# liortalker/MindTheEdge

Hardware: AMD Instinct MI355X
Metric: training images/sec, PackNet-SAN+edge-loss 384x1280 bf16 (higher is better)
Workload: dtype bf16; 1 GPU; T8: PackNet-SAN + silog + 4-scale depth-edge loss training step, 384x1280, 8 frames/GPU, dropout 0.5, flip 0.5; global_batch=8, height=384, width=1280, parallelism=single GPU

## Files before the change

### include/mte_kernels.h

```cpp
#ifndef MTE_KERNELS_H
#define MTE_KERNELS_H

#ifdef __cplusplus
extern "C" {
#endif

typedef struct ihipStream_t* mte_stream_t;

#define MTE_OK 0
#define MTE_ERR_ARG (-1)
#define MTE_ERR_LAUNCH (-2)
#define MTE_ERR_UNSUPPORTED (-3)
#define MTE_DT_BF16 0
#define MTE_DT_F32 1

#define MTE_CONV_ACCUMULATE 1
#define MTE_CONV_SOLO 2
int mte_conv2d_igemm(const void* x, long ldx, const void* wpack, const float* bias, void* y, long ldy, int out_f32,
                     int B, int H, int W, int Cin_p, int N, int KH, int KW, int dtype,
                     float* workspace, long workspace_elems, int accumulate, mte_stream_t stream);
int mte_conv2d_igemm_unshuffle(const void* x, long ldx, const void* wpack, void* y, long ldy,
                               int B, int H, int W, int Cin_p, int N, int KH, int KW, int dtype, int accumulate, mte_stream_t stream);
#define MTE_OPT_GN_PREZEROED 0
#define MTE_OPT_LOSS_PREZEROED 1
#define MTE_OPT_HANDOFF_FENCES 2
#define MTE_OPT_WGRAD_SHARES_CHIP 3
int mte_set_option(int option, int value);
#define MTE_DEVERR_GN_CLUSTER_FWD 1
#define MTE_DEVERR_GN_CLUSTER_BWD 2
#define MTE_DEVERR_IMAGE_RESAMPLE 4
int mte_device_error_init(void);
int mte_device_error_poll(void);
int mte_conv2d_wgrad(const void* x, long ldx, const void* dy, long ldy, float* dw_stage, int stage_parts, int* parts_out,
                     int B, int H, int W, int Cin_p, int N, int KH, int KW, int dtype, mte_stream_t stream);
int mte_conv2d_wgrad_nine_tap(int H, int W, int Cin_p, int N, int KH, int KW, int dtype);
int mte_pack_conv_weights(const float* w_oihw, void* wfwd, void* wbwd, int Cout, int Cin, int KH, int KW,
                          int Cin_p, int Cout_p, int dtype, mte_stream_t stream);
typedef struct { const float* w; void* wf; void* wb; void* pf; void* pb; int Cout, Cin, taps, Cin_p; int end_f, end_b, end_pf, end_pb; } mte_pack_job;
int mte_pack_conv_weights_multi(const void* jobs, int njobs, int dtype, mte_stream_t stream);
int mte_pack_conv_weights_bwd(const void* wfwd, void* wbwd, int Cout, int KH, int KW, int Cin_p, int dtype, mte_stream_t stream);
int mte_unpack_conv_wgrad(float* dw_stage, int parts, float* dw_oihw, int Cout, int Cin, int KH, int KW, int Cin_p, mte_stream_t stream);
int mte_colsum(const void* y, long ld, long M, int N, float* out, int dtype, mte_stream_t stream);

int mte_conv2d_patch_supported(int W, int Cin_p, int N, int KH, int KW, int dtype);
int mte_conv2d_patch_wgrad_supported(int W, int Cin_p, int N, int KH, int KW, int dtype);
long mte_conv2d_patch_pack_elems(int Cin_p, int N, int KH, int KW);
int mte_conv2d_patch_repack(const void* wgeneric, void* wpatch, int Cin_p, int N, int KH, int KW, mte_stream_t stream);
int mte_conv2d_patch_fwd(const void* x, long ldx, const void* wpatch, const float* bias, void* y, long ldy,
                         int B, int H, int W, int Cin_p, int N, int KH, int KW, int accumulate, mte_stream_t stream);
int mte_conv2d_patch_wgrad(const void* x, long ldx, const void* dy, long lddy, float* dw_stage, int stage_parts, int* parts_out,
                           int B, int H, int W, int Cin_p, int N, int KH, int KW, mte_stream_t stream);
long mte_conv2d_patch_fwd_gn_elems(int B, int H, int W);
int mte_conv2d_patch_fwd_gn(const void* x, long ldx, const void* wpatch, const float* bias, void* y, long ldy, int B, int H, int W, int Cin_p, int N, int KH, int KW,
                            int accumulate, float* rec, long rec_elems, int* tiles_per_sample_out, mte_stream_t stream);

int mte_conv2d_stem_supported(int W, int Cin_p, int N, int KH, int KW, int dtype);
int mte_conv2d_stem_fwd(const void* x, long ldx, const void* wf, const float* bias, void* y, long ldy,
                        int B, int H, int W, int N, int KH, int KW, mte_stream_t stream);
int mte_conv2d_stem_wgrad(const void* x, long ldx, const void* dy, long lddy, float* dw_stage, int stage_parts, int* parts_out,
                          int B, int H, int W, int N, int KH, int KW, mte_stream_t stream);

long mte_gn_stats_elems(int B);
int mte_gn_stats(const void* y1, long ld1, const void* y2, long ld2, const float* scale2, double* stats,
                 int B, int HW, int C, int dtype, mte_stream_t stream);
int mte_gn_stats_from_records(const float* rec, int tiles_per_sample, double* stats, int B, mte_stream_t stream);
int mte_gn_fwd_is_single_pass(int HW, int C, int has_y2, int dtype);
int mte_gn_fwd_is_single_pass_b(int B, int HW, int C, int has_y2, int dtype);
int mte_gn_elu_fwd(const void* y1, long ld1, const void* y2, long ld2, const float* scale2, double* stats, int stats_ready,
                   const float* gamma, const float* beta, void* z, long ldz,
                   int B, int HW, int C, float eps, int dtype, mte_stream_t stream);
int mte_gn_elu_bwd(const void* dz, long lddz, const void* y1, long ld1, const void* y2, long ld2, const float* scale2,
                   const double* stats, const float* gamma, const float* beta, float* red,
                   void* d1, long ldd1, void* d2, long ldd2, float* dgamma, float* dbeta, float* dbias,
                   int B, int HW, int C, float eps, int dtype, mte_stream_t stream);
int mte_gn_tail_fwd(const void* y1, long ld1, const double* stats1, const float* gamma1, const float* beta1,
                    const void* y2, long ld2, const float* scale2, void* t, long ldt, double* stats_t,
                    const float* gamma_t, const float* beta_t, void* z, long ldz,
                    int B, int HW, int C, float eps, int dtype, mte_stream_t stream);

int mte_pack3d_fwd(const void* x, long ldx, const float* w3, const float* b3, void* out, long ldo,
                   int B, int H, int W, int C, int dtype, mte_stream_t stream);
int mte_pack3d_bwd_data(const void* dout, long ldo, const float* w3, void* dx, long lddx,
                        int B, int H, int W, int C, int dtype, mte_stream_t stream);
int mte_pack3d_bwd_weight(const void* x, long ldx, const void* dout, long ldo, float* dwb,
                          int B, int H, int W, int C, int dtype, mte_stream_t stream);
int mte_unpack3d_fwd(const void* x, long ldx, const float* w3, const float* b3, void* out, long ldo,
                     int B, int H, int W, int C, int dtype, mte_stream_t stream);
int mte_unpack3d_bwd_data(const void* dout, long ldo, const float* w3, void* dx, long lddx,
                          int B, int H, int W, int C, int dtype, mte_stream_t stream);
int mte_unpack3d_bwd_weight(const void* x, long ldx, const void* dout, long ldo, float* dwb,
                            int B, int H, int W, int C, int dtype, mte_stream_t stream);

int mte_fold_pack_weights(const float* W, const float* K3, const float* b, const float* b3, float* Wf, float* bf,
                          int Co, int D, int k, mte_stream_t stream);
int mte_unfold_pack_wgrad(const float* dWf, const float* dbf, const float* W, const float* K3, const float* b3,
                          float* dW, float* dk3b, int Co, int D, int k, int accumulate, mte_stream_t stream);
int mte_pixel_shuffle(const void* src, long lds_, void* dst, long ldd, int B, int H, int W, int C, int dir, int dtype, mte_stream_t stream);
int mte_copy_rect(const void* src, long lds_, int Hs, int Ws, int sy, int sx, void* dst, long ldd, int Hd, int Wd, int dy, int dx,
                  int B, int h, int w, int C, int mode, int dtype, mte_stream_t stream);
typedef struct { const void* src; long lds_; int Hs, Ws, sy, sx; void* dst; long ldd; int Hd, Wd, dy, dx, h, w, mode; } mte_rect_op;
int mte_copy_rects(const void* ops, int n, int B, int C, int dtype, mte_stream_t stream);

long mte_pack_ring_work_elems(void);
long mte_pack_border_scatter_work_elems(int Co, int k);
long mte_pack_border_class_sums_elems(int Co, int k);
int mte_pack_ring_fwd(const void* P, long ldp, const float* K3, void* R_rows, void* R_cols, int B, int H2, int W2, int D, int dtype, mte_stream_t stream);
int mte_pack_ring_bwd_data(const void* dR_rows, const void* dR_cols, const float* K3, void* dx, long lddx, int B, int H2, int W2, int D, int dtype,
                           mte_stream_t stream);
int mte_pack_ring_bwd_weight(const void* dR_rows, const void* dR_cols, const void* P, long ldp, float* dk3, float* work, int B, int H2, int W2, int D,
                             int dtype, mte_stream_t stream);
int mte_pack_border_weights(const float* W, const float* b3, float* Wr, float* Wc, float* Dt, int Co, int D, int k, mte_stream_t stream);
int mte_pack_border_apply(void* y, long ldy, const float* corr_rows, const float* corr_cols, const float* Dt, int B, int H2, int W2, int Co, int k,
                          int dtype, mte_stream_t stream);
int mte_pack_border_gather(const void* dy, long lddy, void* G_rows, void* G_cols, int B, int H2, int W2, int Co, int k, int dtype, mte_stream_t stream);
int mte_pack_border_class_sums(const void* dy, long lddy, float* part, int B, int H2, int W2, int Co, int k, int dtype, mte_stream_t stream);
int mte_pack_border_scatter(const float* dWr, const float* dWc, const float* part, const float* W, const float* b3, float* dW, float* dk3b, float* work,
                            int Co, int D, int k, mte_stream_t stream);
long mte_pack_border_gemm_ws_elems(int B, int H2, int W2, int C16, int Co, int k, int dtype, int force_splits, int* splits);
int mte_pack_border_gemm_fwd(const void* R_rows, const void* R_cols, const void* Wr_pack, const void* Wc_pack, float* ws, long ws_elems, int B, int H2, int W2,
                             int C16, int Co, int k, int dtype, int force_splits, mte_stream_t stream);
int mte_pack_border_apply_slabs(void* y, long ldy, const float* ws, int splits, const float* Dt, int B, int H2, int W2, int Co, int k, int dtype,
                                mte_stream_t stream);

int mte_invdepth_fwd(const void* x, long ldx, const float* w, const float* bias, float* out,
                     int B, int H, int W, int C, float min_depth, int dtype, mte_stream_t stream);
int mte_invdepth_bwd_data(const float* w, const float* inv_out, const float* dout, float* dlogit,
                          void* dx, long lddx, int B, int H, int W, int C, float min_depth, int dtype, mte_stream_t stream);
long mte_invdepth_bwd_weight_workspace_elems(int C);
int mte_invdepth_bwd_weight(const void* x, long ldx, const float* dlogit, float* dwb, float* records,
                            int B, int H, int W, int C, int dtype, mte_stream_t stream);

int mte_rank1_conv_fwd(const float* inv, const float* w, long w_stride, void* y, long ldy, int B, int h, int wl, int N, int dtype, mte_stream_t stream);
int mte_rank1_conv_bwd_data(const void* dy, long lddy, const float* w, long w_stride, float* dinv, int B, int h, int wl, int N, int accumulate, int dtype,
                            mte_stream_t stream);
int mte_upsample2_f32(const float* inv, float* out, int B, int h, int wl, mte_stream_t stream);
int mte_conv2d_patch_fwd_rank1_ok(const float* bias, long ldx, int B, int H, int W, int Cin_p, int N);
int mte_conv2d_patch_fwd_rank1(const void* x, long ldx, const void* wpatch, const float* bias, void* y, long ldy, int B, int H, int W, int Cin_p, int N,
                               const float* inv, const float* w1, long w1_stride, mte_stream_t stream);
int mte_conv2d_patch_fwd_plus1x1(const void* x, long ldx, const void* wpatch, const float* bias, void* y, long ldy, int B, int H, int W, int Cin_p, int N,
                                 const void* x2, long ldx2, const void* wpatch2, int C2, mte_stream_t stream);
long mte_rank1_conv_bwd_records_elems(int N);
int mte_rank1_conv_bwd_weight(const void* dy, long lddy, const float* inv, float* dw, long dw_stride, float* records,
                              int B, int h, int wl, int N, int dtype, mte_stream_t stream);
int mte_nchw_to_nhwc(const float* src, void* dst, long ldd, int B, int C, int H, int W, int Cp, int flip_w, int dtype, mte_stream_t stream);
int mte_upsample_inv_fwd(const float* inv, void* dst, long ldd, int B, int h, int w, int dtype, mte_stream_t stream);
int mte_upsample_inv_bwd(const void* dsrc, long lds_, float* dinv, int B, int h, int w, int accumulate, int dtype, mte_stream_t stream);
int mte_copy_channels(const void* src, long lds_, void* dst, long ldd, long npix, int C, int dtype, mte_stream_t stream);
int mte_split_record(const float* src, float* dst0, int n0, float* dst1, int n1, mte_stream_t stream);
int mte_add_channels(const void* a, long lda, const void* b, long ldb, void* out, long ldo, long npix, int C, int dtype, mte_stream_t stream);

typedef struct { const float* pred; const float* edge; const float* normal; const float* mask; float* gmap; float* dpred; int H; int W; } mte_edge_scale;
long mte_edge_loss_work_elems(const void* scales, int nscales, int B);
int mte_edge_loss_multi_fwd(const void* scales, int nscales, int B, int from_inv, int is_grad, int is_sigmoid, float thresh,
                            float weight, float pos_to_neg, const float* gt_depth, double* work, float* losses, float* coef,
                            float* silog_loss, float* silog_aux, mte_stream_t stream);
int mte_edge_loss_multi_bwd(const void* scales, int nscales, int B, int from_inv, int is_grad, int is_sigmoid, float thresh,
                            const float* coef, const float* gout, const float* gt_depth, const float* silog_aux, const float* silog_gout,
                            mte_stream_t stream);
typedef struct { const float* pred[2]; float* dpred[2]; const float* edge; const float* normal; int H; int W; } mte_edge_pair_scale;
long mte_edge_loss_pair_work_elems(const void* scales, int nscales, int B);
int mte_edge_loss_pair_fwd(const void* scales, int nscales, int B, float thresh, float weight, float pos_to_neg,
                           const float* gt_depth, double* work, float* losses, float* coef,
                           float* silog_loss, float* silog_aux, mte_stream_t stream);
int mte_edge_loss_pair_bwd(const void* scales, int nscales, int B, float thresh, const float* coef, const float* gout,
                           const float* gt_depth, const float* silog_aux, const float* silog_gout, mte_stream_t stream);
long mte_edge_loss_sums_elems(int B, int H, int W);
int mte_edge_loss_fwd(const float* pred, const float* edge, const float* normal, const float* mask, double* sums, float* gmap,
                      int B, int H, int W, int from_inv, int is_grad, int is_sigmoid, float thresh, mte_stream_t stream);
int mte_edge_loss_finalize(const double* sums, int B, long numel, float weight, float pos_to_neg, int has_mask,
                           float out_scale, float* loss_acc, float* loss_this, float* coef, mte_stream_t stream);
int mte_edge_loss_bwd(const float* pred, const float* edge, const float* normal, const float* mask, const float* coef, const float* gout,
                      float* dpred, int B, int H, int W, int from_inv, int is_grad, int is_sigmoid, float thresh, mte_stream_t stream);

long mte_edge_loss_kind_work_elems(int B, int H, int W);
int mte_edge_loss_kind_fwd(const float* pred, const float* edge, const float* normal, const float* mask, float* gmap, int B, int H, int W,
                           int kind, int dice, int from_inv, int is_grad, int is_sigmoid, float thresh, float weight, float pos_to_neg,
                           double* work, float* loss, float* coef, mte_stream_t stream);
int mte_edge_loss_kind_bwd(const float* pred, const float* edge, const float* normal, const float* mask, const float* coef, const float* gout,
                           float* dpred, int B, int H, int W, int kind, int dice, int from_inv, int is_grad, int is_sigmoid, float thresh,
                           mte_stream_t stream);

typedef struct { const float* pred; float* dpred; int H; int W; } mte_sup_scale;
long mte_supervised_loss_work_elems(const void* scales, int nscales, int B);
int mte_supervised_loss_fwd(const void* scales, int nscales, int B, const float* depth, int Hd, int Wd, int method, int sparse,
                            double* work, float* loss, float* scale_loss, float* coef, mte_stream_t stream);
int mte_supervised_loss_bwd(const void* scales, int nscales, int B, const float* depth, int Hd, int Wd, int method, int sparse,
                            const float* coef, const float* gout, mte_stream_t stream);
typedef struct { const float* src; float* dst; int h; int w; } mte_upsample_map;
int mte_upsample_nearest_fwd(const void* maps, int nmaps, int B, int H, int W, mte_stream_t stream);
int mte_upsample_nearest_bwd(const void* maps, int nmaps, int B, int H, int W, mte_stream_t stream);

int mte_resize_bilinear_fwd(const float* x, float* y, int B, int h, int w, int H, int W, mte_stream_t stream);
int mte_resize_bilinear_bwd(const float* dy, float* dx, int B, int h, int w, int H, int W, mte_stream_t stream);

int mte_silog_fwd(const float* inv, const float* depth, long n, double* sums, float out_scale, float* loss_acc, float* loss_this, float* aux, mte_stream_t stream);
int mte_silog_bwd(const float* inv, const float* depth, const float* aux, const float* gout, float* dinv, long n, int accumulate, mte_stream_t stream);

int mte_adam_step(float* p, const float* g, float* m, float* v, long n, float lr, float beta1, float beta2, float eps,
                  int step, float gscale, mte_stream_t stream);
int mte_adam_step_dev(float* p, const float* g, float* m, float* v, long n, const float* hyper, float beta1, float beta2, float eps,
                      float gscale, mte_stream_t stream);
int mte_adamw_step(float* p, const float* g, float* m, float* v, long n, float lr, float beta1, float beta2, float eps, float weight_decay,
                   int decoupled, int step, float gscale, mte_stream_t stream);
int mte_adamw_step_dev(float* p, const float* g, float* m, float* v, long n, const float* hyper, float beta1, float beta2, float eps,
                       float weight_decay, int decoupled, float gscale, mte_stream_t stream);
int mte_sgd_step(float* p, const float* g, float* buf, long n, float lr, float momentum, float dampening, float weight_decay, int nesterov,
                 int step, float gscale, mte_stream_t stream);
int mte_sgd_step_dev(float* p, const float* g, float* buf, long n, const float* hyper, float momentum, float weight_decay, int nesterov,
                     float gscale, mte_stream_t stream);
long mte_grad_norm_work_bytes(long n);
int mte_grad_norm_clip(const float* g, long n, float gscale, float max_norm, int skip_nonfinite, void* work, float* ctl, mte_stream_t stream);
int mte_adamw_step_ctl_dev(float* p, const float* g, float* m, float* v, long n, const float* hyper, float beta1, float beta2, float eps,
                           float weight_decay, int decoupled, float gscale, const float* ctl, mte_stream_t stream);
int mte_sgd_step_ctl_dev(float* p, const float* g, float* buf, long n, const float* hyper, float momentum, float weight_decay, int nesterov,
                         float gscale, const float* ctl, mte_stream_t stream);
int mte_grad_accumulate(float* dst, const float* src, long n, int assign, mte_stream_t stream);
int mte_ema_update(float* ema, const float* p, long n, float d, float omd, mte_stream_t stream);
int mte_ema_update_dev(float* ema, const float* p, long n, const float* scal, const float* ctl, mte_stream_t stream);
int mte_flat_swap(float* a, float* b, long n, mte_stream_t stream);
int mte_adamw_step_seg_dev(float* p, const float* g, float* m, float* v, long n, const float* hyper, float beta1, float beta2, float eps,
                           float weight_decay, int decoupled, float gscale, const unsigned char* block_class, const float* class_scales,
                           int n_classes, const float* ctl, mte_stream_t stream);
int mte_sgd_step_seg_dev(float* p, const float* g, float* buf, long n, const float* hyper, float momentum, float weight_decay, int nesterov,
                         float gscale, const unsigned char* block_class, const float* class_scales, int n_classes, const float* ctl,
                         mte_stream_t stream);
long mte_tensor_stats_work_bytes(long n, int T);
int mte_tensor_stats(const float* g, const float* p, long n, const long* seg_begin, const long* seg_numel, int T, void* work, double* out,
                     mte_stream_t stream);
long mte_lamb_work_bytes(long n, int T);
int mte_lamb_moments(const float* p, const float* g, float* m, float* v, long n, const float* hyper, float beta1, float beta2, float eps,
                     float weight_decay, float gscale, float max_trust, const long* seg_begin, const long* seg_numel,
                     const float* tensor_table, int T, void* work, float* trust, double* sums, const float* ctl, mte_stream_t stream);
int mte_lamb_apply(float* p, const float* m, const float* v, long n, const float* hyper, float eps, float weight_decay,
                   const long* seg_begin, const long* seg_numel, const float* tensor_table, int T, const float* trust,
                   const float* ctl, mte_stream_t stream);

long mte_depth_metrics_workspace_bytes(int B);
int mte_depth_metrics(const float* gt, const float* pred, int B, int H, int W, int h, int w, int scale_mode, int garg_crop,
                      float min_depth, float max_depth, int use_gt_scale, void* workspace, long workspace_bytes,
                      float* out7, mte_stream_t stream);
int mte_post_process_inv_depth(const float* inv_depth, const float* inv_depth_flipped, float* out, int B, int H, int W,
                               int method, mte_stream_t stream);

int mte_dee_sobel_nms(const float* pred, float scale, unsigned char* normals_u8, float* nms, int B, int H, int W, mte_stream_t stream);
int mte_hysteresis_begin(const float* img, unsigned char* state, int* info, int B, int H, int W, double t_low, double t_high,
                         mte_stream_t stream);
int mte_hysteresis_propagate(unsigned char* state, int* flags, int sweeps, int B, int H, int W, mte_stream_t stream);
int mte_hysteresis_finish(const float* img, const unsigned char* state, const int* info, float* out, int B, int H, int W,
                          mte_stream_t stream);

long mte_chamfer_workspace_bytes(int B, int H, int W);
int mte_chamfer_distance(const float* im_pred, const float* im_gt, int B, int H, int W, double edge_to_edge_thresh,
                         void* workspace, long workspace_bytes, double* out, float* dist_map, float* cond_map, mte_stream_t stream);

int mte_canny_begin(const float* depth, int B, int H, int W, int n_pairs, const int* thresholds, unsigned* max_ws,
                    unsigned char* vis_u8, unsigned char* state, mte_stream_t stream);
int mte_resize_linear(const float* src, int B, int h, int w, float* dst, int H, int W, mte_stream_t stream);
int mte_canny_propagate(unsigned char* state, int* flags, int sweeps, int maps, int H, int W, mte_stream_t stream);
int mte_canny_finish(const unsigned char* state, float* edges, int maps, int H, int W, mte_stream_t stream);
int mte_canny_begin_fixed(const float* depth, int B, int H, int W, float min_depth, float max_depth, float factor, int n_pairs,
                          const int* thresholds, unsigned char* vis_u8, unsigned char* state, mte_stream_t stream);

long mte_edge_match_workspace_bytes(int B, int H, int W, int r2);
int mte_edge_match(const float* pred, const float* gt, const int* gt_of, int B, int Bg, int H, int W, int r2, const int* init_mate,
                   void* workspace, long workspace_bytes, int* result, int* mate_pred, mte_stream_t stream);

int mte_frame_depth_metrics(const double* gt, const float* pred, const unsigned char* mask_u8, int B, int H, int W,
                            double min_depth, double max_depth, int x0, int x1, int y0, int y1, double* out, long* counts, mte_stream_t stream);

int mte_sparsify_depth(const float* depth, void* feat, long ldf, unsigned char* mask, int B, int H, int W, int dtype, mte_stream_t stream);
long mte_sparse_site_list_workspace_elems(long npix);
int mte_sparse_site_list(const unsigned char* mask, long npix, int* sites, int* count, int* ws, mte_stream_t stream);
int mte_conv2d_igemm_sparse(const void* x, long ldx, const void* wpack, const float* bias, void* y, long ldy,
                            int B, int H, int W, int Cin_p, int N, int KH, int KW, int dtype,
                            const int* sites, const int* count, int accumulate, mte_stream_t stream);
int mte_sparse_maxpool3s2(const void* in, long ldi, const unsigned char* mask_in, void* out, long ldo, unsigned char* mask_out,
                          int B, int H, int W, int C, int dtype, mte_stream_t stream);
int mte_sparse_bn_relu(const void* a, long lda, const void* b, long ldb, const void* c, long ldc, const unsigned char* mask,
                       const float* gamma, const float* beta, const float* mean, const float* var, float eps,
                       void* out, long ldo, long npix, int C, int dtype, mte_stream_t stream);
int mte_san_fuse(const void* skip, long ld_skip, const void* sparse, long ld_sparse, const float* w, const float* bias,
                 void* out, long ldo, long npix, int C, int dtype, mte_stream_t stream);
int mte_sparse_bn_stats(const void* a, long lda, const void* b, long ldb, const void* c, long ldc, const unsigned char* mask,
                        double* sums, long npix, int C, int dtype, mte_stream_t stream);
int mte_sparse_bn_relu_bwd(const void* a, long lda, const void* b, long ldb, const void* c, long ldc, const void* out, long ldo,
                           const void* dout, long ldd, const unsigned char* mask, const float* gamma, const float* mean, const float* invstd,
                           const double* n_active, double* sums, void* dx, long ldx, long npix, int C, int dtype, mte_stream_t stream);
int mte_sparse_maxpool3s2_bwd(const void* in, long ldi, const unsigned char* mask_in, const void* dout, long ldd, void* din, long ldn,
                              int B, int H, int W, int C, int dtype, mte_stream_t stream);
int mte_san_fuse_bwd(const void* skip, long ld_skip, const void* dout, long ldd, const float* w, void* dskip, long ldk, double* sums,
                     long npix, int C, int dtype, mte_stream_t stream);
// ... 50 lines not shown
```

### mindtheedge_amd/_lib.py

```python
import ctypes
import os
import re

_HERE = os.path.dirname(os.path.abspath(__file__))
HEADER = os.path.join(os.path.dirname(_HERE), "include", "mte_kernels.h")
DEV_LIB_PATH = os.path.join(_HERE, "csrc", "libmte_hip_dev.so")
_USE_DEV = bool(os.environ.get("MTE_USE_DEV_LIB"))
LIB_PATH = os.environ.get("MTE_LIB_PATH") or (DEV_LIB_PATH if _USE_DEV else os.path.join(_HERE, "csrc", "libmte_hip.so"))

_CTYPES = {"int": ctypes.c_int, "long": ctypes.c_long, "float": ctypes.c_float, "double": ctypes.c_double, "mte_stream_t": ctypes.c_void_p}
_ERRORS = {-1: "MTE_ERR_ARG (bad argument / unsupported shape)", -2: "MTE_ERR_LAUNCH (HIP launch failed)",
           -3: "MTE_ERR_UNSUPPORTED"}


class MteError(RuntimeError):
    pass


RETURNS = {}
QUERIES = ("mte_conv2d_patch_supported", "mte_conv2d_stem_supported", "mte_conv2d_patch_wgrad_supported", "mte_conv2d_wgrad_nine_tap", "mte_conv2d_patch_fwd_gn_elems", "mte_conv2d_patch_pack_elems", "mte_depth_metrics_workspace_bytes",
           "mte_chamfer_workspace_bytes", "mte_edge_match_workspace_bytes", "mte_edge_loss_sums_elems", "mte_gn_fwd_is_single_pass", "mte_gn_fwd_is_single_pass_b",
           "mte_edge_loss_work_elems", "mte_edge_loss_pair_work_elems", "mte_edge_loss_kind_work_elems", "mte_supervised_loss_work_elems", "mte_rank1_conv_bwd_records_elems", "mte_conv2d_patch_fwd_rank1_ok", "mte_gn_stats_elems", "mte_device_error_poll", "mte_invdepth_bwd_weight_workspace_elems", "mte_sparse_site_list_workspace_elems", "mte_image_resample_work_bytes", "mte_lidar_perturb_work_bytes", "mte_order_stats_work_bytes",
           "mte_pack_ring_work_elems", "mte_pack_border_scatter_work_elems", "mte_pack_border_class_sums_elems", "mte_grad_norm_work_bytes",
           "mte_pack_border_gemm_ws_elems", "mte_tensor_stats_work_bytes", "mte_lamb_work_bytes")


def parse_header(path=HEADER, dev=False):
    text = open(path).read()
    text = re.sub(r"/\*.*?\*/", "", text, flags=re.S)
    if not dev:
        text = re.sub(r"#ifdef MTE_DEV.*?#endif", "", text, flags=re.S)
    protos = {}
    for m in re.finditer(r"\b(int|long)\s+(mte_\w+)\s*\(([^)]*)\)\s*;", text):
        RETURNS[m.group(2)] = ctypes.c_long if m.group(1) == "long" else ctypes.c_int
        args = []
        for a in ([] if m.group(3).strip() in ("", "void") else m.group(3).split(",")):
            a = " ".join(a.split())
            if "*" in a:
                args.append((ctypes.c_void_p, a.split("*")[-1].strip()))
            else:
                ty, name = a.rsplit(" ", 1)
                args.append((_CTYPES[ty.replace("const ", "").strip()], name))
        protos[m.group(2)] = args
    return protos


class _Lib:
    def __init__(self, path=None, dev=None):
        self._dll = None
        self._path = path or LIB_PATH
        self._dev = (self._path == DEV_LIB_PATH) if dev is None else bool(dev)
        self._protos = parse_header(dev=self._dev)
        self._options = {}
        self._loaded = {}

    def load(self):
        if self._dll is None:
            if not os.path.exists(self._path):
                raise MteError("%s is not built (%s). Run `python -c 'import __graft_entry__ as g; g.build()'` "
                               "or `python mindtheedge_amd/_build.py`; there is no CPU/eager fallback." % (os.path.basename(self._path), self._path))
            import torch
            dll = self._loaded.get(self._path)
            if dll is None:
                dll = self._loaded[self._path] = ctypes.CDLL(self._path)
            for name, args in self._protos.items():
                fn = getattr(dll, name)
                fn.argtypes = [t for t, _ in args]
                fn.restype = RETURNS.get(name, ctypes.c_int)
            self._dll = dll
            for opt, val in self._options.items():
                dll.mte_set_option(opt, val)
        return self._dll

    def switch(self, path, dev):
        for k in [k for k in self.__dict__ if k.startswith("mte_")]:
            del self.__dict__[k]
        self._dll, self._path, self._dev = None, path, bool(dev)
        self._protos = parse_header(dev=self._dev)

    def set_option(self, option, value, lazy=False):
        self._options[int(option)] = int(value)
        if not lazy or self._dll is not None:
            self.mte_set_option(int(option), int(value))

    def __getattr__(self, name):
        if name.startswith("mte_"):
            fn = getattr(self.load(), name)
            if name in QUERIES:
                call = fn
            else:
                def call(*args):
                    rc = fn(*args)
                    if rc != 0:
                        raise MteError("%s failed: %s" % (name, _ERRORS.get(rc, rc)))
            self.__dict__[name] = call
            return call
        raise AttributeError(name)


lib = _Lib()


class dev_library:

    def __enter__(self):
        self._prev = (lib._path, lib._dev)
        lib.switch(DEV_LIB_PATH, True)
        return lib

    def __exit__(self, *exc):
        lib.switch(*self._prev)
        return False
```

### mindtheedge_amd/csrc/conv_args.hpp

```cpp
#pragma once
#include "common.hpp"
#include "conv_plan.hpp"
#include "wgrad_plan.hpp"

struct ConvArgs {
    const void* x; long ldx;
    const void* w;
    const float* bias;
    void* y; long ldy; int out_f32;
    int B, H, W, Cin_p, N, KH, KW;
    long M;
    int splits; float* ws;
    int accum;
    int solo;
    const int* rows; const int* nrows;
    int kslice;
    int unshuffle_c;
};

__attribute__((visibility("hidden"))) int igemm8_launch(const IgemmPlan& p, const ConvArgs& a, hipStream_t st);

__attribute__((visibility("hidden"))) int wgrad9_launch(const WgradPlan& pl, const void* x, long ldx, const void* dy, long ldy, float* dw_stage,
                                                        int B, int H, int W, int Cin_p, int N, hipStream_t st);
```

### mindtheedge_amd/csrc/conv_igemm.hip

```cpp
#include "common.hpp"
#include "conv_args.hpp"

#ifdef MTE_STAMPS
__device__ unsigned long long g_igemm_stamps[16384 * 8];
extern "C" int mtei_igemm_stamps(unsigned long long* host, int n) {
    return hipMemcpyFromSymbol(host, HIP_SYMBOL(g_igemm_stamps), sizeof(unsigned long long) * n) == hipSuccess ? 0 : -1;
}
#endif

namespace {


template <typename T> struct Mma;
template <> struct Mma<bf16_t> {
    __device__ static __forceinline__ void run(const u32x4_t& a, const u32x4_t& b, f32x16_t& c) {
        c = __builtin_amdgcn_mfma_f32_32x32x16_bf16(__builtin_bit_cast(bf16x8_t, a), __builtin_bit_cast(bf16x8_t, b), c, 0, 0, 0);
    }
};
template <> struct Mma<float> {
    __device__ static __forceinline__ void run(const u32x4_t& a, const u32x4_t& b, f32x16_t& c) {
#pragma unroll
        for (int i = 0; i < 4; ++i)
            c = __builtin_amdgcn_mfma_f32_32x32x2f32(__uint_as_float(a[i]), __uint_as_float(b[i]), c, 0, 0, 0);
    }
};

#if MTE_IGEMM_MFMA16
__device__ __forceinline__ int lds_swz(int row) { return (row >> 1) & 3; }
#else
__device__ __forceinline__ int lds_swz(int row) { return (row >> 2) & 3; }
#endif
__device__ __forceinline__ int lds_chunk_off(int row, int kc) { return row * 64 + ((kc ^ lds_swz(row)) << 4); }

template <typename T> struct Mma16;
template <> struct Mma16<bf16_t> {
    __device__ static __forceinline__ void run(const u32x4_t& a, const u32x4_t& b, f32x4_t& c) {
        c = __builtin_amdgcn_mfma_f32_16x16x32_bf16(__builtin_bit_cast(bf16x8_t, a), __builtin_bit_cast(bf16x8_t, b), c, 0, 0, 0);
    }
};
template <> struct Mma16<float> {
    __device__ static __forceinline__ void run(const u32x4_t& a, const u32x4_t& b, f32x4_t& c) {
#pragma unroll
        for (int i = 0; i < 4; ++i)
            c = __builtin_amdgcn_mfma_f32_16x16x4f32(__uint_as_float(a[i]), __uint_as_float(b[i]), c, 0, 0, 0);
    }
};

__device__ u32x4_t g_zero16 = {0u, 0u, 0u, 0u};

template <typename T, int WM, int WN, int TM, int TN, int LD, int RING = 4, int MINW = 1, int ABL = 0>
__global__ __launch_bounds__(WM * WN * 64, MINW) void conv_igemm_kernel(ConvArgs a) {
    constexpr bool DMA = LD != 0;
    constexpr int NTHR = WM * WN * 64;
    constexpr int BM = WM * TM * 32, BN = WN * TN * 32;
    constexpr int PER16 = Elem<T>::PER16;
    constexpr int A_CH = BM * 4 / NTHR;
    static_assert(BM * 4 % NTHR == 0, "the A tile must split evenly over the threads");
    constexpr int B_CH = (BN * 4 + NTHR - 1) / NTHR;
    constexpr int ST = DMA ? RING : 2;
    extern __shared__ __attribute__((aligned(16))) char smem[];
    char* sA = smem;
    char* sB = smem + ST * BM * 64;

    const int tid = threadIdx.x, lane = tid & 63, wave = tid >> 6;
    const int tiles_n = (a.N + BN - 1) / BN;
    const int tiles_m = (int)((a.M + BM - 1) / BM);
    const int ntiles = tiles_m * tiles_n;
    const int split = blockIdx.x / ntiles;
    const int id = xcd_remap(blockIdx.x - split * ntiles, ntiles);
    const int tile_n = id % tiles_n, tile_m = id / tiles_n;
    const long m0 = (long)tile_m * BM;
    const long Mrows = a.rows ? (long)*a.nrows : a.M;
    if (m0 >= Mrows) return;
    const int n0 = tile_n * BN;

    const int taps = a.KH * a.KW, pad_h = a.KH >> 1, pad_w = a.KW >> 1;
    const int cpt = a.Cin_p / PER16;
    const int total_chunks = taps * cpt;
    const int ksteps_all = (total_chunks + 3) >> 2;
    const int per_split = (ksteps_all + a.splits - 1) / a.splits;
    const int s_begin = split * per_split;
    const int s_end = min(ksteps_all, s_begin + per_split);
    const long Kp = (long)taps * a.Cin_p;
    const T* __restrict__ xp = (const T*)a.x;
    const T* __restrict__ wp = (const T*)a.w;

    const int kc = DMA ? ((tid & 3) ^ lds_swz(tid >> 2)) : (tid & 3);
    int c, ty, tx;
    {
        const int q0 = 4 * s_begin + kc, tap0 = q0 / cpt;
        c = q0 - tap0 * cpt; ty = tap0 / a.KW; tx = tap0 - ty * a.KW;
    }
    long a_pix[A_CH]; int a_oy[A_CH], a_ox[A_CH]; bool a_ok[A_CH];
#pragma unroll
    for (int i = 0; i < A_CH; ++i) {
        const int row = (tid + i * NTHR) >> 2;
        const long m = m0 + row;
        a_ok[i] = m < Mrows;
        const long mm = a_ok[i] ? (a.rows ? (long)a.rows[m] : m) : 0;
        const int hw = a.H * a.W;
        const int b = (int)(mm / hw), rem = (int)(mm - (long)b * hw);
        a_oy[i] = rem / a.W; a_ox[i] = rem - a_oy[i] * a.W;
        a_pix[i] = mm;
    }
    u32x4_t ra[A_CH], rb[B_CH];

    auto load_step = [&](int s) {
        const bool tap_ok = ty < a.KH;
        const int dy = ty - pad_h, dx = tx - pad_w;
#pragma unroll
        for (int i = 0; i < A_CH; ++i) {
            const int iy = a_oy[i] + dy, ix = a_ox[i] + dx;
            const bool ok = a_ok[i] && tap_ok && (unsigned)iy < (unsigned)a.H && (unsigned)ix < (unsigned)a.W;
            u32x4_t v = {0u, 0u, 0u, 0u};
            if (ok) v = *(const u32x4_t*)(xp + (a_pix[i] + (long)dy * a.W + dx) * a.ldx + c * PER16);
            ra[i] = v;
        }
        const int q = 4 * s + kc;
#pragma unroll
        for (int i = 0; i < B_CH; ++i) {
            const int idx = tid + i * NTHR;
            const int row = idx >> 2, n = n0 + row;
            u32x4_t v = {0u, 0u, 0u, 0u};
            if (idx < BN * 4 && n < a.N && q < total_chunks) v = *(const u32x4_t*)(wp + (long)n * Kp + (long)q * PER16);
            rb[i] = v;
        }
        c += 4;
        while (c >= cpt) { c -= cpt; if (++tx == a.KW) { tx = 0; ++ty; } }
    };
    auto dma_step = [&](int s, int buf) {
        typedef const __attribute__((address_space(1))) void* gptr_t;
        typedef __attribute__((address_space(3))) void* lptr_t;
        const bool tap_ok = ty < a.KH;
        const int dy = ty - pad_h, dx = tx - pad_w;
        const int wv = __builtin_amdgcn_readfirstlane(wave);
#pragma unroll
        for (int i = 0; i < A_CH; ++i) {
            const int iy = a_oy[i] + dy, ix = a_ox[i] + dx;
            const bool ok = a_ok[i] && tap_ok && (unsigned)iy < (unsigned)a.H && (unsigned)ix < (unsigned)a.W;
            const void* src = ok ? (const void*)(xp + (a_pix[i] + (long)dy * a.W + dx) * a.ldx + c * PER16) : (const void*)&g_zero16;
            __builtin_amdgcn_global_load_lds((gptr_t)src, (lptr_t)(sA + buf * BM * 64 + (wv * 16 + i * (NTHR / 4)) * 64), 16, 0, 0);
        }
        const int q = 4 * s + kc;
#pragma unroll
        for (int i = 0; i < B_CH; ++i) {
            if (wv * 64 + i * NTHR < BN * 4) {
                const int row = (tid + i * NTHR) >> 2, n = n0 + row;
                const void* src = (n < a.N && q < total_chunks) ? (const void*)(wp + (long)n * Kp + (long)q * PER16) : (const void*)&g_zero16;
                __builtin_amdgcn_global_load_lds((gptr_t)src, (lptr_t)(sB + buf * BN * 64 + (wv * 16 + i * (NTHR / 4)) * 64), 16, 0, 0);
            }
        }
        c += 4;
        while (c >= cpt) { c -= cpt; if (++tx == a.KW) { tx = 0; ++ty; } }
    };
    constexpr unsigned OOB = 0xfffffff0u;
    constexpr int ES = (int)sizeof(T);
    unsigned voffA[A_CH], voffT[A_CH], voffB[B_CH];
    int f_ty = 0, f_tx = 0, f_cb = 0;
    auto set_tap = [&]() {
        const int dy = f_ty - pad_h, dx = f_tx - pad_w;
        const int delta = (dy * a.W + dx) * (int)a.ldx * ES;
#pragma unroll
        for (int i = 0; i < A_CH; ++i) {
            const int iy = a_oy[i] + dy, ix = a_ox[i] + dx;
            const bool ok = a_ok[i] && (unsigned)iy < (unsigned)a.H && (unsigned)ix < (unsigned)a.W;
            voffT[i] = ok ? voffA[i] + (unsigned)delta : OOB;
        }
    };
    if constexpr (LD == 2) {
#pragma unroll
        for (int i = 0; i < A_CH; ++i) voffA[i] = (unsigned)((a_pix[i] * a.ldx + kc * PER16) * ES);
#pragma unroll
        for (int i = 0; i < B_CH; ++i) {
            const int n = n0 + ((tid + i * NTHR) >> 2);
            voffB[i] = n < a.N ? (unsigned)(((long)n * Kp + kc * PER16) * ES) : OOB;
        }
        const int q0 = 4 * s_begin, tap0 = q0 / cpt;
        f_cb = q0 - tap0 * cpt; f_ty = tap0 / a.KW; f_tx = tap0 - f_ty * a.KW;
        set_tap();
    }
    auto dma_fast = [&](int s, int slot) {
#if defined(__HIP_DEVICE_COMPILE__)
        typedef __attribute__((address_space(3))) void* lptr_t;
        const auto rsA = __builtin_amdgcn_make_buffer_rsrc((void*)xp, 0, (int)(((a.M - 1) * a.ldx + a.Cin_p) * ES), 0x00020000);
        const auto rsB = __builtin_amdgcn_make_buffer_rsrc((void*)wp, 0, (int)((long)a.N * Kp * ES), 0x00020000);
        const int wv = __builtin_amdgcn_readfirstlane(wave);
        if (f_cb == cpt) {
            f_cb = 0;
            if (++f_tx == a.KW) { f_tx = 0; ++f_ty; }
            set_tap();
        }
        const int soffA = f_cb * PER16 * ES, soffB = s * 64;
#pragma unroll
        for (int i = 0; i < A_CH; ++i)
            __builtin_amdgcn_raw_ptr_buffer_load_lds(rsA, (lptr_t)(sA + slot * BM * 64 + (wv * 16 + i * (NTHR / 4)) * 64), 16, voffT[i], soffA, 0, 0);
#pragma unroll
        for (int i = 0; i < B_CH; ++i)
            __builtin_amdgcn_raw_ptr_buffer_load_lds(rsB, (lptr_t)(sB + slot * BN * 64 + (wv * 16 + i * (NTHR / 4)) * 64), 16, voffB[i], soffB, 0, 0);
        f_cb += 4;
#else
        (void)s; (void)slot;
#endif
    };
    auto store_step = [&](int buf) {
#pragma unroll
        for (int i = 0; i < A_CH; ++i) {
            const int row = (tid + i * NTHR) >> 2;
            *(u32x4_t*)(sA + buf * BM * 64 + lds_chunk_off(row, kc)) = ra[i];
        }
#pragma unroll
        for (int i = 0; i < B_CH; ++i) {
            const int idx = tid + i * NTHR;
            if (idx < BN * 4) *(u32x4_t*)(sB + buf * BN * 64 + lds_chunk_off(idx >> 2, kc)) = rb[i];
        }
    };

    const int wm = wave / WN, wn = wave % WN;
#if MTE_IGEMM_MFMA16
    static_assert(ABL == 0, "the ablation arms exist for the 32x32x16 form only");
    constexpr int AM = TM * 2, AN = TN * 2;
    f32x4_t acc[AM][AN];
#pragma unroll
    for (int i = 0; i < AM; ++i)
#pragma unroll
        for (int j = 0; j < AN; ++j) acc[i][j] = f32x4_t{0.f, 0.f, 0.f, 0.f};
    const int r16 = lane & 15, q16 = lane >> 4;
    u32x4_t fa[AM], fb[AN];
    auto read_frags = [&](int slot) {
        const char* pA = sA + slot * BM * 64;
        const char* pB = sB + slot * BN * 64;
#pragma unroll
        for (int i = 0; i < AM; ++i) fa[i] = *(const u32x4_t*)(pA + lds_chunk_off((wm * AM + i) * 16 + r16, q16));
#pragma unroll
        for (int j = 0; j < AN; ++j) fb[j] = *(const u32x4_t*)(pB + lds_chunk_off((wn * AN + j) * 16 + r16, q16));
    };
    auto mfmas = [&]() {
#pragma unroll
        for (int i = 0; i < AM; ++i)
#pragma unroll
            for (int j = 0; j < AN; ++j) Mma16<T>::run(fb[j], fa[i], acc[i][j]);
    };
    auto compute = [&](int slot) { read_frags(slot); mfmas(); };
    auto acc_row = [&](int i, int e) { (void)e; return (wm * AM + i) * 16 + r16; };
    auto acc_col = [&](int j, int e) { return (wn * AN + j) * 16 + 4 * q16 + e; };
    constexpr int AE = 4;
#else
    constexpr int AM = TM, AN = TN;
    f32x16_t acc[TM][TN];
#pragma unroll
    for (int i = 0; i < TM; ++i)
#pragma unroll
        for (int j = 0; j < TN; ++j)
#pragma unroll
            for (int e = 0; e < 16; ++e) acc[i][j][e] = 0.f;

    const int r = lane & 31, h = lane >> 5;

    auto compute = [&](int slot) {
        const char* pA = sA + slot * BM * 64;
        const char* pB = sB + slot * BN * 64;
#pragma unroll
        for (int kk = 0; kk < 2; ++kk) {
            u32x4_t fa[TM], fb[TN];
            if constexpr (ABL & 4) {
#pragma unroll
                for (int i = 0; i < TM; ++i) { fa[i] = u32x4_t{(unsigned)lane, (unsigned)i, 0x3f803f80u, 0x3f803f80u}; asm volatile("" : "+v"(fa[i])); }
#pragma unroll
                for (int j = 0; j < TN; ++j) { fb[j] = u32x4_t{(unsigned)lane, (unsigned)j, 0x3f803f80u, 0x3f803f80u}; asm volatile("" : "+v"(fb[j])); }
            } else {
#pragma unroll
            for (int i = 0; i < TM; ++i) fa[i] = *(const u32x4_t*)(pA + lds_chunk_off((wm * TM + i) * 32 + r, 2 * kk + h));
#pragma unroll
            for (int j = 0; j < TN; ++j) fb[j] = *(const u32x4_t*)(pB + lds_chunk_off((wn * TN + j) * 32 + r, 2 * kk + h));
            }
            if constexpr (ABL & 1) {
#pragma unroll
                for (int i = 0; i < TM; ++i) asm volatile("" ::"v"(fa[i]));
#pragma unroll
                for (int j = 0; j < TN; ++j) asm volatile("" ::"v"(fb[j]));
            } else {
#pragma unroll
            for (int i = 0; i < TM; ++i)
#pragma unroll
                for (int j = 0; j < TN; ++j) Mma<T>::run(fa[i], fb[j], acc[i][j]);
            }
        }
    };
    auto acc_row = [&](int i, int e) { return (wm * TM + i) * 32 + (e & 3) + 8 * (e >> 2) + 4 * h; };
    auto acc_col = [&](int j, int e) { (void)e; return (wn * TN + j) * 32 + r; };
    constexpr int AE = 16;
#endif
    if constexpr (DMA) {
        static_assert((BN * 4) % NTHR == 0, "every wave must issue the same number of DMA instructions per stage");
        static_assert(ST == 3 || ST == 4 || ST == 6, "wait ladder below is written for 3, 4 or 6 slots");
        constexpr int LPS = A_CH + B_CH;
        constexpr int AHEAD = ST - 1;
        const int nst = s_end - s_begin;
#pragma unroll
        for (int p = 0; p < AHEAD; ++p)
            if (p < nst) { if constexpr (LD == 2) dma_fast(s_begin + p, p); else dma_step(s_begin + p, p); }
#if MTE_IGEMM_MFMA16
        constexpr bool PP = LD == 2 && WM == 2 && WN == 4 && TM == 4 && TN == 2 && ST == 4;
        if constexpr (PP) {
            const int grp = __builtin_amdgcn_readfirstlane(wm);
            {
                if (nst >= 3) asm volatile("s_waitcnt vmcnt(%0)" ::"n"(2 * LPS) : "memory");
                else if (nst == 2) asm volatile("s_waitcnt vmcnt(%0)" ::"n"(LPS) : "memory");
                else asm volatile("s_waitcnt vmcnt(0)" ::: "memory");
                __builtin_amdgcn_s_barrier();
            }
            if (grp == 1) __builtin_amdgcn_s_barrier();
#ifdef MTE_STAMPS
            unsigned long long t_wait = 0, t_bar = 0, t_dma = 0, t_cmp = 0, t_a, t_b;
            const unsigned long long t_start = __builtin_amdgcn_s_memtime();
#define PP_STAMP(ACC) { __builtin_amdgcn_sched_barrier(0); t_b = __builtin_amdgcn_s_memtime(); ACC += t_b - t_a; t_a = t_b; __builtin_amdgcn_sched_barrier(0); }
#else
#define PP_STAMP(ACC)
#endif
            for (int k = 0; k < nst; ++k) {
#ifdef MTE_STAMPS
                t_a = __builtin_amdgcn_s_memtime();
#endif
                const int rem = nst - 2 - k;
                read_frags(k % ST);
                if (k + AHEAD < nst) dma_fast(s_begin + k + AHEAD, (k + AHEAD) % ST);
                asm volatile("s_waitcnt lgkmcnt(0)" ::: "memory");
                if (rem >= 2) asm volatile("s_waitcnt vmcnt(%0)" ::"n"(2 * LPS) : "memory");
                else if (rem == 1) asm volatile("s_waitcnt vmcnt(%0)" ::"n"(LPS) : "memory");
                else asm volatile("s_waitcnt vmcnt(0)" ::: "memory");
                PP_STAMP(t_dma)
                __builtin_amdgcn_s_barrier();
                PP_STAMP(t_bar)
                mfmas();
                PP_STAMP(t_cmp)
                if (rem >= 2) asm volatile("s_waitcnt vmcnt(%0)" ::"n"(2 * LPS) : "memory");
                else if (rem == 1) asm volatile("s_waitcnt vmcnt(%0)" ::"n"(LPS) : "memory");
                else asm volatile("s_waitcnt vmcnt(0)" ::: "memory");
                __builtin_amdgcn_s_barrier();
                PP_STAMP(t_wait)
// ... 126 lines not shown
#pragma unroll
                    for (int e = 0; e < AE; ++e) {
                        const int row = acc_row(i, e);
                        Elem<T>::st((T*)(smem + (row * BN) * ES + (((col / PER16) + row) % CPR_) * 16 + (col % PER16) * ES), acc[i][j][e] + bv);
                    }
            }
#endif
            __syncthreads();
            constexpr int CPR = BN / PER16;
            const int cvalid = (a.N - n0) / PER16;
            const int cc = tid % CPR;
            if constexpr (sizeof(T) == 2 && BN % 32 == 0) {
                if (a.unshuffle_c) {
                    constexpr int C8 = BN / 32;
                    const int hw = a.H * a.W;
                    for (int idx = tid; idx < BM * C8; idx += NTHR) {
                        const int row = idx / C8, c8l = idx - row * C8;
                        const int c0 = (n0 >> 2) + c8l * 8;
                        const long m = m0 + row;
                        if (m < Mrows && c0 + 8 <= a.unshuffle_c) {
                            const int b = (int)(m / hw), rem = (int)(m - (long)b * hw);
                            const int h = rem / a.W, w = rem - h * a.W;
                            const char* rowp = smem + (row * BN) * ES;
                            u32x4_t q[4];
#pragma unroll
                            for (int j = 0; j < 4; ++j) q[j] = *(const u32x4_t*)(rowp + ((4 * c8l + j + row) % CPR) * 16);
                            T* dst0 = (T*)a.y + ((((long)b * 2 * a.H + 2 * h) * (2 * a.W) + 2 * w) * a.ldy + c0);
#pragma unroll
                            for (int s_ = 0; s_ < 4; ++s_) {
                                u32x4_t c;
#pragma unroll
                                for (int j = 0; j < 4; ++j) c[j] = __builtin_amdgcn_perm(q[j][2 + (s_ >> 1)], q[j][s_ >> 1], (s_ & 1) ? 0x07060302u : 0x05040100u);
                                T* dst = dst0 + ((long)(s_ >> 1) * (2 * a.W) + (s_ & 1)) * a.ldy;
                                if (a.accum) {
                                    float vn[PER16], vo[PER16];
                                    unpack16<T>(c, vn);
                                    unpack16<T>(*(const u32x4_t*)dst, vo);
#pragma unroll
                                    for (int k = 0; k < PER16; ++k) vn[k] += vo[k];
                                    c = pack16<T>(vn);
                                }
                                *(u32x4_t*)dst = c;
                            }
                        }
                    }
                    return;
                }
            }
#pragma unroll
            for (int it = 0; it < BM * CPR / NTHR; ++it) {
                const int row = tid / CPR + it * (NTHR / CPR);
                const long m = m0 + row;
                if (m < Mrows && cc < cvalid) {
                    const long pm = a.rows ? (long)a.rows[m] : m;
                    u32x4_t c = *(const u32x4_t*)(smem + (row * BN) * ES + ((cc + row) % CPR) * 16);
                    if (a.accum) {
                        float vn[PER16], vo[PER16];
                        unpack16<T>(c, vn);
                        unpack16<T>(*(const u32x4_t*)((const T*)a.y + pm * a.ldy + n0 + cc * PER16), vo);
#pragma unroll
                        for (int k = 0; k < PER16; ++k) vn[k] += vo[k];
                        c = pack16<T>(vn);
                    }
                    *(u32x4_t*)((T*)a.y + pm * a.ldy + n0 + cc * PER16) = c;
                }
            }
            return;
        }
    }

#pragma unroll
    for (int j = 0; j < AN; ++j) {
#pragma unroll
        for (int i = 0; i < AM; ++i) {
#pragma unroll
            for (int e = 0; e < AE; ++e) {
                const int n = n0 + acc_col(j, e);
                if (n >= a.N) continue;
                const float bv = a.bias ? a.bias[n] : 0.f;
                const long m = m0 + acc_row(i, e);
                if (m < Mrows) {
                    const float v = acc[i][j][e] + bv;
                    const long pm = a.rows ? (long)a.rows[m] : m;
                    if (a.splits > 1) a.ws[((long)split * a.M + m) * a.N + n] = acc[i][j][e];
                    else if (a.out_f32) ((float*)a.y)[pm * a.ldy + n] = a.accum ? v + ((float*)a.y)[pm * a.ldy + n] : v;
                    else Elem<T>::st((T*)a.y + pm * a.ldy + n, a.accum ? Elem<T>::rnd(v) + Elem<T>::ld((const T*)a.y + pm * a.ldy + n) : v);
                }
            }
        }
    }
}


template <typename T>
__global__ void splitk_finish_kernel(const float* __restrict__ ws, int splits, const float* __restrict__ bias, T* y, long ldy, long M, int N, int accum) {
    const long n4 = M * N / 4;
    for (long i = blockIdx.x * (long)blockDim.x + threadIdx.x; i < n4; i += (long)gridDim.x * blockDim.x) {
        const long m = (i * 4) / N; const int n = (int)((i * 4) % N);
        f32x4_t v = ((const f32x4_t*)ws)[i];
        for (int s = 1; s < splits; ++s) v += ((const f32x4_t*)ws)[(long)s * n4 + i];
#pragma unroll
        for (int k = 0; k < 4; ++k) {
            const float r = v[k] + (bias ? bias[n + k] : 0.f);
            Elem<T>::st(y + m * ldy + n + k, accum ? Elem<T>::rnd(r) + Elem<T>::ld(y + m * ldy + n + k) : r);
        }
    }
}

IgemmKnobs g_igemm_knobs;

template <auto Kernel> int launch_instance(const IgemmPlan& p, const ConvArgs& a, hipStream_t st) {
    if (p.lds_optin && mte_allow_lds<Kernel>(p.lds_bytes) != MTE_OK) return MTE_ERR_LAUNCH;
    hipLaunchKernelGGL(Kernel, dim3(p.grid), dim3(p.threads), p.lds_bytes, st, a);
    return MTE_OK;
}

constexpr int igemm_instance(IgemmForm f, int elem_size, int loader, int ring = 4) { return (((int)f * 2 + (elem_size == 4)) * 4 + loader) * 8 + ring; }

#if defined(MTE_DEV) && !MTE_IGEMM_MFMA16
template <int WM, int WN, int TM, int TN> int launch_ablated_tile(const IgemmPlan& p, const ConvArgs& a, hipStream_t st) {
    switch (p.ablate) {
    case 1: return launch_instance<conv_igemm_kernel<bf16_t, WM, WN, TM, TN, 2, 4, 1, 1>>(p, a, st);
    case 2: return launch_instance<conv_igemm_kernel<bf16_t, WM, WN, TM, TN, 2, 4, 1, 2>>(p, a, st);
    case 3: return launch_instance<conv_igemm_kernel<bf16_t, WM, WN, TM, TN, 2, 4, 1, 3>>(p, a, st);
    case 4: return launch_instance<conv_igemm_kernel<bf16_t, WM, WN, TM, TN, 2, 4, 1, 4>>(p, a, st);
    case 5: return launch_instance<conv_igemm_kernel<bf16_t, WM, WN, TM, TN, 2, 4, 1, 5>>(p, a, st);
    case 6: return launch_instance<conv_igemm_kernel<bf16_t, WM, WN, TM, TN, 2, 4, 1, 6>>(p, a, st);
    default: return launch_instance<conv_igemm_kernel<bf16_t, WM, WN, TM, TN, 2, 4, 1, 7>>(p, a, st);
    }
}
int launch_ablated(const IgemmPlan& p, const ConvArgs& a, hipStream_t st) {
    switch (p.form) {
    case IgemmForm::T256x128: return launch_ablated_tile<4, 2, 2, 2>(p, a, st);
    case IgemmForm::T128x128: return launch_ablated_tile<2, 2, 2, 2>(p, a, st);
    case IgemmForm::T256x256_PP: return launch_ablated_tile<2, 4, 4, 2>(p, a, st);
    case IgemmForm::T256x256_W16: return launch_ablated_tile<4, 4, 2, 2>(p, a, st);
    default: return MTE_ERR_UNSUPPORTED;
    }
}
#else
int launch_ablated(const IgemmPlan&, const ConvArgs&, hipStream_t) { return MTE_ERR_UNSUPPORTED; }
#endif

int launch_plan(const IgemmPlan& p, ConvArgs a, hipStream_t st) {
    using F = IgemmForm;
    if (p.rc != MTE_OK) return p.rc;
    a.splits = p.splits;
    a.kslice = p.kslice;
    int rc = MTE_ERR_UNSUPPORTED;
#define MTE_IGEMM_CASE(FORM, T, WM, WN, TM, TN, ...) \
    case igemm_instance(FORM, sizeof(T), __VA_ARGS__): rc = launch_instance<conv_igemm_kernel<T, WM, WN, TM, TN, __VA_ARGS__>>(p, a, st); break
    if (p.form == F::P8_256x256 || p.form == F::P8_256x128) rc = igemm8_launch(p, a, st);
    else if (p.ablate) rc = launch_ablated(p, a, st);
    else switch (igemm_instance(p.form, p.elem_size, p.loader, p.ring)) {
    MTE_IGEMM_CASE(F::T128x32, bf16_t, 4, 1, 1, 1, 0);
    MTE_IGEMM_CASE(F::T128x32_W2, bf16_t, 2, 1, 2, 1, 2);
    MTE_IGEMM_CASE(F::T128x32_W2, bf16_t, 2, 1, 2, 1, 1);
    MTE_IGEMM_CASE(F::T128x64, bf16_t, 2, 2, 2, 1, 2);
    MTE_IGEMM_CASE(F::T128x64, bf16_t, 2, 2, 2, 1, 1);
    MTE_IGEMM_CASE(F::T128x64, bf16_t, 2, 2, 2, 1, 0);
    MTE_IGEMM_CASE(F::T128x128, bf16_t, 2, 2, 2, 2, 2);
    MTE_IGEMM_CASE(F::T128x128, bf16_t, 2, 2, 2, 2, 1);
    MTE_IGEMM_CASE(F::T128x128, bf16_t, 2, 2, 2, 2, 0);
    MTE_IGEMM_CASE(F::T192x96, bf16_t, 2, 3, 3, 1, 2);
    MTE_IGEMM_CASE(F::T192x96, bf16_t, 2, 3, 3, 1, 1);
    MTE_IGEMM_CASE(F::T256x128, bf16_t, 4, 2, 2, 2, 2);
    MTE_IGEMM_CASE(F::T256x128, bf16_t, 4, 2, 2, 2, 1);
    MTE_IGEMM_CASE(F::T256x128, bf16_t, 4, 2, 2, 2, 2, 6);
    case igemm_instance(F::T256x128, 2, 2, 3): rc = launch_instance<conv_igemm_kernel<bf16_t, 4, 2, 2, 2, 2, 3, 4>>(p, a, st); break;
    MTE_IGEMM_CASE(F::T256x256_PP, bf16_t, 2, 4, 4, 2, 2);
    MTE_IGEMM_CASE(F::T256x256_PP, bf16_t, 2, 4, 4, 2, 1);
    MTE_IGEMM_CASE(F::T256x256_W16, bf16_t, 4, 4, 2, 2, 2);
    MTE_IGEMM_CASE(F::T256x256_W16, bf16_t, 4, 4, 2, 2, 1);
    MTE_IGEMM_CASE(F::T128x32, float, 4, 1, 1, 1, 0);
    MTE_IGEMM_CASE(F::T128x64, float, 2, 2, 2, 1, 2);
    MTE_IGEMM_CASE(F::T128x64, float, 2, 2, 2, 1, 1);
    MTE_IGEMM_CASE(F::T128x64, float, 2, 2, 2, 1, 0);
    MTE_IGEMM_CASE(F::T128x128, float, 2, 2, 2, 2, 2);
    MTE_IGEMM_CASE(F::T128x128, float, 2, 2, 2, 2, 1);
    MTE_IGEMM_CASE(F::T128x128, float, 2, 2, 2, 2, 0);
    }
#undef MTE_IGEMM_CASE
    if (rc != MTE_OK) return rc;
    if (p.finish) {
        if (p.elem_size == 2) hipLaunchKernelGGL(splitk_finish_kernel<bf16_t>, dim3(p.finish_grid), dim3(256), 0, st, a.ws, a.splits, a.bias, (bf16_t*)a.y, a.ldy, a.M, a.N, a.accum);
        else hipLaunchKernelGGL(splitk_finish_kernel<float>, dim3(p.finish_grid), dim3(256), 0, st, a.ws, a.splits, a.bias, (float*)a.y, a.ldy, a.M, a.N, a.accum);
    }
    return mte_check_launch();
}

#ifdef MTE_DEV
constexpr bool kDevBuild = true;
#else
constexpr bool kDevBuild = false;
#endif

int plan_and_launch(const ConvArgs& a, int elem_size, long ws_elems, hipStream_t st) {
    const IgemmProblem p{elem_size, a.M, a.N, a.Cin_p, a.KH, a.KW, a.ldx, a.out_f32, a.rows != nullptr, a.unshuffle_c, a.solo, a.ws != nullptr, ws_elems};
    return launch_plan(plan_igemm(p, g_igemm_knobs, kDevBuild), a, st);
}

struct WgradArgs {
    const void* x; long ldx;
    const void* dy; long ldy;
    float* dw;
    int B, H, W, Cin_p, N, KH, KW;
    long M;
    int splits, blocks_per_split;
    int tiles_c, tiles_n;
    long part_stride;
};

template <int BYTES> __device__ __forceinline__ int padded_row(void) {
    return (BYTES % 128 == 64) ? BYTES : BYTES + 64;
}

template <typename T, int WNO, int WC, int TNO, int TC, bool FL>
__global__ __launch_bounds__(256) void conv_wgrad_kernel(WgradArgs a) {
    constexpr int BNO = WNO * TNO * 32, BC = WC * TC * 32;
    constexpr int PER16 = Elem<T>::PER16, ES = (int)sizeof(T);
    constexpr int RS_Y = (BNO * ES % 128 == 64) ? BNO * ES : BNO * ES + 64;
    constexpr int RS_X = (BC * ES % 128 == 64) ? BC * ES : BC * ES + 64;
    constexpr int KB = 32;
    constexpr int YCH = KB * BNO / PER16, XCH = KB * BC / PER16;
    constexpr int YCT = (YCH + 255) / 256, XCT = (XCH + 255) / 256;
    constexpr int YCPR = BNO / PER16, XCPR = BC / PER16;
    extern __shared__ __attribute__((aligned(16))) char smem[];
    char* sY = smem;
    char* sX = smem + 2 * KB * RS_Y;

    const int tid = threadIdx.x, lane = tid & 63, wave = tid >> 6;
    int id = blockIdx.x;
    const int taps = a.KH * a.KW;
    const int tile_c = id % a.tiles_c; id /= a.tiles_c;
    const int tap = id % taps; id /= taps;
    const int tile_n = id % a.tiles_n; id /= a.tiles_n;
    const int split = id;
    const int ty = tap / a.KW, tx = tap % a.KW;
    const int dyo = ty - (a.KH >> 1), dxo = tx - (a.KW >> 1);
    const int n0 = tile_n * BNO, c0 = tile_c * BC;
    const T* __restrict__ xp = (const T*)a.x;
    const T* __restrict__ yp = (const T*)a.dy;

    const int bpr = (a.W + KB - 1) / KB;
    const long nblk_total = FL ? (long)a.B * a.H * bpr : (a.M + KB - 1) / KB;
    const long blk0 = (long)split * a.blocks_per_split;
    long blk1 = blk0 + a.blocks_per_split; if (blk1 > nblk_total) blk1 = nblk_total;

    int y_row[YCT], y_cc[YCT], x_row[XCT], x_cc[XCT];
    int x_b[XCT], x_oy[XCT], x_ox[XCT];
#pragma unroll
    for (int i = 0; i < YCT; ++i) { const int idx = tid + i * 256; y_row[i] = idx / YCPR; y_cc[i] = idx % YCPR; }
#pragma unroll
    for (int i = 0; i < XCT; ++i) {
        const int idx = tid + i * 256; x_row[i] = idx / XCPR; x_cc[i] = idx % XCPR;
        const long m = blk0 * KB + x_row[i];
        const int hw = a.H * a.W;
        const int b = (int)(m / hw), rem = (int)(m - (long)b * hw);
        x_b[i] = b; x_oy[i] = rem / a.W; x_ox[i] = rem - x_oy[i] * a.W;
    }
    u32x4_t ry[YCT], rx[XCT];
    auto load_step = [&](long blk) {
#pragma unroll
        for (int i = 0; i < YCT; ++i) {
            const long m = blk * KB + y_row[i];
            const int n = n0 + y_cc[i] * PER16;
            u32x4_t v = {0u, 0u, 0u, 0u};
            if ((YCH % 256 == 0 || tid + i * 256 < YCH) && m < a.M && n < a.N) v = *(const u32x4_t*)(yp + m * a.ldy + n);
            ry[i] = v;
        }
#pragma unroll
        for (int i = 0; i < XCT; ++i) {
            const int cc = c0 + x_cc[i] * PER16;
            const int iy = x_oy[i] + dyo, ix = x_ox[i] + dxo;
            const bool ok = (XCH % 256 == 0 || tid + i * 256 < XCH) && x_b[i] < a.B && cc < a.Cin_p &&
                            (unsigned)iy < (unsigned)a.H && (unsigned)ix < (unsigned)a.W;
            u32x4_t v = {0u, 0u, 0u, 0u};
            if (ok) v = *(const u32x4_t*)(xp + (((long)x_b[i] * a.H + iy) * a.W + ix) * a.ldx + cc);
            rx[i] = v;
            x_ox[i] += KB;
            while (x_ox[i] >= a.W) { x_ox[i] -= a.W; if (++x_oy[i] == a.H) { x_oy[i] = 0; ++x_b[i]; } }
        }
    };
    constexpr unsigned OOB = 0xfffffff0u;
    const int padw = a.KW >> 1;
    unsigned voffY[YCT], voffX[XCT];
    int f_xb = 0, f_y = 0, f_b = 0;
    if constexpr (FL) {
        f_xb = (int)(blk0 % bpr); const long t = blk0 / bpr; f_y = (int)(t % a.H); f_b = (int)(t / a.H);
#pragma unroll
        for (int i = 0; i < YCT; ++i) {
            const int n = n0 + y_cc[i] * PER16;
            voffY[i] = ((YCH % 256 == 0 || tid + i * 256 < YCH) && n < a.N) ? (unsigned)((y_row[i] * a.ldy + n) * ES) : OOB;
        }
#pragma unroll
        for (int i = 0; i < XCT; ++i) {
            const int cc = c0 + x_cc[i] * PER16;
            voffX[i] = ((XCH % 256 == 0 || tid + i * 256 < XCH) && cc < a.Cin_p) ? (unsigned)(((x_row[i] + dxo + padw) * a.ldx + cc) * ES) : OOB;
        }
    }
    auto load_fast = [&]() {
#if defined(__HIP_DEVICE_COMPILE__)
        const auto rsY = __builtin_amdgcn_make_buffer_rsrc((void*)yp, 0, (int)(((a.M - 1) * a.ldy + a.N) * ES), 0x00020000);
        const auto rsX = __builtin_amdgcn_make_buffer_rsrc((void*)(xp - (long)padw * a.ldx), 0, (int)(((a.M - 1 + padw) * a.ldx + a.Cin_p) * ES), 0x00020000);
        const int x0 = f_xb * KB, rem = a.W - x0;
        const int yy = f_y + dyo;
        const bool row_ok = (unsigned)yy < (unsigned)a.H;
        const int soffY = (int)((((long)f_b * a.H + f_y) * a.W + x0) * a.ldy * ES);
        const int soffX = (int)((((long)f_b * a.H + yy) * a.W + x0) * a.ldx * ES);
#pragma unroll
        for (int i = 0; i < YCT; ++i)
            ry[i] = __builtin_amdgcn_raw_buffer_load_b128(rsY, y_row[i] < rem ? voffY[i] : OOB, soffY, 0);
#pragma unroll
        for (int i = 0; i < XCT; ++i) {
            const bool ok = row_ok && (unsigned)(x0 + x_row[i] + dxo) < (unsigned)a.W;
            rx[i] = __builtin_amdgcn_raw_buffer_load_b128(rsX, ok ? voffX[i] : OOB, row_ok ? soffX : 0, 0);
        }
        if (++f_xb == bpr) { f_xb = 0; if (++f_y == a.H) { f_y = 0; ++f_b; } }
#endif
    };
    auto store_step = [&](int buf) {
#pragma unroll
        for (int i = 0; i < YCT; ++i)
            if (YCH % 256 == 0 || tid + i * 256 < YCH) *(u32x4_t*)(sY + buf * KB * RS_Y + y_row[i] * RS_Y + y_cc[i] * 16) = ry[i];
#pragma unroll
        for (int i = 0; i < XCT; ++i)
            if (XCH % 256 == 0 || tid + i * 256 < XCH) *(u32x4_t*)(sX + buf * KB * RS_X + x_row[i] * RS_X + x_cc[i] * 16) = rx[i];
    };

    f32x16_t acc[TNO][TC];
#pragma unroll
    for (int i = 0; i < TNO; ++i)
#pragma unroll
        for (int j = 0; j < TC; ++j)
#pragma unroll
            for (int e = 0; e < 16; ++e) acc[i][j][e] = 0.f;

    const int wno = wave / WC, wc = wave % WC;
    const int r = lane & 31, h = lane >> 5;

    if (blk0 < blk1) {
        if constexpr (FL) load_fast(); else load_step(blk0);
        store_step(0);
        __syncthreads();
        for (long blk = blk0; blk < blk1; ++blk) {
            const int buf = (int)((blk - blk0) & 1);
            if (blk + 1 < blk1) { if constexpr (FL) load_fast(); else load_step(blk + 1); }
            const char* pY = sY + buf * KB * RS_Y;
            const char* pX = sX + buf * KB * RS_X;
            if constexpr (sizeof(T) == 2) {
                const int g = lane >> 4, li = lane & 15, q = li >> 2, p = li & 3;
                const int chb = 16 * (g & 1) + 4 * p, pxb = 8 * (g >> 1) + q;
#pragma unroll
                for (int kk = 0; kk < 2; ++kk) {
// ... 727 lines not shown
```

### mindtheedge_amd/csrc/conv_igemm8.hip

```cpp
#include "common.hpp"
#include "conv_args.hpp"

#ifdef MTE_STAMPS
__device__ unsigned long long g_igemm8_stamps[4096 * 24];
extern "C" int mtei_igemm8_stamps(unsigned long long* host, int n) {
    return hipMemcpyFromSymbol(host, HIP_SYMBOL(g_igemm8_stamps), sizeof(unsigned long long) * n) == hipSuccess ? 0 : -1;
}
#endif

MTE_CLOCK_DEFINE(igemm8)

namespace {

constexpr unsigned OOB8 = 0xfffffff0u;

__device__ __forceinline__ f32x4_t mma16(const u32x4_t& a, const u32x4_t& b, const f32x4_t& c) {
    return __builtin_amdgcn_mfma_f32_16x16x32_bf16(__builtin_bit_cast(bf16x8_t, a), __builtin_bit_cast(bf16x8_t, b), c, 0, 0, 0);
}

template <int BN, bool SM = false, bool ONE = false>
__global__ __launch_bounds__(512, 2) void conv_igemm8_kernel(ConvArgs a) {
    static_assert(!(SM && ONE), "the slice-major order has its own single tap state");
    typedef bf16_t T;
    constexpr int BM = 256, HM = 128, HN = BN / 2;
    constexpr int WN = BN == 256 ? 4 : 2;
    constexpr int QA = BN == 256 ? 4 : 2, QB = 2;
    constexpr int IA = 2, IB = BN == 256 ? 2 : 1;
    constexpr int A_BYTES = 4 * HM * 64, B_BYTES = 4 * HN * 64;
    constexpr int BUF = A_BYTES + B_BYTES;
    extern __shared__ __attribute__((aligned(16))) char smem[];

    const int tid = threadIdx.x, lane = tid & 63;
    const int wv = __builtin_amdgcn_readfirstlane(tid >> 6);
    const int wm = wv / WN, wn = wv % WN;
    const int grp = wv >> 2;
    const int tiles_n = (a.N + BN - 1) / BN;
    const int tiles_m = (int)((a.M + BM - 1) / BM);
    const int ntiles = tiles_m * tiles_n;
    const int split = blockIdx.x / ntiles;
    const int id = xcd_remap(blockIdx.x - split * ntiles, ntiles);
    const int tile_n = id % tiles_n, tile_m = id / tiles_n;
    const long m0 = (long)tile_m * BM;
    const int n0 = tile_n * BN;

    const int pad_h = a.KH >> 1, pad_w = a.KW >> 1;
    const int taps = a.KH * a.KW;
    const int cpt = a.Cin_p >> 3;
    const int ksteps_all = (taps * cpt) >> 2;
    constexpr bool sm = SM;
    const int units_all = sm ? ksteps_all >> 1 : ksteps_all;
    const int per_split = (units_all + a.splits - 1) / a.splits;
    const int s_begin = split * per_split;
    const int s_end = min(units_all, s_begin + per_split);
    const int nkt = s_end > s_begin ? (sm ? s_end - s_begin : (s_end - s_begin + 1) >> 1) : 0;
    const long Kp = (long)taps * a.Cin_p;
    const T* __restrict__ xp = (const T*)a.x;
    const T* __restrict__ wp = (const T*)a.w;

    const int lrow = wv * 16 + (lane >> 2);
    const int kc = (lane & 3) ^ ((lane >> 3) & 3);
    int a_oy[2], a_ox[2]; unsigned voffA[2]; bool a_ok[2];
#pragma unroll
    for (int h = 0; h < 2; ++h) {
        const long m = m0 + h * HM + lrow;
        a_ok[h] = m < a.M;
        const long mm = a_ok[h] ? m : 0;
        const int hw = a.H * a.W;
        const int b = (int)(mm / hw), rem = (int)(mm - (long)b * hw);
        a_oy[h] = rem / a.W; a_ox[h] = rem - a_oy[h] * a.W;
        voffA[h] = (unsigned)((mm * a.ldx + kc * 8) * 2);
    }
    const int brow = BN == 256 ? lrow : (wv & 3) * 16 + (lane >> 2);
    unsigned voffB[2];
#pragma unroll
    for (int h = 0; h < 2; ++h) {
        const int n = n0 + h * HN + brow;
        voffB[h] = n < a.N ? (unsigned)(((long)n * Kp + kc * 8) * 2) : OOB8;
    }
    int st_s[2], st_ty[2], st_tx[2], st_cb[2];
    bool st_live[2];
    int a_t = s_begin, a_slice = 0;
    unsigned voffT[2][2];
    auto set_tap = [&](int kh) {
#ifdef MTE_I8_TAP0
        const int dy = 0, dx = 0;
#else
        const int dy = st_ty[kh] - pad_h, dx = st_tx[kh] - pad_w;
#endif
        const int delta = (dy * a.W + dx) * (int)a.ldx * 2;
#pragma unroll
        for (int h = 0; h < 2; ++h) {
            const int iy = a_oy[h] + dy, ix = a_ox[h] + dx;
            const bool ok = a_ok[h] && (unsigned)iy < (unsigned)a.H && (unsigned)ix < (unsigned)a.W;
            voffT[kh][h] = ok ? voffA[h] + (unsigned)delta : OOB8;
        }
    };
    auto sm_place = [&]() {
        const int tap = st_ty[0] * a.KW + st_tx[0];
#pragma unroll
        for (int kh = 0; kh < 2; ++kh) {
            st_cb[kh] = a_slice * 8 + 4 * kh;
            st_s[kh] = tap * (cpt >> 2) + a_slice * 2 + kh;
            st_live[kh] = a_t < s_end;
        }
        st_ty[1] = st_ty[0]; st_tx[1] = st_tx[0];
        set_tap(0);
        voffT[1][0] = voffT[0][0]; voffT[1][1] = voffT[0][1];
    };
    if (sm) {
        a_slice = s_begin / taps;
        const int tap0 = s_begin - a_slice * taps;
        st_ty[0] = tap0 / a.KW; st_tx[0] = tap0 - st_ty[0] * a.KW;
        sm_place();
    } else {
#pragma unroll
        for (int kh = 0; kh < 2; ++kh) {
            st_s[kh] = s_begin + kh;
            st_live[kh] = st_s[kh] < s_end;
            const int q0 = 4 * st_s[kh], tap0 = q0 / cpt;
            st_cb[kh] = q0 - tap0 * cpt; st_ty[kh] = tap0 / a.KW; st_tx[kh] = tap0 - st_ty[kh] * a.KW;
            set_tap(kh);
        }
    }
    auto advance = [&]() {
        if (sm) {
            ++a_t;
            if (++st_tx[0] == a.KW) { st_tx[0] = 0; if (++st_ty[0] == a.KH) { st_ty[0] = 0; ++a_slice; } }
            sm_place();
            return;
        }
        if constexpr (ONE) {
            st_s[0] += 2; st_cb[0] += 8;
            st_live[0] = st_s[0] < s_end;
            if (st_cb[0] >= cpt) {
                st_cb[0] = 0;
                if (++st_tx[0] == a.KW) { st_tx[0] = 0; ++st_ty[0]; }
                set_tap(0);
            }
            return;
        }
#pragma unroll
        for (int kh = 0; kh < 2; ++kh) {
            st_s[kh] += 2; st_cb[kh] += 8;
            st_live[kh] = st_s[kh] < s_end;
            if (st_cb[kh] >= cpt) {
                do { st_cb[kh] -= cpt; if (++st_tx[kh] == a.KW) { st_tx[kh] = 0; ++st_ty[kh]; } } while (st_cb[kh] >= cpt);
                set_tap(kh);
            }
        }
    };
    int b_t = s_begin, b_tap = 0, b_slice = 0, b_sp0 = s_begin;
    if (sm) { b_slice = s_begin / taps; b_tap = s_begin - b_slice * taps; b_sp0 = b_tap * (cpt >> 2) + b_slice * 2; }
    auto advanceB = [&]() {
        if (sm) {
            ++b_t;
            if (++b_tap == taps) { b_tap = 0; ++b_slice; }
            b_sp0 = b_tap * (cpt >> 2) + b_slice * 2;
        } else { b_t += 2; b_sp0 += 2; }
    };
#if defined(__HIP_DEVICE_COMPILE__)
    typedef __attribute__((address_space(3))) void* lptr_t;
    const auto rsA = __builtin_amdgcn_make_buffer_rsrc((void*)xp, 0, (int)(((a.M - 1) * a.ldx + a.Cin_p) * 2), 0x00020000);
    const auto rsB = __builtin_amdgcn_make_buffer_rsrc((void*)wp, 0, (int)((long)a.N * Kp * 2), 0x00020000);
#endif
    auto stageA = [&](int h, int buf) {
#if defined(__HIP_DEVICE_COMPILE__)
#pragma unroll
        for (int kh = 0; kh < 2; ++kh) {
            if constexpr (ONE) {
                const unsigned vo = st_live[0] ? voffT[0][h] : OOB8;
                __builtin_amdgcn_raw_ptr_buffer_load_lds(rsA, (lptr_t)(smem + buf * BUF + (h * 2 + kh) * (HM * 64) + wv * 1024), 16, vo, (st_cb[0] + 4 * kh) * 16, 0, 0);
            } else {
                const unsigned vo = st_live[kh] ? voffT[kh][h] : OOB8;
                __builtin_amdgcn_raw_ptr_buffer_load_lds(rsA, (lptr_t)(smem + buf * BUF + (h * 2 + kh) * (HM * 64) + wv * 1024), 16, vo, st_cb[kh] * 16, 0, 0);
            }
        }
#endif
    };
    auto stageB = [&](int h, int buf) {
#if defined(__HIP_DEVICE_COMPILE__)
        if constexpr (BN == 256) {
#pragma unroll
            for (int kh = 0; kh < 2; ++kh) {
                const bool live = (sm || ONE) ? b_t < s_end : b_t + kh < s_end;
                __builtin_amdgcn_raw_ptr_buffer_load_lds(rsB, (lptr_t)(smem + buf * BUF + A_BYTES + (h * 2 + kh) * (HN * 64) + wv * 1024), 16,
                                                         live ? voffB[h] : OOB8, (b_sp0 + kh) * 64, 0, 0);
            }
        } else {
            const int kh = wv >> 2;
            const bool live = (sm || ONE) ? b_t < s_end : b_t + kh < s_end;
            __builtin_amdgcn_raw_ptr_buffer_load_lds(rsB, (lptr_t)(smem + buf * BUF + A_BYTES + (h * 2 + kh) * (HN * 64) + (wv & 3) * 1024), 16,
                                                     live ? voffB[h] : OOB8, (b_sp0 + kh) * 64, 0, 0);
        }
#endif
    };

    const int r16 = lane & 15, q16 = lane >> 4;
    const int swz = (q16 ^ ((r16 >> 1) & 3)) << 4;
    const int offA = (wm * QA * 16 + r16) * 64 + swz;
    const int offB = A_BYTES + (wn * QB * 16 + r16) * 64 + swz;
    u32x4_t fa[QA][2], fb0[QB][2], fb1[QB][2];
    f32x4_t acc[2][QA][2][QB];
#pragma unroll
    for (int h = 0; h < 2; ++h)
#pragma unroll
        for (int i = 0; i < QA; ++i)
#pragma unroll
            for (int g = 0; g < 2; ++g)
#pragma unroll
                for (int j = 0; j < QB; ++j) acc[h][i][g][j] = f32x4_t{0.f, 0.f, 0.f, 0.f};
    auto readA = [&](int h, const char* pb) {
#pragma unroll
        for (int kh = 0; kh < 2; ++kh)
#pragma unroll
            for (int i = 0; i < QA; ++i) fa[i][kh] = *(const u32x4_t*)(pb + offA + (h * 2 + kh) * (HM * 64) + i * 1024);
    };
    auto readB = [&](int g, u32x4_t (&fb)[QB][2], const char* pb) {
#pragma unroll
        for (int kh = 0; kh < 2; ++kh)
#pragma unroll
            for (int j = 0; j < QB; ++j) fb[j][kh] = *(const u32x4_t*)(pb + offB + (g * 2 + kh) * (HN * 64) + j * 1024);
    };
    auto quadrant = [&](int h, int g, const u32x4_t (&fb)[QB][2]) {
        __builtin_amdgcn_s_setprio(1);
#pragma unroll
        for (int kh = 0; kh < 2; ++kh)
#pragma unroll
            for (int i = 0; i < QA; ++i)
#pragma unroll
                for (int j = 0; j < QB; ++j) acc[h][i][g][j] = mma16(fb[j][kh], fa[i][kh], acc[h][i][g][j]);
        __builtin_amdgcn_s_setprio(0);
    };
#define MTE8_WAIT_VM(N) asm volatile("s_waitcnt vmcnt(%0)" ::"n"(N) : "memory")
#define MTE8_WAIT_LGKM(N) asm volatile("s_waitcnt lgkmcnt(%0)" ::"n"(N) : "memory")
#define MTE8_BARRIER() { __builtin_amdgcn_sched_barrier(0); __builtin_amdgcn_s_barrier(); __builtin_amdgcn_sched_barrier(0); }

    stageB(0, 0); stageA(0, 0); stageB(1, 0); stageA(1, 0);
    advance(); advanceB();
    stageB(0, 1); stageA(0, 1); stageB(1, 1);
    advanceB();
    MTE8_WAIT_VM(2 * IB + IA);
    MTE8_BARRIER();
    if (grp == 1) MTE8_BARRIER();
#ifdef MTE_STAMPS
    unsigned long long t_st[16] = {0, 0, 0, 0, 0, 0, 0, 0, 0, 0, 0, 0, 0, 0, 0, 0}, t_a, t_b;
    const unsigned long long t_start = __builtin_amdgcn_s_memtime();
#define ST8(ACC) { __builtin_amdgcn_sched_barrier(0); t_b = __builtin_amdgcn_s_memtime(); t_st[ACC] += t_b - t_a; t_a = t_b; __builtin_amdgcn_sched_barrier(0); }
#else
#define ST8(ACC)
#endif
    MTE_CLOCK_BEGIN()
    for (int kt = 0; kt < nkt; ++kt) {
        const int buf = kt & 1;
        const char* pb = smem + buf * BUF;
#ifdef MTE_STAMPS
        t_a = __builtin_amdgcn_s_memtime();
#endif
        readB(0, fb0, pb);
        __builtin_amdgcn_sched_barrier(0);
        readA(0, pb);
        stageA(1, buf ^ 1);
        MTE8_WAIT_LGKM(QA * 2);
        ST8(0)
        MTE8_BARRIER();
        ST8(1)
        MTE8_WAIT_LGKM(0);
        __builtin_amdgcn_sched_barrier(0);
        quadrant(0, 0, fb0);
        ST8(2)
        MTE8_BARRIER();
        ST8(3)
        readB(1, fb1, pb);
        stageB(0, buf);
        advance();
        ST8(4)
        MTE8_BARRIER();
        ST8(5)
        MTE8_WAIT_LGKM(0);
        __builtin_amdgcn_sched_barrier(0);
        quadrant(0, 1, fb1);
        ST8(6)
        MTE8_BARRIER();
        ST8(7)
        readA(1, pb);
        stageA(0, buf);
        ST8(8)
        MTE8_BARRIER();
        ST8(9)
        MTE8_WAIT_LGKM(0);
        __builtin_amdgcn_sched_barrier(0);
        quadrant(1, 1, fb1);
        ST8(10)
        MTE8_BARRIER();
        ST8(11)
        stageB(1, buf);
        advanceB();
        MTE8_WAIT_VM(2 * IB + IA);
        ST8(12)
        MTE8_BARRIER();
        ST8(13)
        quadrant(1, 0, fb0);
        ST8(14)
        MTE8_BARRIER();
        ST8(15)
    }
    MTE_CLOCK_END(igemm8)
    if (grp == 0) MTE8_BARRIER();
#ifdef MTE_STAMPS
    if (lane == 0 && blockIdx.x < 512) {
        unsigned long long* o = g_igemm8_stamps + ((long)blockIdx.x * 8 + wv) * 24;
#pragma unroll
        for (int k = 0; k < 16; ++k) o[k] = t_st[k];
        o[16] = __builtin_amdgcn_s_memtime() - t_start; o[17] = nkt;
    }
#endif
    MTE8_WAIT_VM(0);
    MTE8_BARRIER();

    if (a.splits > 1) {
#pragma unroll
        for (int h = 0; h < 2; ++h)
#pragma unroll
            for (int i = 0; i < QA; ++i) {
                const long m = m0 + h * HM + (wm * QA + i) * 16 + r16;
#pragma unroll
                for (int g = 0; g < 2; ++g)
#pragma unroll
                    for (int j = 0; j < QB; ++j) {
                        const int n = n0 + g * HN + (wn * QB + j) * 16 + 4 * q16;
                        if (m < a.M && n < a.N) *(f32x4_t*)(a.ws + ((long)split * a.M + m) * a.N + n) = acc[h][i][g][j];
                    }
            }
        return;
    }
    constexpr int ROWB = BN * 2, CPR = BN / 8;
    static_assert(BM * ROWB <= 2 * BUF, "output tile must fit the ring");
#pragma unroll
    for (int g = 0; g < 2; ++g)
#pragma unroll
        for (int j = 0; j < QB; ++j) {
            const int col = g * HN + (wn * QB + j) * 16 + 4 * q16;
            f32x4_t bv = {0.f, 0.f, 0.f, 0.f};
            if (a.bias && n0 + col < a.N) {
#pragma unroll
                for (int e = 0; e < 4; ++e) bv[e] = a.bias[n0 + col + e];
            }
#pragma unroll
            for (int h = 0; h < 2; ++h)
#pragma unroll
                for (int i = 0; i < QA; ++i) {
                    const int row = h * HM + (wm * QA + i) * 16 + r16;
                    const f32x4_t v = acc[h][i][g][j] + bv;
                    uint2 pk; pk.x = pack2bf(v[0], v[1]); pk.y = pack2bf(v[2], v[3]);
                    *(uint2*)(smem + row * ROWB + ((((col >> 3) ^ r16)) << 4) + (col & 7) * 2) = pk;
                }
        }
    __syncthreads();
    const int cvalid = (a.N - n0) >> 3;
    const int cc = tid % CPR;
#pragma unroll
    for (int it = 0; it < BM * CPR / 512; ++it) {
        const int row = tid / CPR + it * (512 / CPR);
        const long m = m0 + row;
        if (m < a.M && cc < cvalid) {
            u32x4_t c = *(const u32x4_t*)(smem + row * ROWB + ((cc ^ (row & 15)) << 4));
            T* dst = (T*)a.y + m * a.ldy + n0 + cc * 8;
            if (a.accum) {
                float vn[8], vo[8];
                unpack16<T>(c, vn);
                unpack16<T>(*(const u32x4_t*)dst, vo);
#pragma unroll
                for (int k = 0; k < 8; ++k) vn[k] += vo[k];
                c = pack16<T>(vn);
            }
            *(u32x4_t*)dst = c;
        }
    }
}


template <auto Kernel> int launch8(const IgemmPlan& p, const ConvArgs& a, hipStream_t st) {
    if (mte_allow_lds<Kernel>(p.lds_bytes) != MTE_OK) return MTE_ERR_LAUNCH;
    hipLaunchKernelGGL(Kernel, dim3(p.grid), dim3(p.threads), p.lds_bytes, st, a);
    return MTE_OK;
}

}

int igemm8_launch(const IgemmPlan& p, const ConvArgs& a, hipStream_t st) {
    const bool wide = p.form == IgemmForm::P8_256x256;
    if (p.kslice) {
#ifdef MTE_DEV
        return wide ? launch8<conv_igemm8_kernel<256, true>>(p, a, st) : launch8<conv_igemm8_kernel<128, true>>(p, a, st);
#else
        return MTE_ERR_UNSUPPORTED;
#endif
    }
    if (p.one) return wide ? launch8<conv_igemm8_kernel<256, false, true>>(p, a, st) : launch8<conv_igemm8_kernel<128, false, true>>(p, a, st);
    return wide ? launch8<conv_igemm8_kernel<256, false>>(p, a, st) : launch8<conv_igemm8_kernel<128, false>>(p, a, st);
}
```

### mindtheedge_amd/csrc/conv_patch.hip

```cpp
#include "common.hpp"
#include "patch_plan.hpp"
#include <type_traits>

#ifdef MTE_STAMPS
__device__ unsigned long long g_patch_stamps[16384 * 16];
extern "C" int mtei_patch_stamps(unsigned long long* host, int n) {
    return hipMemcpyFromSymbol(host, HIP_SYMBOL(g_patch_stamps), sizeof(unsigned long long) * n) == hipSuccess ? 0 : -1;
}
#define PATCH_STAMP_DECL int stamp_i_ = 0
#define PATCH_STAMP()                                                                                                              \
    {                                                                                                                               \
        if (threadIdx.x == 0 && blockIdx.x < 16384 && stamp_i_ < 16) g_patch_stamps[blockIdx.x * 16 + stamp_i_] = __builtin_amdgcn_s_memrealtime(); \
        ++stamp_i_;                                                                                                                 \
    }
#else
#define PATCH_STAMP_DECL
#define PATCH_STAMP()
#endif

MTE_CLOCK_DEFINE(patch)

namespace {

constexpr int TH = 8, TW = 32;
typedef __attribute__((ext_vector_type(2))) unsigned int u32x2_t;

__device__ __forceinline__ int swz_off(int p, int kc) { return p * 64 + ((kc ^ ((p >> 2) & 3)) << 4); }

struct PatchArgs {
    const bf16_t* x; long ldx;
    const bf16_t* wp;
    const float* bias;
    bf16_t* y; long ldy;
    int B, H, W, Cin_p, N;
    int accum;
    const float* r1_inv;
    const float* r1_w; long r1_ws;
    const bf16_t* x2; long ldx2; const bf16_t* wp2; int C2;
    float* gn_rec;
};

__device__ __forceinline__ void patch_gn_add(const u32x4_t& v, bool ok, float* s, float* q) {
    float f[8];
    unpack16<bf16_t>(v, f);
#pragma unroll
    for (int k = 0; k < 8; ++k) { const float t = ok ? f[k] : 0.f; s[k] += t; q[k] = fmaf(t, t, q[k]); }
}
template <int NT>
__device__ __forceinline__ void patch_gn_record(const PatchArgs& a, float* s, float* q, int tid, long tile, char* smem) {
    constexpr int NC = NT * 4;
    const int lane = tid & 63, wave = tid >> 6, c = tid % NC;
#pragma unroll
    for (int k = 0; k < 8; ++k)
#pragma unroll
        for (int off = NC; off < 64; off <<= 1) { s[k] += __shfl_xor(s[k], off, 64); q[k] += __shfl_xor(q[k], off, 64); }
    __syncthreads();
    float* sred = (float*)smem;
    if (lane < NC) {
#pragma unroll
        for (int k = 0; k < 8; ++k) { sred[(wave * NC + c) * 16 + k] = s[k]; sred[(wave * NC + c) * 16 + 8 + k] = q[k]; }
    }
    __syncthreads();
    if (tid < 32) {
        const int g = tid >> 1, which = tid & 1, gs = a.N >> 4;
        float t = 0.f;
        for (int ch = g * gs; ch < (g + 1) * gs; ++ch)
#pragma unroll
            for (int w = 0; w < 4; ++w) t += sred[(w * NC + (ch >> 3)) * 16 + which * 8 + (ch & 7)];
        a.gn_rec[tile * 32 + tid] = t;
    }
}


template <int MM, int Q> struct ExtraFrags { u32x4_t px[Q][MM][2], w[Q][2]; };
template <int MM, int NT, int Q>
__device__ __forceinline__ void extra_load(ExtraFrags<MM, Q>& f, const PatchArgs& a, int s2, int b, int yrow0, int xcol, int h, int nsel, int lane) {
    const int cp2 = a.C2 >> 3, n2 = (a.C2 + 31) >> 5;
#pragma unroll
    for (int q = 0; q < Q; ++q) {
        const int sl = s2 + q;
        const bool sok = sl < n2;
#pragma unroll
        for (int kk = 0; kk < 2; ++kk) {
            const u32x4_t wv = *((const u32x4_t*)a.wp2 + lane + ((long)((sok ? sl : 0) * 2 + kk) * NT + nsel) * 64);
            f.w[q][kk] = sok ? wv : u32x4_t{0u, 0u, 0u, 0u};
            const int cc = sl * 4 + kk * 2 + h;
            const bool cok = sok && cc < cp2;
#pragma unroll
            for (int m = 0; m < MM; ++m) {
                const int yy = yrow0 + m;
                const bool ok = cok && yy < a.H;
                const u32x4_t v = *(const u32x4_t*)(a.x2 + (((long)b * a.H + (yy < a.H ? yy : a.H - 1)) * a.W + xcol) * a.ldx2 + (cok ? cc : 0) * 8);
                f.px[q][m][kk] = ok ? v : u32x4_t{0u, 0u, 0u, 0u};
            }
        }
    }
}

template <int MM, int NT, int Q>
__device__ __forceinline__ void extra_load16(ExtraFrags<MM, Q>& f, const PatchArgs& a, int s2, int b, int yrow0, int x0, int c16, int g16, unsigned w16off) {
    const int cp2 = a.C2 >> 3, n2 = (a.C2 + 31) >> 5;
#pragma unroll
    for (int q = 0; q < Q; ++q) {
        const int sl = s2 + q;
        const bool sok = sl < n2;
#pragma unroll
        for (int c = 0; c < 2; ++c) {
            const u32x4_t wv = *(const u32x4_t*)((const char*)a.wp2 + (long)(sok ? sl : 0) * (2 * NT * 1024) + w16off + c * 256);
            f.w[q][c] = sok ? wv : u32x4_t{0u, 0u, 0u, 0u};
        }
        const int cc = sl * 4 + g16;
        const bool cok = sok && cc < cp2;
#pragma unroll
        for (int m = 0; m < MM; ++m) {
            const int yy = yrow0 + m;
            const bool ok = cok && yy < a.H;
#pragma unroll
            for (int ph = 0; ph < 2; ++ph) {
                const u32x4_t v = *(const u32x4_t*)(a.x2 + (((long)b * a.H + (yy < a.H ? yy : a.H - 1)) * a.W + x0 + 16 * ph + c16) * a.ldx2 + (cok ? cc : 0) * 8);
                f.px[q][m][ph] = ok ? v : u32x4_t{0u, 0u, 0u, 0u};
            }
        }
    }
}

template <int K, int NT, bool TALL, bool ACC = false, bool EXTRA = false, bool M16 = false>
__global__ __launch_bounds__(256, 2) void conv_patch_fwd_kernel(PatchArgs a) {
    static_assert(!TALL || NT == 1, "tall tiles are for the 32-output kernels");
    static_assert(!EXTRA || K == 3, "the 1x1 second source rides the 3x3 kernels");
    constexpr int TH = TALL ? 16 : 8;
    constexpr int PAD = K / 2, PH = TH + K - 1, PW = TW + K - 1, TAPS = K * K;
    constexpr int PCH = PH * PW * 4;
    constexpr int NCH = (PCH + 255) / 256;
    constexpr int PBYTES = PH * PW * 64;
    constexpr int OSTR = M16 ? NT * 64 + 16 : NT * 64;
    constexpr int OBYTES = TH * TW * OSTR;
    constexpr int NBUF = (TALL && K > 3) ? 1 : 2;
    constexpr int LDS_BYTES = ((NBUF * PBYTES > OBYTES) ? NBUF * PBYTES : OBYTES);
    __shared__ __attribute__((aligned(16))) char smem[LDS_BYTES];

    const int tid = threadIdx.x, lane = tid & 63, wave = tid >> 6;
    const int r = lane & 31, h = lane >> 5;
    const int tiles_x = a.W / TW, tiles_y = (a.H + TH - 1) / TH;
    int id = xcd_remap(blockIdx.x, tiles_x * tiles_y * a.B);
    const int tx_ = id % tiles_x; id /= tiles_x;
    const int ty_ = id % tiles_y; const int b = id / tiles_y;
    const int x0 = tx_ * TW, y0 = ty_ * TH;
    const int cpt = a.Cin_p >> 3;
    const int nslices = (a.Cin_p + 31) >> 5;

    u32x4_t st[NCH];
    auto load_patch = [&](int s) {
#pragma unroll
        for (int i = 0; i < NCH; ++i) {
// ... 783 lines not shown
            for (int e = 0; e < 16; ++e) {
                const int co = (nh * NT + n) * 32 + (e & 3) + 8 * (e >> 2) + 4 * h;
                if (co < a.N) {
                    float* dst = a.dw + (long)blockIdx.x * a.part_stride + ((long)co * TAPS + tap) * a.Cin_p + cc;
                    if (a.part_stride) *dst = acc[i][n][e]; else atomicAdd(dst, acc[i][n][e]);
                }
            }
    }
}

static_assert(TH == PATCH_TH && TW == PATCH_TW, "patch_plan.hpp counts the tiles the kernels walk");

PatchKnobs g_patch_knobs;

template <auto K> int launch_patch_fwd(const PatchPlan& pl, const PatchArgs& a, hipStream_t st) {
    hipLaunchKernelGGL(K, dim3(pl.grid_x), dim3(pl.block), 0, st, a);
    return mte_check_launch();
}
template <auto K> int launch_patch_wgrad(const PatchPlan& pl, const PatchWgradArgs& a, hipStream_t st) {
    if (mte_allow_lds<K>((int)pl.lds) != MTE_OK) return MTE_ERR_LAUNCH;
    hipLaunchKernelGGL(K, dim3(pl.grid_x, pl.grid_y), dim3(pl.block), pl.lds, st, a);
    return mte_check_launch();
}

#define PATCH_FWD(...) case patch_fwd_key(__VA_ARGS__): return launch_patch_fwd<conv_patch_fwd_kernel<__VA_ARGS__>>(pl, a, st);
#define PATCH_FWD2(...) case patch_fwd2_key(__VA_ARGS__): return launch_patch_fwd<conv_patch_fwd2_kernel<__VA_ARGS__>>(pl, a, st);
#define PATCH_WGRAD(...) case patch_wgrad_key(__VA_ARGS__): return launch_patch_wgrad<conv_patch_wgrad_kernel<__VA_ARGS__>>(pl, a, st);
#ifdef MTE_DEV
#define PATCH_FWD_32(...) PATCH_FWD(__VA_ARGS__, false)
#define PATCH_FWD2_32(...) PATCH_FWD2(__VA_ARGS__, false)
#else
#define PATCH_FWD_32(...)
#define PATCH_FWD2_32(...)
#endif
int launch_patch_plan(const PatchPlan& pl, const PatchArgs& a, hipStream_t st) {
    if (pl.rc != MTE_OK) return pl.rc;
    switch (patch_key(pl)) {
    PATCH_FWD_32(1, 1, true, true, false) PATCH_FWD_32(1, 1, true, false, false) PATCH_FWD(1, 1, true, true, false, true) PATCH_FWD(1, 1, true, false, false, true)
    PATCH_FWD_32(1, 1, false, true, false) PATCH_FWD_32(1, 1, false, false, false) PATCH_FWD(1, 1, false, true, false, true) PATCH_FWD(1, 1, false, false, false, true)
    PATCH_FWD2_32(3, 1, true, false, true, false) PATCH_FWD2_32(3, 1, true, false, false, false) PATCH_FWD2(3, 1, true, false, true, false, true) PATCH_FWD2(3, 1, true, false, false, false, true)
    PATCH_FWD_32(3, 1, true, true, false) PATCH_FWD_32(3, 1, true, false, false) PATCH_FWD(3, 1, true, true, false, true) PATCH_FWD(3, 1, true, false, false, true)
    PATCH_FWD2_32(3, 1, false, false, true, false) PATCH_FWD2_32(3, 1, false, false, false, false) PATCH_FWD2(3, 1, false, false, true, false, true) PATCH_FWD2(3, 1, false, false, false, false, true)
    PATCH_FWD_32(3, 1, false, true, false) PATCH_FWD_32(3, 1, false, false, false) PATCH_FWD(3, 1, false, true, false, true) PATCH_FWD(3, 1, false, false, false, true)
    PATCH_FWD2_32(5, 1, true, false, true, false) PATCH_FWD2_32(5, 1, true, false, false, false) PATCH_FWD2(5, 1, true, false, true, false, true) PATCH_FWD2(5, 1, true, false, false, false, true)
    PATCH_FWD_32(5, 1, true, true, false) PATCH_FWD_32(5, 1, true, false, false) PATCH_FWD(5, 1, true, true, false, true) PATCH_FWD(5, 1, true, false, false, true)
    PATCH_FWD2_32(5, 1, false, false, true, false) PATCH_FWD2_32(5, 1, false, false, false, false) PATCH_FWD2(5, 1, false, false, true, false, true) PATCH_FWD2(5, 1, false, false, false, false, true)
    PATCH_FWD_32(5, 1, false, true, false) PATCH_FWD_32(5, 1, false, false, false) PATCH_FWD(5, 1, false, true, false, true) PATCH_FWD(5, 1, false, false, false, true)
    PATCH_FWD2_32(7, 1, true, false, true, false) PATCH_FWD2_32(7, 1, true, false, false, false) PATCH_FWD2(7, 1, true, false, true, false, true) PATCH_FWD2(7, 1, true, false, false, false, true)
    PATCH_FWD_32(7, 1, true, true, false) PATCH_FWD_32(7, 1, true, false, false) PATCH_FWD(7, 1, true, true, false, true) PATCH_FWD(7, 1, true, false, false, true)
    PATCH_FWD2_32(7, 1, false, false, true, false) PATCH_FWD2_32(7, 1, false, false, false, false) PATCH_FWD2(7, 1, false, false, true, false, true) PATCH_FWD2(7, 1, false, false, false, false, true)
    PATCH_FWD_32(7, 1, false, true, false) PATCH_FWD_32(7, 1, false, false, false) PATCH_FWD(7, 1, false, true, false, true) PATCH_FWD(7, 1, false, false, false, true)
    PATCH_FWD_32(1, 2, false, true, false) PATCH_FWD_32(1, 2, false, false, false) PATCH_FWD(1, 2, false, true, false, true) PATCH_FWD(1, 2, false, false, false, true)
    PATCH_FWD2_32(3, 2, false, false, true, false) PATCH_FWD2_32(3, 2, false, false, false, false) PATCH_FWD2(3, 2, false, false, true, false, true) PATCH_FWD2(3, 2, false, false, false, false, true)
    PATCH_FWD_32(3, 2, false, true, false) PATCH_FWD_32(3, 2, false, false, false) PATCH_FWD(3, 2, false, true, false, true) PATCH_FWD(3, 2, false, false, false, true)
    PATCH_FWD2_32(5, 2, false, false, true, false) PATCH_FWD2_32(5, 2, false, false, false, false) PATCH_FWD2(5, 2, false, false, true, false, true) PATCH_FWD2(5, 2, false, false, false, false, true)
    PATCH_FWD_32(5, 2, false, true, false) PATCH_FWD_32(5, 2, false, false, false) PATCH_FWD(5, 2, false, true, false, true) PATCH_FWD(5, 2, false, false, false, true)
    PATCH_FWD2_32(3, 1, true, true, false, false) PATCH_FWD2(3, 1, true, true, false, false, true)
    PATCH_FWD2_32(3, 1, false, true, false, false) PATCH_FWD2(3, 1, false, true, false, false, true)
    PATCH_FWD2_32(3, 2, false, true, false, false) PATCH_FWD2(3, 2, false, true, false, false, true)
    PATCH_FWD2_32(3, 1, true, false, false, true) PATCH_FWD2(3, 1, true, false, false, true, true)
    PATCH_FWD_32(3, 1, true, false, true) PATCH_FWD(3, 1, true, false, true, true)
    PATCH_FWD2_32(3, 1, false, false, false, true) PATCH_FWD2(3, 1, false, false, false, true, true)
    PATCH_FWD_32(3, 1, false, false, true) PATCH_FWD(3, 1, false, false, true, true)
    PATCH_FWD2_32(3, 2, false, false, false, true) PATCH_FWD2(3, 2, false, false, false, true, true)
    PATCH_FWD_32(3, 2, false, false, true) PATCH_FWD(3, 2, false, false, true, true)
    }
    return MTE_ERR_UNSUPPORTED;
}
int launch_patch_plan(const PatchPlan& pl, PatchWgradArgs a, hipStream_t st) {
    if (pl.rc != MTE_OK) return pl.rc;
    a.groups = pl.groups; a.part_stride = pl.part_stride;
    if (pl.clear_bytes && mte_memset_async(a.dw, 0, pl.clear_bytes, st) != hipSuccess) return MTE_ERR_LAUNCH;
    switch (patch_key(pl)) {
    PATCH_WGRAD(3, 2, 2, 8, 2, 4)
    PATCH_WGRAD(1, 1, 2, 4, 1, 8) PATCH_WGRAD(1, 1, 1, 4, 1, 8) PATCH_WGRAD(3, 1, 3, 8, 1, 8) PATCH_WGRAD(3, 1, 2, 4, 1, 8)
    PATCH_WGRAD(3, 1, 1, 4, 1, 8) PATCH_WGRAD(5, 1, 2, 8, 1, 8) PATCH_WGRAD(5, 1, 2, 4, 1, 8) PATCH_WGRAD(5, 1, 1, 4, 1, 8)
    PATCH_WGRAD(7, 1, 1, 8, 1, 8) PATCH_WGRAD(7, 1, 1, 4, 1, 8)
    PATCH_WGRAD(1, 2, 2, 4, 1, 8) PATCH_WGRAD(1, 2, 1, 4, 1, 8) PATCH_WGRAD(3, 2, 3, 8, 1, 4) PATCH_WGRAD(3, 2, 2, 8, 1, 8)
    PATCH_WGRAD(3, 2, 2, 4, 1, 8) PATCH_WGRAD(3, 2, 1, 4, 1, 8) PATCH_WGRAD(5, 2, 1, 8, 1, 8) PATCH_WGRAD(5, 2, 1, 4, 1, 8)
    }
    return MTE_ERR_UNSUPPORTED;
}
#undef PATCH_FWD
#undef PATCH_FWD2
#undef PATCH_WGRAD
#undef PATCH_FWD_32
#undef PATCH_FWD2_32

PatchProblem fwd_problem(PatchOp op, const float* bias, long ldx, int B, int H, int W, int Cin_p, int N, int KH, int KW, int accumulate = 0, int C2 = 0) {
    return {op, B, H, W, Cin_p, N, KH, KW, ldx, accumulate != 0, ((uintptr_t)bias & 15) == 0, C2, 0, false};
}

}

#ifdef MTE_DEV
extern "C" int mtei_set_patch_tall(int v) { return patch_knob_set(g_patch_knobs, v); }
#endif

extern "C" {

int mte_conv2d_patch_supported(int W, int Cin_p, int N, int KH, int KW, int dtype) {
    return (dtype == MTE_DT_BF16 && plan_patch(fwd_problem(PatchOp::Fwd, nullptr, Cin_p, 1, 1, W, Cin_p, N, KH, KW), g_patch_knobs).rc == MTE_OK) ? 1 : 0;
}

int mte_conv2d_patch_wgrad_supported(int W, int Cin_p, int N, int KH, int KW, int dtype) {
    const PatchProblem p{PatchOp::Wgrad, 1, 1, W, Cin_p, N, KH, KW, Cin_p, false, true, 0, 1, false};
    return (dtype == MTE_DT_BF16 && plan_patch(p, g_patch_knobs).rc == MTE_OK) ? 1 : 0;
}

long mte_conv2d_patch_pack_elems(int Cin_p, int N, int KH, int KW) {
    return (long)((Cin_p + 31) / 32) * KH * KW * 2 * ((N + 31) / 32) * 64 * 8;
}

int mte_conv2d_patch_repack(const void* wgeneric, void* wpatch, int Cin_p, int N, int KH, int KW, hipStream_t stream) {
    (void)hipGetLastError();
    if (!wgeneric || !wpatch) return MTE_ERR_ARG;
    const long total = mte_conv2d_patch_pack_elems(Cin_p, N, KH, KW);
    long g = (total + 255) / 256; if (g > 4096) g = 4096;
    hipLaunchKernelGGL(repack_patch_kernel, dim3((unsigned)g), dim3(256), 0, stream, (const bf16_t*)wgeneric, (bf16_t*)wpatch, N, KH * KW, Cin_p, (N + 31) / 32);
    return mte_check_launch();
}

int mte_conv2d_patch_fwd(const void* x, long ldx, const void* wpatch, const float* bias, void* y, long ldy,
                         int B, int H, int W, int Cin_p, int N, int KH, int KW, int accumulate, hipStream_t stream) {
    (void)hipGetLastError();
    if (!x || !wpatch || !y) return MTE_ERR_ARG;
    PatchArgs a{(const bf16_t*)x, ldx, (const bf16_t*)wpatch, bias, (bf16_t*)y, ldy, B, H, W, Cin_p, N, accumulate ? 1 : 0, nullptr, nullptr, 0, nullptr, 0, nullptr, 0};
    return launch_patch_plan(plan_patch(fwd_problem(PatchOp::Fwd, bias, ldx, B, H, W, Cin_p, N, KH, KW, accumulate), g_patch_knobs), a, stream);
}

long mte_conv2d_patch_fwd_gn_elems(int B, int H, int W) { return (long)B * (W / TW) * ((H + TH - 1) / TH) * 32; }
int mte_conv2d_patch_fwd_gn(const void* x, long ldx, const void* wpatch, const float* bias, void* y, long ldy, int B, int H, int W, int Cin_p, int N, int KH, int KW,
                            int accumulate, float* rec, long rec_elems, int* tiles_per_sample_out, hipStream_t stream) {
    (void)hipGetLastError();
    if (!x || !wpatch || !y || !rec || !tiles_per_sample_out) return MTE_ERR_ARG;
    const PatchPlan pl = plan_patch(fwd_problem(PatchOp::FwdGn, bias, ldx, B, H, W, Cin_p, N, KH, KW, accumulate), g_patch_knobs);
    if (pl.rc == MTE_OK && rec_elems < mte_conv2d_patch_fwd_gn_elems(B, H, W)) return MTE_ERR_ARG;
    PatchArgs a{(const bf16_t*)x, ldx, (const bf16_t*)wpatch, bias, (bf16_t*)y, ldy, B, H, W, Cin_p, N, accumulate ? 1 : 0, nullptr, nullptr, 0, nullptr, 0, nullptr, 0, rec};
    if (pl.rc == MTE_OK) *tiles_per_sample_out = pl.tiles_per_sample;
    return launch_patch_plan(pl, a, stream);
}

int mte_conv2d_patch_fwd_rank1_ok(const float* bias, long ldx, int B, int H, int W, int Cin_p, int N) {
    return plan_patch(fwd_problem(PatchOp::FwdRank1, bias, ldx, B, H, W, Cin_p, N, 3, 3), g_patch_knobs).rc == MTE_OK ? 1 : 0;
}
int mte_conv2d_patch_fwd_rank1(const void* x, long ldx, const void* wpatch, const float* bias, void* y, long ldy, int B, int H, int W, int Cin_p, int N,
                               const float* inv, const float* w1, long w1_stride, hipStream_t stream) {
    (void)hipGetLastError();
    if (!x || !wpatch || !y || !inv || !w1) return MTE_ERR_ARG;
    PatchArgs a{(const bf16_t*)x, ldx, (const bf16_t*)wpatch, bias, (bf16_t*)y, ldy, B, H, W, Cin_p, N, 0, inv, w1, w1_stride, nullptr, 0, nullptr, 0};
    return launch_patch_plan(plan_patch(fwd_problem(PatchOp::FwdRank1, bias, ldx, B, H, W, Cin_p, N, 3, 3), g_patch_knobs), a, stream);
}

int mte_conv2d_patch_fwd_plus1x1(const void* x, long ldx, const void* wpatch, const float* bias, void* y, long ldy, int B, int H, int W, int Cin_p, int N,
                                 const void* x2, long ldx2, const void* wpatch2, int C2, hipStream_t stream) {
    (void)hipGetLastError();
    if (!x || !wpatch || !y || !x2 || !wpatch2) return MTE_ERR_ARG;
    PatchArgs a{(const bf16_t*)x, ldx, (const bf16_t*)wpatch, bias, (bf16_t*)y, ldy, B, H, W, Cin_p, N, 0, nullptr, nullptr, 0, (const bf16_t*)x2, ldx2, (const bf16_t*)wpatch2, C2};
    return launch_patch_plan(plan_patch(fwd_problem(PatchOp::FwdPlus1x1, bias, ldx, B, H, W, Cin_p, N, 3, 3, 0, C2), g_patch_knobs), a, stream);
}
int mte_conv2d_patch_wgrad(const void* x, long ldx, const void* dy, long lddy, float* dw_stage, int stage_parts, int* parts_out,
                           int B, int H, int W, int Cin_p, int N, int KH, int KW, hipStream_t stream) {
    (void)hipGetLastError();
    if (!x || !dy || !dw_stage) return MTE_ERR_ARG;
    PatchWgradArgs a{(const bf16_t*)x, ldx, (const bf16_t*)dy, lddy, dw_stage, B, H, W, Cin_p, N, 1};
    const PatchPlan pl = plan_patch({PatchOp::Wgrad, B, H, W, Cin_p, N, KH, KW, ldx, false, true, 0, stage_parts, g_mte_wgrad_shared != 0}, g_patch_knobs);
    if (parts_out) *parts_out = pl.parts_out;
    return launch_patch_plan(pl, a, stream);
}

}
```

### mindtheedge_amd/csrc/conv_plan.hpp

```cpp
#pragma once

#ifndef MTE_OK
#define MTE_OK 0
#define MTE_ERR_ARG (-1)
#define MTE_ERR_LAUNCH (-2)
#define MTE_ERR_UNSUPPORTED (-3)
#endif

#ifndef MTE_IGEMM_MFMA16
#define MTE_IGEMM_MFMA16 1
#endif
#ifndef MTE_IGEMM8_DEFAULT
#define MTE_IGEMM8_DEFAULT 51
#endif

struct IgemmKnobs {
    int dma = 1;
    int pair_ksteps = 72;
    int ablate = 0;
    int ring6 = 0;
    int big_min_tiles = 224;
    int igemm8 = MTE_IGEMM8_DEFAULT;
    int n32_dma = 1;
    int igemm8_split_bn128 = 64;
    int igemm8_min_tiles = 200;
    int pp = 1;
    int big = 3;
    int igemm8_one = 1;
};
constexpr int MTE_KNOB_IGEMM_RESET = 33;

inline bool igemm_knob_set(IgemmKnobs& k, int key, int value) {
    switch (key) {
    case 0: k.dma = value; return true;
    case 6: k.big = value; return true;
    case 7: k.big_min_tiles = value; return true;
    case 15: k.ring6 = value; return true;
    case 17: k.ablate = value; return true;
    case 19: k.pair_ksteps = value; return true;
    case 21: k.pp = value; return true;
    case 23: k.igemm8 = value; return true;
    case 24: k.igemm8_min_tiles = value; return true;
    case 28: k.igemm8_one = value; return true;
    case 29: k.igemm8_split_bn128 = value; return true;
    case 32: k.n32_dma = value; return true;
    case MTE_KNOB_IGEMM_RESET: k = IgemmKnobs{}; return true;
    }
    return false;
}

struct IgemmProblem {
    int elem_size;
    long M;
    int N, Cin_p, KH, KW;
    long ldx;
    int out_f32;
    bool sparse;
    int unshuffle_c;
    int solo;
    bool has_ws; long ws_elems;
};

enum class IgemmForm {
    T128x32,
    T128x32_W2,
    T128x64,
    T128x128,
    T192x96,
    T256x128,
    T256x256_PP,
    T256x256_W16,
    P8_256x256, P8_256x128,
};
struct IgemmTile { int WM, WN, TM, TN; };
inline IgemmTile igemm_tile(IgemmForm f) {
    switch (f) {
    case IgemmForm::T128x32: return {4, 1, 1, 1};
    case IgemmForm::T128x32_W2: return {2, 1, 2, 1};
    case IgemmForm::T128x64: return {2, 2, 2, 1};
    case IgemmForm::T128x128: return {2, 2, 2, 2};
    case IgemmForm::T192x96: return {2, 3, 3, 1};
    case IgemmForm::T256x128: return {4, 2, 2, 2};
    case IgemmForm::T256x256_PP: return {2, 4, 4, 2};
    case IgemmForm::T256x256_W16: return {4, 4, 2, 2};
    default: return {0, 0, 0, 0};
    }
}

struct IgemmPlan {
    int rc = MTE_OK;
    int elem_size = 2;
    IgemmForm form = IgemmForm::T128x128;
    int loader = 0;
    int ring = 4, wpc = 1;
    int ablate = 0;
    int one = 0, kslice = 0;
    int splits = 1;
    unsigned grid = 0; int threads = 0, lds_bytes = 0;
    bool lds_optin = false;
    bool finish = false;
    unsigned finish_grid = 0;
};

inline int choose_splits(long tiles, int ksteps, long M, int N, long ws_elems, int nthr = 256) {
    const long want = 768L * 256 / nthr;
    if (tiles >= want / 2 || ws_elems < M * N || N % 4 != 0) return 1;
    long s = (want + tiles - 1) / tiles;
    const long max_s = ksteps / 16;
    if (s > max_s) s = max_s;
    if (s > ws_elems / (M * N)) s = ws_elems / (M * N);
    return (int)(s < 1 ? 1 : s);
}

inline bool igemm_dma_fits(const IgemmProblem& p, const IgemmKnobs& k) {
    const long es = p.elem_size;
    return k.dma == 1 && p.Cin_p % (int)(64 / es) == 0 && ((p.M - 1) * p.ldx + p.Cin_p) * es < 0x7ff00000L && (long)p.N * p.KH * p.KW * p.Cin_p * es < 0x7ff00000L;
}

namespace igemm_plan_detail {

inline void finish_after(IgemmPlan& pl, const IgemmProblem& p) {
    pl.finish = pl.splits > 1;
    long g = (p.M * p.N / 4 + 255) / 256; if (g > 4096) g = 4096;
    pl.finish_grid = (unsigned)g;
}

inline IgemmPlan plan_tile(IgemmForm form, long ws_elems, const IgemmProblem& p, const IgemmKnobs& k, bool dev_build) {
    IgemmPlan pl;
    pl.elem_size = p.elem_size; pl.form = form;
    const IgemmTile t = igemm_tile(form);
    const int BM = t.WM * t.TM * 32, BN = t.WN * t.TN * 32, NTHR = t.WM * t.WN * 64;
    const bool bf16 = p.elem_size == 2;
    const long tiles = ((p.M + BM - 1) / BM) * ((p.N + BN - 1) / BN);
    const int ksteps = (p.KH * p.KW * (p.Cin_p / (16 / p.elem_size)) + 3) / 4;
    pl.splits = (p.has_ws && !p.out_f32 && !p.sparse) ? choose_splits(tiles, ksteps, p.M, p.N, ws_elems, NTHR) : 1;
    pl.threads = NTHR;
    pl.grid = (unsigned)(tiles * pl.splits);
    finish_after(pl, p);
    const bool dma_stage = (BN * 4) % NTHR == 0;
    if (p.unshuffle_c && (pl.splits != 1 || p.out_f32 || p.sparse || !bf16 || BN % 32 != 0 || !dma_stage || !k.dma)) { pl.rc = MTE_ERR_UNSUPPORTED; return pl; }
    if (dma_stage && k.dma) {
        const bool fast = igemm_dma_fits(p, k);
        pl.loader = fast ? 2 : 1;
        pl.lds_bytes = 4 * (BM + BN) * 64;
        const bool square = (BM == 256 && BN == 128) || (BM == 128 && BN == 128) || (BM == 256 && BN == 256);
        if (dev_build && !MTE_IGEMM_MFMA16 && bf16 && square && fast && k.ablate) {
            pl.ablate = k.ablate >= 1 && k.ablate <= 6 ? k.ablate : 7;
            return pl;
        }
        if (bf16 && form == IgemmForm::T256x128 && fast) {
            const bool pair = p.solo || (ksteps <= k.pair_ksteps && tiles >= 512);
            if (k.ring6 == 3 || (k.ring6 == 0 && pair)) { pl.ring = 3; pl.wpc = 4; pl.lds_bytes = 3 * (BM + BN) * 64; pl.lds_optin = true; }
            else if (k.ring6 == 1) { pl.ring = 6; pl.lds_bytes = 6 * (BM + BN) * 64; pl.lds_optin = true; }
        }
        return pl;
    }
    if (NTHR != 256) { pl.rc = MTE_ERR_UNSUPPORTED; return pl; }
    pl.loader = 0;
    pl.lds_bytes = 2 * (BM + BN) * 64;
    return pl;
}

}

inline IgemmPlan plan_igemm(const IgemmProblem& p, const IgemmKnobs& k, bool dev_build) {
    using namespace igemm_plan_detail;
    using F = IgemmForm;
    if (p.elem_size != 2 && p.elem_size != 4) { IgemmPlan pl; pl.rc = MTE_ERR_UNSUPPORTED; return pl; }
    if (p.unshuffle_c && !(p.elem_size == 2 && k.dma == 1 && p.Cin_p % 32 == 0)) { IgemmPlan pl; pl.rc = MTE_ERR_UNSUPPORTED; return pl; }
    if (p.elem_size == 2) {
        const long tiles_big = ((p.M + 255) / 256) * ((p.N + 127) / 128);
        const bool dma_ok = igemm_dma_fits(p, k);
        const long n256 = (p.N + 255) / 256;
        const long t256 = ((p.M + 255) / 256) * n256;
        const bool wide = p.N > 128 && (p.N % 256 == 0 || p.N % 256 > 128);
        const int ksteps = p.KH * p.KW * (p.Cin_p / 32);
        const bool can_split = p.has_ws && p.ws_elems >= 2 * p.M * p.N && p.N % 4 == 0;
        long smax = can_split ? p.ws_elems / (p.M * p.N) : 1;
        if (smax > 8) smax = 8;
        const long reach256 = t256 * (can_split ? (ksteps / 16 < smax ? (ksteps / 16 > 0 ? ksteps / 16 : 1) : smax) : 1);
        if (k.igemm8 && dma_ok && !p.out_f32 && !p.sparse && p.N > 64 && !p.unshuffle_c) {
            const int nkt = (ksteps + 1) / 2;
            int bn = 0, splits = 1;
            if (k.igemm8 & 4) {
                if (wide && t256 >= k.igemm8_min_tiles) bn = 256;
                else if (tiles_big >= k.igemm8_min_tiles) bn = 128;
            } else if (wide && (k.igemm8 & 1) && t256 >= k.igemm8_min_tiles) {
                if (nkt >= (t256 <= 256 ? 18 : 36)) bn = 256;
            } else if ((k.igemm8 & 2) && tiles_big >= k.igemm8_min_tiles && tiles_big <= 256 && nkt >= 36) bn = 128;
            if (!bn && wide && (k.igemm8 & 1) && can_split && t256 < 128 && ksteps >= 32) {
                bn = 256;
                long tsp = t256;
                if (t256 <= k.igemm8_split_bn128 && ksteps <= 288) { bn = 128; tsp = tiles_big; }
                long sp = 256 / tsp;
                if (sp > smax) sp = smax;
                if (sp > ksteps / 16) sp = ksteps / 16;
                const int per = (int)((ksteps + sp - 1) / (sp < 1 ? 1 : sp));
                splits = (ksteps + per - 1) / per;
            }
            const int kslice = (!(k.igemm8 & 32) && p.Cin_p % 64 == 0) ? 1 : 0;
            if (bn && p.N % 8 == 0 && p.M < 0x7fffff00L && (!kslice || dev_build)) {
                IgemmPlan pl;
                pl.elem_size = 2; pl.form = bn == 256 ? F::P8_256x256 : F::P8_256x128;
                pl.loader = 2; pl.kslice = kslice; pl.splits = splits;
                pl.one = !kslice && k.igemm8_one && p.Cin_p % 64 == 0 && (splits == 1 || ((ksteps + splits - 1) / splits) % 2 == 0);
                pl.threads = 512;
                pl.lds_bytes = 2 * (4 * 128 * 64 + 4 * (bn / 2) * 64); pl.lds_optin = true;
                pl.grid = (unsigned)(((p.M + 255) / 256) * ((p.N + bn - 1) / bn) * splits);
                finish_after(pl, p);
                return pl;
            }
        }
        if (k.big >= 2 && dma_ok && !p.out_f32 && wide &&
            (t256 >= k.big_min_tiles || (can_split && t256 < 96 && reach256 >= 160))) {
            if (k.pp && t256 >= k.big_min_tiles) return plan_tile(F::T256x256_PP, 0, p, k, dev_build);
            return plan_tile(F::T256x256_W16, t256 >= k.big_min_tiles ? 0 : p.ws_elems, p, k, dev_build);
        }
        if (k.big >= 3 && dma_ok && !p.out_f32 && p.N > 64 && p.N <= 96 && ((p.M + 191) / 192) >= k.big_min_tiles)
            return plan_tile(F::T192x96, 0, p, k, dev_build);
        if (k.big && dma_ok && !p.out_f32 && p.N > 64 && tiles_big >= k.big_min_tiles)
            return plan_tile(F::T256x128, 0, p, k, dev_build);
        if (p.N <= 32 && k.n32_dma && dma_ok && !p.out_f32) return plan_tile(F::T128x32_W2, p.ws_elems, p, k, dev_build);
    }
    return plan_tile(p.N <= 32 ? F::T128x32 : p.N <= 64 ? F::T128x64 : F::T128x128, p.ws_elems, p, k, dev_build);
}
```

### mindtheedge_amd/kernels.py

```python
import ctypes
import itertools
import math
import os
import weakref

import torch

from ._lib import lib, MteError

DT_BF16, DT_F32 = 0, 1
_state = {"compute_dtype": torch.bfloat16, "weights_epoch": 0}


def set_compute_dtype(dtype):
    dtype = {"bf16": torch.bfloat16, "fp32": torch.float32, "f32": torch.float32}.get(dtype, dtype)
    assert dtype in (torch.bfloat16, torch.float32)
    _state["compute_dtype"] = dtype


def compute_dtype():
    return _state["compute_dtype"]


def bump_weights_epoch():
# ... 338 lines not shown
            self._pack(w, dtype, need_bwd)
            self.key = key
        else:
            self._sync_prefetch()
            if need_bwd and not self.has_bwd:
                cout, cin, kh, kw = w.shape
                cin_p = round8(cin)
                if self.wb is None:
                    self.wb = torch.empty((cin_p, kh * kw, cout), dtype=dtype, device=w.device)
                lib.mte_pack_conv_weights_bwd(self.wf.data_ptr(), self.wb.data_ptr(), cout, kh, kw, cin_p,
                                              DT_BF16 if dtype == torch.bfloat16 else DT_F32, _stream())
                self.has_bwd = True
        return self.wf, (self.wb if self.has_bwd else None)


class _PackJob(ctypes.Structure):
    _fields_ = [("w", ctypes.c_void_p), ("wf", ctypes.c_void_p), ("wb", ctypes.c_void_p), ("pf", ctypes.c_void_p), ("pb", ctypes.c_void_p),
                ("Cout", ctypes.c_int), ("Cin", ctypes.c_int), ("taps", ctypes.c_int), ("Cin_p", ctypes.c_int),
                ("end_f", ctypes.c_int), ("end_b", ctypes.c_int), ("end_pf", ctypes.c_int), ("end_pb", ctypes.c_int)]


_PACK_CHUNKS = (16, 48)
_pack_jobs = {"sig": None, "chunks": []}


def _pack_job_chunks(packs):
    sig = (len(packs),) + tuple((id(pk), pk._last[0]().data_ptr(), pk.wf.data_ptr(), _ptr(pk.wb) if pk.has_bwd else 0,
                                 _ptr(pk.pf) if pk._want_pf else 0, _ptr(pk.pb) if pk._want_pb else 0) for pk in packs)
    if _pack_jobs["sig"] == sig:
        return _pack_jobs["chunks"]
    chunks = []
    for dt in (torch.bfloat16, torch.float32):
        part = [pk for pk in packs if pk._last[1] == dt and pk.wf is not None and pk.wf.dtype == dt]
        i = 0
        while i < len(part):
            group = part[i:i + (_PACK_CHUNKS[0] if i == 0 else _PACK_CHUNKS[1])]
            i += len(group)
            arr = (_PackJob * len(group))()
            for o, pk in zip(arr, group):
                w = pk._last[0]()
                cout, cin, kh, kw = w.shape
                o.w, o.wf = w.data_ptr(), pk.wf.data_ptr()
                o.wb = pk.wb.data_ptr() if pk.has_bwd else None
                o.pf = pk.pf.data_ptr() if pk._want_pf else None
                o.pb = pk.pb.data_ptr() if pk._want_pb else None
                o.Cout, o.Cin, o.taps, o.Cin_p = cout, cin, kh * kw, round8(cin)
            chunks.append((arr, len(group), DT_BF16 if dt == torch.bfloat16 else DT_F32, group))
    _pack_jobs["sig"], _pack_jobs["chunks"] = sig, chunks
    return chunks


def prefetch_weight_packs():
    packs = []
    for r in WeightPack._live:
        pk = r()
        if pk is not None and pk._last is not None and pk.key is not None and pk._last[0]() is not None and pk._last[0]().is_cuda:
            packs.append(pk)
    WeightPack._live = [r for r in WeightPack._live if r() is not None]
    if not packs:
        return
    packs.sort(key=lambda pk: pk._order)
    if _side["enabled"]:
        if not _side["streams"]:
            _side["streams"] = [_new_side_stream() for _ in range(max(1, _SIDE_STREAMS))]
        side = _side["streams"][0]
        ev = torch.cuda.Event()
        ev.record()
        side.wait_event(ev)
    else:
        side = torch.cuda.current_stream()
    with torch.cuda.stream(side):
        _refold_all()
        _refresh_main_weights(packs)
        for pk in packs:
            pk._want_pf = pk.pf_ok and pk.pkey == pk.key and pk.pf is not None
            pk._want_pb = pk.pb_ok and pk.pkey == pk.key and pk.pb is not None and pk.has_bwd
        st = _stream()
        odd = [pk for pk in packs if not (pk._last[0]().is_contiguous() and pk._last[0]().dtype == torch.float32)]
        if odd:
            packs = [pk for pk in packs if pk not in odd]
            for pk in odd:
                w, dtype = pk._last[0](), pk._last[1]
                pk._pack(w, dtype, pk.has_bwd)
                pk.key = (w.data_ptr(), w._version, weights_epoch(), dtype, tuple(w.shape))
                pk.pkey, pk.pf_ok, pk.pb_ok, pk._event = None, False, False, None
        for arr, n, dtc, group in _pack_job_chunks(packs):
            lib.mte_pack_conv_weights_multi(ctypes.addressof(arr), n, dtc, st)
            ev = None
            if _side["enabled"]:
                ev = torch.cuda.Event()
                ev.record(side)
            for pk in group:
                w, dtype = pk._last[0](), pk._last[1]
                pk.key = (w.data_ptr(), w._version, weights_epoch(), dtype, tuple(w.shape))
                pk.pkey = pk.key
                pk.pf_ok, pk.pb_ok = pk._want_pf, pk._want_pb
                pk._event = ev
    if _side["enabled"] and torch.cuda.is_current_stream_capturing():
        torch.cuda.current_stream().wait_stream(side)
        for pk in packs:
            pk._event = None


SPLITK_SLABS = 8
_splitk_ws = {}


def _splitk_workspace(M, N, device):
    tiles = ((M + 127) // 128) * ((N + 127) // 128)
    if tiles >= 384:
        return None, 0
    n = SPLITK_SLABS * M * N
    if torch.cuda.is_current_stream_capturing():
        return torch.empty((n,), dtype=torch.float32, device=device), n
    key = (str(device), _stream())
    ws = _splitk_ws.get(key)
    if ws is None or ws.numel() < n:
        ws = _splitk_ws[key] = torch.empty((n,), dtype=torch.float32, device=device)
    return ws, n


_cfg = {"patch_kernels": True, "pack_folding": True, "pack_fold_max_overhead": 0.30,
        "no_fork_accumulate": bool(os.environ.get("MTE_NO_FORK_ACCUM")),
        "patch_wgrad_slabs": not os.environ.get("MTE_PATCH_WGRAD_ATOMICS"),
        "split_inv_channel": os.environ.get("MTE_SPLIT_INV", "1") == "1",
        "fuse_inv_term": os.environ.get("MTE_FUSE_INV", "1") == "1",
        "fold_shortcut_dgrad": os.environ.get("MTE_FOLD_SHORTCUT", "1") == "1",
        "fuse_residual_tail": os.environ.get("MTE_FUSE_TAIL", "1") == "1",
        "gn_stats_in_conv": os.environ.get("MTE_GN_IN_CONV", "1") == "1"}



def use_pack_folding(flag):
    _cfg["pack_folding"] = bool(flag)


def pack_folding_enabled():
    return _cfg["pack_folding"]


def use_patch_kernels(flag):
    _cfg["patch_kernels"] = bool(flag)


def _stem_ok(W, cin_p, n, kh, kw, dtype):
    return (_cfg["patch_kernels"] and cin_p == 8 and dtype == torch.bfloat16
            and lib.mte_conv2d_stem_supported(W, cin_p, n, kh, kw, DT_BF16) == 1)


def _patch_ok(W, cin_p, n, kh, kw, dtype):
    return _cfg["patch_kernels"] and dtype == torch.bfloat16 and lib.mte_conv2d_patch_supported(W, cin_p, n, kh, kw, DT_BF16) == 1


class SiteList:

    def __init__(self, mask):
        _require_gpu(mask)
        if mask.dtype != torch.uint8 or not mask.is_contiguous():
            raise MteError("site list: expected a contiguous uint8 mask [B,H,W]")
        n = mask.numel()
        self.rows = torch.empty((n,), dtype=torch.int32, device=mask.device)
        self.count = torch.empty((1,), dtype=torch.int32, device=mask.device)
        ws = torch.empty((int(lib.mte_sparse_site_list_workspace_elems(n)),), dtype=torch.int32, device=mask.device)
        lib.mte_sparse_site_list(mask.data_ptr(), n, self.rows.data_ptr(), self.count.data_ptr(), ws.data_ptr(), _stream())
        self.shape = tuple(mask.shape)


def conv_forward(x, wf, bias, cout, kh, kw, out=None, pack=None, w=None, accumulate=False, sites=None, gn_records=None):
    B, Cp, H, W = x.shape
    if out is None:
        out = new_act(B, cout, H, W, x.dtype, x.device)
        if sites is not None:
            out.zero_()
    xp, ldx = _pl(x)
    yp, ldy = _pl(out)
    if sites is not None:
        if sites.shape != (B, H, W):
            raise MteError("site list of a %s mask used on a %s map" % (sites.shape, (B, H, W)))
        lib.mte_conv2d_igemm_sparse(xp, ldx, wf.data_ptr(), _ptr(bias), yp, ldy, B, H, W, Cp, cout, kh, kw, _dt(x),
                                    sites.rows.data_ptr(), sites.count.data_ptr(), 1 if accumulate else 0, _stream())
        return out
    if not accumulate and _stem_ok(W, Cp, cout, kh, kw, x.dtype):
        lib.mte_conv2d_stem_fwd(xp, ldx, wf.data_ptr(), _ptr(bias), yp, ldy, B, H, W, cout, kh, kw, _stream())
        return out
    if pack is not None and _patch_ok(W, Cp, cout, kh, kw, x.dtype):
        if (gn_records is not None and _cfg["gn_stats_in_conv"] and cout % 16 == 0
                and lib.mte_gn_fwd_is_single_pass_b(B, H * W, cout, 0, _dt(x)) != 1):
            n = int(lib.mte_conv2d_patch_fwd_gn_elems(B, H, W))
            rec = torch.empty((n,), dtype=torch.float32, device=x.device)
            tiles = ctypes.c_int(0)
            lib.mte_conv2d_patch_fwd_gn(xp, ldx, pack.get_patch(w, 'f').data_ptr(), _ptr(bias), yp, ldy, B, H, W, Cp, cout, kh, kw,
                                        1 if accumulate else 0, rec.data_ptr(), n, ctypes.byref(tiles), _stream())
            gn_records.append((rec, tiles.value))
            return out
        lib.mte_conv2d_patch_fwd(xp, ldx, pack.get_patch(w, 'f').data_ptr(), _ptr(bias), yp, ldy, B, H, W, Cp, cout, kh, kw,
                                 1 if accumulate else 0, _stream())
        return out
    ws, ws_n = _splitk_workspace(B * H * W, cout, x.device)
    lib.mte_conv2d_igemm(xp, ldx, wf.data_ptr(), _ptr(bias), yp, ldy, 0, B, H, W, Cp, cout, kh, kw, _dt(x), _ptr(ws), ws_n,
                         (1 if accumulate else 0) | _CONV_SOLO, _stream())
    return out


_CONV_SOLO = 2


_side = {"enabled": True, "streams": [], "next": 0, "keep": [], "keep_bytes": 0, "callback_queued": False, "dirty": False}
lib.set_option(3, 1, lazy=True)
def _new_side_stream():
    pr = int(os.environ.get("MTE_SIDE_PRIORITY", "1"))
    if pr == 0:
        return torch.cuda.Stream()
    hip = ctypes.CDLL("libamdhip64.so")
    h = ctypes.c_void_p()
    if hip.hipStreamCreateWithPriority(ctypes.byref(h), 1, pr) != 0:
        raise RuntimeError("hipStreamCreateWithPriority(%d) failed" % pr)
    return torch.cuda.ExternalStream(h.value)


_SIDE_STREAMS = 1
_SIDE_KEEP_LIMIT = 24 << 30


def use_wgrad_side_stream(flag):
    _side["enabled"] = bool(flag)
    lib.set_option(3, 1 if flag else 0, lazy=True)


def join_side_stream():
    if _side["dirty"]:
        for st in _side["streams"]:
            ev = torch.cuda.Event()
            ev.record(st)
            torch.cuda.current_stream().wait_event(ev)
        _side["dirty"] = False
    _side["keep"].clear()
    _side["keep_bytes"] = 0


def side_streams_wait_into(stream):
    if _side["dirty"]:
        for st in _side["streams"]:
            ev = torch.cuda.Event()
            ev.record(st)
            stream.wait_event(ev)


def _side_join_callback():
    _side["callback_queued"] = False
    join_side_stream()


def _side_stream_for(*tensors):
    if not _side["streams"]:
        _side["streams"] = [_new_side_stream() for _ in range(max(1, _SIDE_STREAMS))]
    side = _side["streams"][_side["next"] % len(_side["streams"])]
    _side["next"] += 1
    ev = torch.cuda.Event()
    ev.record()
    side.wait_event(ev)
    _side["keep"].append(tensors)
    _side["keep_bytes"] += sum(t.numel() * t.element_size() for t in tensors)
    _side["dirty"] = True
    if not _side["callback_queued"]:
        try:
            torch.autograd.Variable._execution_engine.queue_callback(_side_join_callback)
            _side["callback_queued"] = True
        except RuntimeError:
            pass
    return side


def _conv_wgrad(x, dy, w, need_dbias, dw_out, dbias_out):
    cout, cin, kh, kw = w.shape
    B, Cp, H, W = x.shape
    dyp, lddy = _pl(dy)
    xp, ldx = _pl(x)
    st = _stream()
    dbias = None
    per = cout * kh * kw * Cp
    patch = _cfg["patch_kernels"] and x.dtype == torch.bfloat16 and lib.mte_conv2d_patch_wgrad_supported(W, Cp, cout, kh, kw, DT_BF16) == 1
    if patch and lib.mte_conv2d_wgrad_nine_tap(H, W, Cp, cout, kh, kw, _dt(x)) == 1:
        patch = False
    if kh * kw == 1 and Cp >= 64:
        patch = False
    wide = 256 if per <= (1 << 18) else (64 if per <= (1 << 19) else 32)
    cap = max(1, min(512, (192 << 20) // (4 * per))) if patch and _cfg["patch_wgrad_slabs"] else max(1, min(wide, (96 << 20) // (4 * per)))
    stem = _stem_ok(W, Cp, cout, kh, kw, x.dtype)
    if stem:
        cap = 2048
    stage = torch.empty((cap + (32 if cap > 32 else 0), cout, kh * kw, Cp), dtype=torch.float32, device=x.device)
    parts = ctypes.c_int(1)
    if stem:
        lib.mte_conv2d_stem_wgrad(xp, ldx, dyp, lddy, stage.data_ptr(), cap, ctypes.byref(parts), B, H, W, cout, kh, kw, st)
    elif patch:
        lib.mte_conv2d_patch_wgrad(xp, ldx, dyp, lddy, stage.data_ptr(), cap, ctypes.byref(parts), B, H, W, Cp, cout, kh, kw, st)
    else:
        lib.mte_conv2d_wgrad(xp, ldx, dyp, lddy, stage.data_ptr(), cap, ctypes.byref(parts), B, H, W, Cp, cout, kh, kw, _dt(x), st)
    dw = dw_out if dw_out is not None else torch.empty_like(w, dtype=torch.float32)
    lib.mte_unpack_conv_wgrad(stage.data_ptr(), parts.value, dw.data_ptr(), cout, cin, kh, kw, Cp, st)
    if need_dbias:
        dbias = dbias_out if dbias_out is not None else torch.empty((cout,), dtype=torch.float32, device=x.device)
        lib.mte_colsum(dyp, lddy, B * H * W, cout, dbias.data_ptr(), _dt(dy), st)
    return dw, dbias


def conv_backward(x, dy, w, pack, need_dx, need_dw=True, need_dbias=True, dw_out=None, dbias_out=None, fork_slot=None, sunk=False, sites=None):
    dw = dbias = dx = None
    on_side = False
    if need_dw:
        sunk = bool(sunk) and dw_out is not None and (dbias_out is not None or not need_dbias)
        on_side = sunk and _side["enabled"] and need_dx

    def wgrad():
        if on_side:
            if _side["keep_bytes"] > _SIDE_KEEP_LIMIT:
                join_side_stream()
            with torch.cuda.stream(_side_stream_for(x, dy)):
                return _conv_wgrad(x, dy, w, need_dbias, dw_out, dbias_out)
        return _conv_wgrad(x, dy, w, need_dbias, dw_out, dbias_out)

    if need_dw:
        dw, dbias = wgrad()
    if need_dx:
        dx = _conv_dgrad(x, dy, w, pack, fork_slot, sites)
    return dx, dw, dbias


def _conv_dgrad(x, dy, w, pack, fork_slot, sites):
    cout, cin, kh, kw = w.shape
    B, Cp, H, W = x.shape
    dyp, lddy = _pl(dy)
    st = _stream()
    target = _fork_target(fork_slot, (B, Cp, H, W), x.dtype, keep_pending=True)
    if (target is None and fork_slot is not None and (kh, kw) == (1, 1) and sites is None and _cfg["fold_shortcut_dgrad"]
            and not _cfg.get("no_fork_accumulate") and _patch_ok(W, cout, Cp, 1, 1, x.dtype) and _patch_ok(W, 32, Cp, 3, 3, x.dtype)):
        dx = new_act(B, Cp, H, W, x.dtype, x.device)
        fork_slot["buf"] = dx
        fork_slot["pending"] = (dy, w, pack)
        return dx
    pend = _pending_slot(fork_slot) if target is not None else None
    if pend is not None:
        dy3, w3, pack3 = pend["pending"]
        if ((kh, kw) == (3, 3) and sites is None and target is pend["buf"] and _patch_ok(W, cout, Cp, 3, 3, x.dtype)
                and tuple(dy3.shape[2:]) == (H, W) and dy3.dtype == x.dtype):
            del pend["pending"]
            d3p, ldd3 = _pl(dy3)
            dxp, lddx = _pl(target)
            lib.mte_conv2d_patch_fwd_plus1x1(dyp, lddy, pack.get_patch(w, 'b').data_ptr(), 0, dxp, lddx, B, H, W, cout, Cp,
                                             d3p, ldd3, pack3.get_patch(w3, 'b').data_ptr(), dy3.shape[1], st)
            fork_slot["buf"] = target
            return target
        _flush_pending(pend)
    dx = target if target is not None else new_act(B, Cp, H, W, x.dtype, x.device)
    if target is None and sites is not None:
        dx.zero_()
    acc = 1 if target is not None else 0
    dxp, lddx = _pl(dx)
    if sites is not None:
        _, wb = pack.get(w, x.dtype, True)
        lib.mte_conv2d_igemm_sparse(dyp, lddy, wb.data_ptr(), 0, dxp, lddx, B, H, W, cout, Cp, kh, kw, _dt(x),
                                    sites.rows.data_ptr(), sites.count.data_ptr(), acc, st)
    elif _patch_ok(W, cout, Cp, kh, kw, x.dtype):
        lib.mte_conv2d_patch_fwd(dyp, lddy, pack.get_patch(w, 'b').data_ptr(), 0, dxp, lddx, B, H, W, cout, Cp, kh, kw, acc, st)
    else:
        _, wb = pack.get(w, x.dtype, True)
        ws, ws_n = _splitk_workspace(B * H * W, Cp, x.device)
        lib.mte_conv2d_igemm(dyp, lddy, wb.data_ptr(), 0, dxp, lddx, 0, B, H, W, cout, Cp, kh, kw, _dt(x), _ptr(ws), ws_n, acc, st)
    if fork_slot is not None:
        fork_slot["buf"] = dx
    return dx


_stats_elems = {}


def gn_stats_buffer(B, device):
    n = _stats_elems.get(B)
    if n is None:
        n = _stats_elems[B] = int(lib.mte_gn_stats_elems(B))
    return _zeros((n,), torch.float64, device)


def _gn_forward(y1, y2, scale2, gamma, beta, eps, out=None, records=None):
    B, C, H, W = y1.shape
    p1, l1 = _pl(y1)
    p2, l2 = _pl(y2) if y2 is not None else (0, 0)
    st = _stream()
    ready = 1
    stats = gn_stats_buffer(B, y1.device)
    if lib.mte_gn_fwd_is_single_pass_b(B, H * W, C, 1 if y2 is not None else 0, _dt(y1)) == 1:
        ready = 0
    elif records and y2 is None:
        lib.mte_gn_stats_from_records(records[0][0].data_ptr(), records[0][1], stats.data_ptr(), B, st)
    else:
        lib.mte_gn_stats(p1, l1, p2, l2, _ptr(scale2), stats.data_ptr(), B, H * W, C, _dt(y1), st)
    z = out if out is not None else new_act(B, C, H, W, y1.dtype, y1.device)
    if tuple(z.shape) != (B, C, H, W) or z.dtype != y1.dtype:
        raise MteError("output destination has shape %s / %s, expected %s / %s" % (tuple(z.shape), z.dtype, (B, C, H, W), y1.dtype))
    zp, lz = _pl(z)
    lib.mte_gn_elu_fwd(p1, l1, p2, l2, _ptr(scale2), stats.data_ptr(), ready, gamma.data_ptr(), beta.data_ptr(), zp, lz,
                       B, H * W, C, eps, _dt(y1), st)
    return z, stats


def _gn_backward(dz, y1, y2, scale2, stats, gamma, beta, eps, need_d2, want_dbias=False, dgamma=None, dbeta=None, dbias=None):
    B, C, H, W = y1.shape
    dz = as_act(dz, y1.dtype)
    red = _zeros((B, C, 2), torch.float32, y1.device)
    d1 = new_act(B, C, H, W, y1.dtype, y1.device)
    d2 = new_act(B, C, H, W, y1.dtype, y1.device) if need_d2 else None
    dgamma = dgamma if dgamma is not None else _zeros((C,), torch.float32, y1.device)
    dbeta = dbeta if dbeta is not None else _zeros((C,), torch.float32, y1.device)
    if want_dbias and dbias is None:
        dbias = _zeros((C,), torch.float32, y1.device)
    pz, lz = _pl(dz)
    p1, l1 = _pl(y1)
    p2, l2 = _pl(y2) if y2 is not None else (0, 0)
    pd1, ld1 = _pl(d1)
    pd2, ld2 = _pl(d2) if d2 is not None else (0, 0)
    lib.mte_gn_elu_bwd(pz, lz, p1, l1, p2, l2, _ptr(scale2), stats.data_ptr(), gamma.data_ptr(), beta.data_ptr(), red.data_ptr(),
                       pd1, ld1, pd2, ld2, dgamma.data_ptr(), dbeta.data_ptr(), _ptr(dbias), B, H * W, C, eps, _dt(y1), _stream())
    if want_dbias:
        return d1, d2, dgamma, dbeta, dbias
    return d1, d2, dgamma, dbeta


GN_EPS = 1e-5

_dropout_pool = {}


def dropout2d_scale(B, C, p, device):
    key = (str(device), float(p))
    pool = _dropout_pool.get(key)
    n = B * C
    if pool is None or pool[1] + n > pool[0].numel():
        size = max(1 << 17, 2 * n)
        pool = _dropout_pool[key] = [(torch.rand((size,), device=device) >= p).float() / (1.0 - p), 0]
    out = pool[0][pool[1]:pool[1] + n].view(B, C)
    pool[1] += n
    return out



class ConvGnEluFn(torch.autograd.Function):

    @staticmethod
    def forward(ctx, x, w, b, gamma, beta, pack, out=None):
        ctx.fork_slot = getattr(x, "_mte_fork_slot", None)
        wf, _ = pack.get(w, x.dtype, bool(ctx.needs_input_grad[0]))
        cout, cin, kh, kw = w.shape
        recs = []
        y = conv_forward(x, wf, b, cout, kh, kw, pack=pack, w=w, gn_records=recs)
        z, stats = _gn_forward(y, None, None, gamma, beta, GN_EPS, out=None if out is None else alias_of(out), records=recs)
        ctx.save_for_backward(x, w, y, stats, gamma, beta)
        ctx.pack = pack
        ctx.bias = b
        return z

    @staticmethod
    def backward(ctx, dz):
        x, w, y, stats, gamma, beta = ctx.saved_tensors
        b = ctx.bias
        gg, sg = _grad_dst(gamma, zero=True)
        gb, sb = _grad_dst(beta, zero=True)
        gbias, sbias = _grad_dst(b, zero=True)
        gw, sw = _grad_dst(w)
        dy, _, dgamma, dbeta, db = _gn_backward(dz, y, None, None, stats, gamma, beta, GN_EPS, False, want_dbias=True,
                                                dgamma=gg, dbeta=gb, dbias=gbias)
        dx, dw, _ = conv_backward(x, dy, w, ctx.pack, ctx.needs_input_grad[0], need_dbias=False, dw_out=gw, fork_slot=ctx.fork_slot, sunk=sw)
        return dx, _grad_ret(w, dw, sw), _grad_ret(b, db, sbias), _grad_ret(gamma, dgamma, sg), _grad_ret(beta, dbeta, sb), None, None


def _main_weight(pack, w, cm):
    key = (w.data_ptr(), w._version, weights_epoch())
    wm = getattr(pack, "_main_w", None)
    if wm is None or tuple(wm.shape) != (w.shape[0], cm, w.shape[2], w.shape[3]) or wm.device != w.device:
        wm = pack._main_w = torch.empty((w.shape[0], cm, w.shape[2], w.shape[3]), dtype=torch.float32, device=w.device)
        pack._main_key = None
    pack._main_src = (weakref.ref(w), cm)
    if pack._main_key != key:
        wm.copy_(w.detach()[:, :cm])
        pack._main_key = key
    return wm


def _refresh_main_weights(packs):
    for pk in packs:
        src = getattr(pk, "_main_src", None)
        wm = getattr(pk, "_main_w", None)
        if src is None or wm is None:
            continue
        w = src[0]()
        if w is None or tuple(wm.shape) != (w.shape[0], src[1], w.shape[2], w.shape[3]):
            continue
        key = (w.data_ptr(), w._version, weights_epoch())
        if pk._main_key != key:
            wm.copy_(w.detach()[:, :src[1]])
            pk._main_key = key


class ConvGnEluInvFn(torch.autograd.Function):

    @staticmethod
    def forward(ctx, x, inv, w, b, gamma, beta, pack, out=None):
# ... 467 lines not shown
        pad, N = k // 2, 2 * (k // 2) * co
        dt, dev = _dt(x), x.device
        w3c, b3c = w3.detach().contiguous().float(), b3.detach().contiguous().float()
        P = new_act(B, 4 * C, H2, W2, x.dtype, dev)
        xp, ldx = _pl(x)
        pp, ldp = _pl(P)
        lib.mte_pixel_shuffle(xp, ldx, pp, ldp, B, H, W, C, 0, dt, _stream())
        Wf, bf = _folded_weights(pack_fold, w, w3, b, b3, co, C, k, dev)
        f = pack_fold.fold
        wfp, _ = pack_fold.get(Wf, x.dtype, False)
        y = conv_forward(P, wfp, bf, co, k + 2, k + 2, pack=pack_fold, w=Wf)
        Rr = new_act(2 * B, 16 * C, 1, W2 + 2, x.dtype, dev)
        Rc = new_act(2 * B, 16 * C, H2, 1, x.dtype, dev)
        lib.mte_pack_ring_fwd(pp, ldp, w3c.data_ptr(), Rr.data_ptr(), Rc.data_ptr(), B, H2, W2, 4 * C, dt, _stream())
        wr, _ = f["pk_r"].get(f["Wr"], x.dtype, False)
        wc, _ = f["pk_c"].get(f["Wc"], x.dtype, False)
        yp, ldy = _pl(y)
        ws, splits = _ring_terms_grouped(Rr, Rc, wr, wc, B, H2, W2, 16 * C, co, k, dt)
        if ws is not None:
            lib.mte_pack_border_apply_slabs(yp, ldy, ws.data_ptr(), splits, f["Dt"].data_ptr(), B, H2, W2, co, k, dt, _stream())
        else:
            cr = _ring_gemm(Rr, wr, N, 1, k, True, _CONV_SOLO)
            cc = _ring_gemm(Rc, wc, N, k, 1, True, _CONV_SOLO)
            lib.mte_pack_border_apply(yp, ldy, cr.data_ptr(), cc.data_ptr(), f["Dt"].data_ptr(), B, H2, W2, co, k, dt, _stream())
        z, stats = _gn_forward(y, None, None, gamma, beta, GN_EPS, out=None if out is None else alias_of(out))
        ctx.save_for_backward(P, Rr, Rc, y, stats, w, w3c, b3c, gamma, beta, Wf)
        ctx.params = (w3, b3, b)
        ctx.packs = (pack_unf, pack_fold)
        ctx.geom = (B, C, H, W, co, k)
        return z

    @staticmethod
    def backward(ctx, dz):
        P, Rr, Rc, y, stats, w, w3c, b3c, gamma, beta, Wf = ctx.saved_tensors
        w3, b3, b = ctx.params
        pack_unf, pack_fold = ctx.packs
        B, C, H, W, co, k = ctx.geom
        H2, W2, pad, N = H // 2, W // 2, k // 2, 2 * (k // 2) * co
        dt, dev = _dt(P), P.device
        f = pack_fold.fold
        gg, sg = _grad_dst(gamma, zero=True)
        gbt, sbt = _grad_dst(beta, zero=True)
        dy, _, dgamma, dbeta = _gn_backward(dz, y, None, None, stats, gamma, beta, GN_EPS, False, dgamma=gg, dbeta=gbt)
        dyp, lddy = _pl(dy)
        pp, ldp = _pl(P)
        Gr = new_act(2 * B, N, 1, W2 + 2, P.dtype, dev)
        Gc = new_act(2 * B, N, H2, 1, P.dtype, dev)
        lib.mte_pack_border_gather(dyp, lddy, Gr.data_ptr(), Gc.data_ptr(), B, H2, W2, co, k, dt, _stream())
        _, wrb = f["pk_r"].get(f["Wr"], P.dtype, True)
        _, wcb = f["pk_c"].get(f["Wc"], P.dtype, True)
        dRr = _ring_gemm(Gr, wrb, 16 * C, 1, k, False)
        dRc = _ring_gemm(Gc, wcb, 16 * C, k, 1, False)

        def weight_grads():
            sw = _stream()
            dst3 = _claim_adjacent(w3, b3)
            dk3b = dst3 if dst3 is not None else torch.zeros((112,), dtype=torch.float32, device=dev)
            gw_dst, gw_sunk = _grad_dst(w)
            gb_dst, gb_sunk = _grad_dst(b)
            part = torch.empty((int(lib.mte_pack_border_class_sums_elems(co, k)),), dtype=torch.float32, device=dev)
            lib.mte_pack_border_class_sums(dyp, lddy, part.data_ptr(), B, H2, W2, co, k, dt, sw)
            dWr = _ring_wgrad(Rr, Gr, f["Wr"])
            dWc = _ring_wgrad(Rc, Gc, f["Wc"])
            work = torch.empty((int(lib.mte_pack_border_scatter_work_elems(co, k)) + int(lib.mte_pack_ring_work_elems()),), dtype=torch.float32, device=dev)
            lib.mte_pack_border_scatter(dWr.data_ptr(), dWc.data_ptr(), part.data_ptr(), w.detach().data_ptr(), b3c.data_ptr(), gw_dst.data_ptr(),
                                        dk3b.data_ptr(), work.data_ptr(), co, 4 * C, k, sw)
            lib.mte_pack_ring_bwd_weight(dRr.data_ptr(), dRc.data_ptr(), pp, ldp, dk3b.data_ptr(),
                                         work.data_ptr() + 4 * int(lib.mte_pack_border_scatter_work_elems(co, k)), B, H2, W2, 4 * C, dt, sw)
            dWf, db = _conv_wgrad(P, dy, Wf, True, None, gb_dst)
            lib.mte_unfold_pack_wgrad(dWf.data_ptr(), db.data_ptr(), w.detach().data_ptr(), w3c.data_ptr(), b3c.data_ptr(),
                                      gw_dst.data_ptr(), dk3b.data_ptr(), co, 4 * C, k, 1, sw)
            if dst3 is not None:
                _announce(w3, b3)
                g3 = gb3 = None
            else:
                g3, gb3 = _deliver_pair(w3, b3, dk3b, 108)
            return (g3, gb3, _grad_ret(w, gw_dst, gw_sunk), _grad_ret(b, db, gb_sunk))

        if _side["enabled"] and _all_sunk(w3, b3, w, b):
            with torch.cuda.stream(_side_stream_for(P, dy, Rr, Rc, Gr, Gc, dRr, dRc, Wf)):
                g3, gb3, gw, gb = weight_grads()
        else:
            g3, gb3, gw, gb = weight_grads()
        dx = new_act(B, C, H, W, P.dtype, dev)
        dxp, lddx = _pl(dx)
        if not _dgrad_unshuffled(dy, Wf, pack_fold, dx, k + 2):
            dP, _, _ = conv_backward(P, dy, Wf, pack_fold, True, need_dw=False)
            sp, lds_ = _pl(dP)
            lib.mte_pixel_shuffle(sp, lds_, dxp, lddx, B, H, W, C, 1, dt, _stream())
        lib.mte_pack_ring_bwd_data(dRr.data_ptr(), dRc.data_ptr(), w3c.data_ptr(), dxp, lddx, B, H2, W2, 4 * C, dt, _stream())
        return (dx, g3, gb3, gw, gb, _grad_ret(gamma, dgamma, sg), _grad_ret(beta, dbeta, sbt), None, None, None)


class InvDepthFn(torch.autograd.Function):

    @staticmethod
    def forward(ctx, x, w, b, min_depth):
        B, C, H, W = x.shape
        out = torch.empty((B, 1, H, W), dtype=torch.float32, device=x.device)
        xp, ldx = _pl(x)
        wc = w.detach().contiguous().float()
        lib.mte_invdepth_fwd(xp, ldx, wc.data_ptr(), b.detach().float().data_ptr(), out.data_ptr(), B, H, W, C, min_depth, _dt(x), _stream())
        ctx.save_for_backward(x, wc, out)
        ctx.min_depth = min_depth
        ctx.params = (w, b)
        return out

    @staticmethod
    def backward(ctx, dout):
        x, wc, out = ctx.saved_tensors
        w, b = ctx.params
        B, C, H, W = x.shape
        dout = dout.contiguous().float()
        dx = new_act(B, C, H, W, x.dtype, x.device)
        dlogit = torch.empty((B, H, W), dtype=torch.float32, device=x.device)
        dxp, lddx = _pl(dx)
        lib.mte_invdepth_bwd_data(wc.data_ptr(), out.data_ptr(), dout.data_ptr(), dlogit.data_ptr(), dxp, lddx,
                                  B, H, W, C, ctx.min_depth, _dt(x), _stream())

        def weight_grads():
            xp, ldx = _pl(x)
            dst = _claim_adjacent(w, b) if tuple(w.shape) == (1, C, 3, 3) and b.numel() == 1 else None
            dwb = dst if dst is not None else torch.empty((C * 9 + 1,), dtype=torch.float32, device=x.device)
            rec = torch.empty((int(lib.mte_invdepth_bwd_weight_workspace_elems(C)),), dtype=torch.float32, device=x.device)
            lib.mte_invdepth_bwd_weight(xp, ldx, dlogit.data_ptr(), dwb.data_ptr(), rec.data_ptr(), B, H, W, C, _dt(x), _stream())
            if dst is not None:
                _announce(w, b)
                return None, None
            return _deliver_pair(w, b, dwb, C * 9)

        if _side["enabled"] and _all_sunk(w, b):
            with torch.cuda.stream(_side_stream_for(x, dlogit)):
                dw, db = weight_grads()
        else:
            dw, db = weight_grads()
        return dx, dw, db, None


def _pending_slot(slot):
    while slot is not None:
        if slot["buf"] is not None:
            return slot if "pending" in slot else None
        slot = slot["parent"]
    return None


def _flush_pending(slot):
    dy3, w3, pack3 = slot.pop("pending")
    dx = slot["buf"]
    B, Cp, H, W = dx.shape
    cout = w3.shape[0]
    d3p, ldd3 = _pl(dy3)
    dxp, lddx = _pl(dx)
    lib.mte_conv2d_patch_fwd(d3p, ldd3, pack3.get_patch(w3, 'b').data_ptr(), 0, dxp, lddx, B, H, W, cout, Cp, 1, 1, 0, _stream())


def _fork_target(slot, shape, dtype, keep_pending=False):
    if _cfg.get("no_fork_accumulate"):
        return None
    while slot is not None:
        buf = slot["buf"]
        if buf is not None:
            if "pending" in slot and not keep_pending:
                _flush_pending(slot)
            return buf if (tuple(buf.shape) == tuple(shape) and buf.dtype == dtype and is_act(buf)) else None
        slot = slot["parent"]
    return None


class ForkFn(torch.autograd.Function):

    @staticmethod
    def forward(ctx, x, slot):
        ctx.slot = slot
        return alias_of(x), alias_of(x)

    @staticmethod
    def backward(ctx, g1, g2):
        slot = ctx.slot
        if "pending" in slot:
            _flush_pending(slot)
        if g1 is None or g2 is None:
            out = g1 if g2 is None else g2
        elif g1.data_ptr() == g2.data_ptr() and g1.shape == g2.shape and g1.stride() == g2.stride():
            out = g1
        else:
            dt = g1.dtype if g1.dtype == g2.dtype else compute_dtype()
            g1, g2 = as_act(g1, dt), as_act(g2, dt)
            B, C, H, W = g1.shape
            out = new_act(B, C, H, W, dt, g1.device)
            p1, l1 = _pl(g1)
            p2, l2 = _pl(g2)
            po, lo = _pl(out)
            lib.mte_add_channels(p1, l1, p2, l2, po, lo, B * H * W, C, _dt(out), _stream())
        slot["buf"] = None
        return out, None


def fork(x):
    if not (torch.is_grad_enabled() and x.requires_grad):
        return x, x
    slot = {"buf": None, "parent": getattr(x, "_mte_fork_slot", None)}
    a, b = ForkFn.apply(x, slot)
    a._mte_fork_slot = slot
    b._mte_fork_slot = slot
    return a, b


class ConcatFn(torch.autograd.Function):

    @staticmethod
    def forward(ctx, inv, buf, *parts):
        B, _, H, W = parts[0].shape
        dtype = parts[0].dtype
        chans = [p.shape[1] for p in parts]
        ctot = sum(chans) + (8 if inv is not None else 0)
        if buf is None:
            buf = new_act(B, ctot, H, W, dtype, parts[0].device)
        else:
            if tuple(buf.shape) != (B, ctot, H, W) or buf.dtype != dtype:
                raise MteError("concat buffer has shape %s, expected %s" % (tuple(buf.shape), (B, ctot, H, W)))
            buf = alias_of(buf)
        st = _stream()
        off = 0
        for p, c in zip(parts, chans):
            dst = buf[:, off:off + c]
            off += c
            if p.dtype == dtype and p.data_ptr() == dst.data_ptr() and p.stride() == dst.stride():
                continue
            p = as_act(p, dtype)
            sp, lds_ = _pl(p)
            dp, ldd = _pl(dst)
            lib.mte_copy_channels(sp, lds_, dp, ldd, B * H * W, c, _dt(p), st)
        if inv is not None:
            dst = buf[:, off:off + 8]
            dp, ldd = _pl(dst)
            lib.mte_upsample_inv_fwd(inv.contiguous().data_ptr(), dp, ldd, B, H // 2, W // 2, _dt(buf), st)
        ctx.chans = chans
        ctx.has_inv = inv is not None
        ctx.slots = [getattr(p, "_mte_fork_slot", None) for p in parts]
        return buf

    @staticmethod
    def backward(ctx, dbuf):
        dbuf = as_act(dbuf)
        B, _, H, W = dbuf.shape
        outs = []
        off = 0
        for c, slot in zip(ctx.chans, ctx.slots):
            g = dbuf[:, off:off + c]
            if slot is not None and slot["buf"] is None and _fork_target(slot["parent"], g.shape, g.dtype) is None:
                slot["buf"] = g
            outs.append(g)
            off += c
        dinv = None
        if ctx.has_inv:
            dinv = torch.empty((B, 1, H // 2, W // 2), dtype=torch.float32, device=dbuf.device)
            src = dbuf[:, off:off + 8]
            sp, lds_ = _pl(src)
            lib.mte_upsample_inv_bwd(sp, lds_, dinv.data_ptr(), B, H // 2, W // 2, 0, _dt(dbuf), _stream())
        return (dinv, None) + tuple(outs)


def new_concat_buffer(B, chans, with_inv, H, W, dtype=None, device="cuda"):
    c = sum(chans) + (8 if with_inv else 0)
    ld = (c + 31) // 32 * 32
    if ld == c or os.environ.get("MTE_CONCAT_TIGHT"):
        return new_act(B, c, H, W, dtype or compute_dtype(), device)
    return alias_of(new_act(B, ld, H, W, dtype or compute_dtype(), device)[:, :c])


def image_to_act(rgb, flip=False, dtype=None):
    _require_gpu(rgb)
    B, C, H, W = rgb.shape
    rgb = rgb.contiguous().float()
    out = new_act(B, round8(C), H, W, dtype or compute_dtype(), rgb.device)
    op, ldo = _pl(out)
    lib.mte_nchw_to_nhwc(rgb.data_ptr(), op, ldo, B, C, H, W, round8(C), 1 if flip else 0, _dt(out), _stream())
    return out




from .kernels_loss import EdgeLossFn, EdgeLossKindFn, BilinearResizeFn, DepthLossesFn, DepthLossesPairFn, SilogFn, SupervisedLossFn, NearestUpsampleFn, _EdgeScale, adam_step_flat, adamw_step_flat, sgd_step_flat, grad_norm_work, grad_norm_clip_flat, grad_accumulate_flat, ema_update_flat, flat_swap
```

Before: 383.8 images/sec.

## Fold shortcut 1x1 dgrad into 3x3 igemm as extra K source

Extends the implicit-GEMM conv kernels (both the tile kernel and the 256-row igemm8 kernel) so they can take a second K source. That source is the 1x1 shortcut's dy and weights, appended after the last 3x3 tap. This lets the shortcut-plus-3x3 dgrad fold also run at shapes where the patch kernel is unsupported, saving a separate 1x1 conv pass and its output read-modify-write. The planner rejects the fused route when the standalone conv would have used split-K, and the fallback flush now handles non-patch shapes via igemm. It adds template instances and per-step branching in the loaders, which may cost registers or occupancy.

```diff
diff --git a/include/mte_kernels.h b/include/mte_kernels.h
--- a/include/mte_kernels.h
+++ b/include/mte_kernels.h
@@ -137,6 +137,7 @@
 int mte_conv2d_patch_fwd_rank1_ok(const float* bias, long ldx, int B, int H, int W, int Cin_p, int N);
 int mte_conv2d_patch_fwd_rank1(const void* x, long ldx, const void* wpatch, const float* bias, void* y, long ldy, int B, int H, int W, int Cin_p, int N,
                                const float* inv, const float* w1, long w1_stride, mte_stream_t stream);
+int mte_conv2d_plus1x1_supported(int B, int H, int W, int Cin_p, int N, int C2);
 int mte_conv2d_patch_fwd_plus1x1(const void* x, long ldx, const void* wpatch, const float* bias, void* y, long ldy, int B, int H, int W, int Cin_p, int N,
                                  const void* x2, long ldx2, const void* wpatch2, int C2, mte_stream_t stream);
 long mte_rank1_conv_bwd_records_elems(int N);
diff --git a/mindtheedge_amd/_lib.py b/mindtheedge_amd/_lib.py
--- a/mindtheedge_amd/_lib.py
+++ b/mindtheedge_amd/_lib.py
@@ -22,7 +22,7 @@
            "mte_chamfer_workspace_bytes", "mte_edge_match_workspace_bytes", "mte_edge_loss_sums_elems", "mte_gn_fwd_is_single_pass", "mte_gn_fwd_is_single_pass_b",
            "mte_edge_loss_work_elems", "mte_edge_loss_pair_work_elems", "mte_edge_loss_kind_work_elems", "mte_supervised_loss_work_elems", "mte_rank1_conv_bwd_records_elems", "mte_conv2d_patch_fwd_rank1_ok", "mte_gn_stats_elems", "mte_device_error_poll", "mte_invdepth_bwd_weight_workspace_elems", "mte_sparse_site_list_workspace_elems", "mte_image_resample_work_bytes", "mte_lidar_perturb_work_bytes", "mte_order_stats_work_bytes",
            "mte_pack_ring_work_elems", "mte_pack_border_scatter_work_elems", "mte_pack_border_class_sums_elems", "mte_grad_norm_work_bytes",
-           "mte_pack_border_gemm_ws_elems", "mte_tensor_stats_work_bytes", "mte_lamb_work_bytes")
+           "mte_pack_border_gemm_ws_elems", "mte_tensor_stats_work_bytes", "mte_lamb_work_bytes", "mte_conv2d_plus1x1_supported")
 
 
 def parse_header(path=HEADER, dev=False):
diff --git a/mindtheedge_amd/csrc/conv_args.hpp b/mindtheedge_amd/csrc/conv_args.hpp
--- a/mindtheedge_amd/csrc/conv_args.hpp
+++ b/mindtheedge_amd/csrc/conv_args.hpp
@@ -16,9 +16,13 @@
     const int* rows; const int* nrows;
     int kslice;
     int unshuffle_c;
+    const void* x2; long ldx2; const void* w2; int C2;
 };
 
 __attribute__((visibility("hidden"))) int igemm8_launch(const IgemmPlan& p, const ConvArgs& a, hipStream_t st);
 
+__attribute__((visibility("hidden"))) IgemmPlan igemm_plus1x1_plan(long M, int N, int Cin_p, int KH, int KW, long ldx, int C2);
+__attribute__((visibility("hidden"))) int igemm_plus1x1_launch(const ConvArgs& a, hipStream_t st);
+
 __attribute__((visibility("hidden"))) int wgrad9_launch(const WgradPlan& pl, const void* x, long ldx, const void* dy, long ldy, float* dw_stage,
                                                         int B, int H, int W, int Cin_p, int N, hipStream_t st);
diff --git a/mindtheedge_amd/csrc/conv_igemm.hip b/mindtheedge_amd/csrc/conv_igemm.hip
--- a/mindtheedge_amd/csrc/conv_igemm.hip
+++ b/mindtheedge_amd/csrc/conv_igemm.hip
@@ -48,8 +48,12 @@
 
 __device__ u32x4_t g_zero16 = {0u, 0u, 0u, 0u};
 
-template <typename T, int WM, int WN, int TM, int TN, int LD, int RING = 4, int MINW = 1, int ABL = 0>
+constexpr int IGEMM_X2 = 8;
+template <typename T, int WM, int WN, int TM, int TN, int LD, int RING = 4, int MINW = 1, int ABL_ = 0>
 __global__ __launch_bounds__(WM * WN * 64, MINW) void conv_igemm_kernel(ConvArgs a) {
+    constexpr bool X2 = ABL_ == IGEMM_X2;
+    constexpr int ABL = X2 ? 0 : ABL_;
+    static_assert(!X2 || (LD == 2 && sizeof(T) == 2), "the second K source exists on the bf16 buffer-descriptor loader only");
     constexpr bool DMA = LD != 0;
     constexpr int NTHR = WM * WN * 64;
     constexpr int BM = WM * TM * 32, BN = WN * TN * 32;
@@ -78,9 +82,10 @@
     const int cpt = a.Cin_p / PER16;
     const int total_chunks = taps * cpt;
     const int ksteps_all = (total_chunks + 3) >> 2;
-    const int per_split = (ksteps_all + a.splits - 1) / a.splits;
+    const int ksteps_x = X2 ? ksteps_all + (a.C2 >> 5) : ksteps_all;
+    const int per_split = (ksteps_x + a.splits - 1) / a.splits;
     const int s_begin = split * per_split;
-    const int s_end = min(ksteps_all, s_begin + per_split);
+    const int s_end = min(ksteps_x, s_begin + per_split);
     const long Kp = (long)taps * a.Cin_p;
     const T* __restrict__ xp = (const T*)a.x;
     const T* __restrict__ wp = (const T*)a.w;
@@ -157,6 +162,9 @@
     constexpr int ES = (int)sizeof(T);
     unsigned voffA[A_CH], voffT[A_CH], voffB[B_CH];
     int f_ty = 0, f_tx = 0, f_cb = 0;
+    unsigned voffA2[X2 ? A_CH : 1], voffB2[X2 ? B_CH : 1];
+    int f_cpt = cpt;
+    bool f_x2 = false;
     auto set_tap = [&]() {
         const int dy = f_ty - pad_h, dx = f_tx - pad_w;
         const int delta = (dy * a.W + dx) * (int)a.ldx * ES;
@@ -178,13 +186,47 @@
         const int q0 = 4 * s_begin, tap0 = q0 / cpt;
         f_cb = q0 - tap0 * cpt; f_ty = tap0 / a.KW; f_tx = tap0 - f_ty * a.KW;
         set_tap();
+        if constexpr (X2) {
+#pragma unroll
+            for (int i = 0; i < A_CH; ++i) voffA2[i] = a_ok[i] ? (unsigned)((a_pix[i] * a.ldx2 + kc * PER16) * ES) : OOB;
+#pragma unroll
+            for (int i = 0; i < B_CH; ++i) {
+                const int n = n0 + ((tid + i * NTHR) >> 2);
+                voffB2[i] = n < a.N ? (unsigned)(((long)n * a.C2 + kc * PER16) * ES) : OOB;
+            }
+        }
     }
     auto dma_fast = [&](int s, int slot) {
 #if defined(__HIP_DEVICE_COMPILE__)
         typedef __attribute__((address_space(3))) void* lptr_t;
+        const int wv = __builtin_amdgcn_readfirstlane(wave);
+        if constexpr (X2) {
+            if (f_cb == f_cpt && !f_x2) {
+                f_cb = 0;
+                if (f_ty == a.KH - 1 && f_tx == a.KW - 1) {
+                    f_x2 = true; f_cpt = a.C2 / PER16;
+#pragma unroll
+                    for (int i = 0; i < A_CH; ++i) voffT[i] = voffA2[i];
+                } else {
+                    if (++f_tx == a.KW) { f_tx = 0; ++f_ty; }
+                    set_tap();
+                }
+            }
+            const auto rsA = __builtin_amdgcn_make_buffer_rsrc(f_x2 ? (void*)a.x2 : (void*)xp, 0,
+                                                               f_x2 ? (int)(((a.M - 1) * a.ldx2 + a.C2) * ES) : (int)(((a.M - 1) * a.ldx + a.Cin_p) * ES), 0x00020000);
+            const auto rsB = __builtin_amdgcn_make_buffer_rsrc(f_x2 ? (void*)a.w2 : (void*)wp, 0, f_x2 ? (int)((long)a.N * a.C2 * ES) : (int)((long)a.N * Kp * ES), 0x00020000);
+            const int soffA = f_cb * PER16 * ES, soffB = (f_x2 ? s - ksteps_all : s) * 64;
+#pragma unroll
+            for (int i = 0; i < A_CH; ++i)
+                __builtin_amdgcn_raw_ptr_buffer_load_lds(rsA, (lptr_t)(sA + slot * BM * 64 + (wv * 16 + i * (NTHR / 4)) * 64), 16, voffT[i], soffA, 0, 0);
+#pragma unroll
+            for (int i = 0; i < B_CH; ++i)
+                __builtin_amdgcn_raw_ptr_buffer_load_lds(rsB, (lptr_t)(sB + slot * BN * 64 + (wv * 16 + i * (NTHR / 4)) * 64), 16, f_x2 ? voffB2[i] : voffB[i], soffB, 0, 0);
+            f_cb += 4;
+            return;
+        }
         const auto rsA = __builtin_amdgcn_make_buffer_rsrc((void*)xp, 0, (int)(((a.M - 1) * a.ldx + a.Cin_p) * ES), 0x00020000);
         const auto rsB = __builtin_amdgcn_make_buffer_rsrc((void*)wp, 0, (int)((long)a.N * Kp * ES), 0x00020000);
-        const int wv = __builtin_amdgcn_readfirstlane(wave);
         if (f_cb == cpt) {
             f_cb = 0;
             if (++f_tx == a.KW) { f_tx = 0; ++f_ty; }
@@ -617,6 +659,9 @@
     case igemm_instance(FORM, sizeof(T), __VA_ARGS__): rc = launch_instance<conv_igemm_kernel<T, WM, WN, TM, TN, __VA_ARGS__>>(p, a, st); break
     if (p.form == F::P8_256x256 || p.form == F::P8_256x128) rc = igemm8_launch(p, a, st);
     else if (p.ablate) rc = launch_ablated(p, a, st);
+    else if (a.C2) {
+        if (p.form == F::T256x128 && p.elem_size == 2 && p.loader == 2 && p.ring == 3) rc = launch_instance<conv_igemm_kernel<bf16_t, 4, 2, 2, 2, 2, 3, 4, IGEMM_X2>>(p, a, st);
+    }
     else switch (igemm_instance(p.form, p.elem_size, p.loader, p.ring)) {
     MTE_IGEMM_CASE(F::T128x32, bf16_t, 4, 1, 1, 1, 0);
     MTE_IGEMM_CASE(F::T128x32_W2, bf16_t, 2, 1, 2, 1, 2);
@@ -665,6 +710,18 @@
     return launch_plan(plan_igemm(p, g_igemm_knobs, kDevBuild), a, st);
 }
 
+}
+
+IgemmPlan igemm_plus1x1_plan(long M, int N, int Cin_p, int KH, int KW, long ldx, int C2) {
+    return plan_igemm_plus1x1(M, N, Cin_p, KH, KW, ldx, C2, g_igemm_knobs, kDevBuild);
+}
+int igemm_plus1x1_launch(const ConvArgs& a, hipStream_t st) {
+    if (a.C2 <= 0 || ((a.M - 1) * a.ldx2 + a.C2) * 2 >= 0x7ff00000L) return MTE_ERR_UNSUPPORTED;
+    return launch_plan(igemm_plus1x1_plan(a.M, a.N, a.Cin_p, a.KH, a.KW, a.ldx, a.C2), a, st);
+}
+
+namespace {
+
 struct WgradArgs {
     const void* x; long ldx;
     const void* dy; long ldy;
diff --git a/mindtheedge_amd/csrc/conv_igemm8.hip b/mindtheedge_amd/csrc/conv_igemm8.hip
--- a/mindtheedge_amd/csrc/conv_igemm8.hip
+++ b/mindtheedge_amd/csrc/conv_igemm8.hip
@@ -18,9 +18,10 @@
     return __builtin_amdgcn_mfma_f32_16x16x32_bf16(__builtin_bit_cast(bf16x8_t, a), __builtin_bit_cast(bf16x8_t, b), c, 0, 0, 0);
 }
 
-template <int BN, bool SM = false, bool ONE = false>
-__global__ __launch_bounds__(512, 2) void conv_igemm8_kernel(ConvArgs a) {
+template <int BN, bool SM, bool ONE, bool X2>
+__device__ __forceinline__ void conv_igemm8_tile(const ConvArgs a) {
     static_assert(!(SM && ONE), "the slice-major order has its own single tap state");
+    static_assert(!X2 || ONE, "the second K source rides the one-tap-state form");
     typedef bf16_t T;
     constexpr int BM = 256, HM = 128, HN = BN / 2;
     constexpr int WN = BN == 256 ? 4 : 2;
@@ -48,7 +49,7 @@
     const int cpt = a.Cin_p >> 3;
     const int ksteps_all = (taps * cpt) >> 2;
     constexpr bool sm = SM;
-    const int units_all = sm ? ksteps_all >> 1 : ksteps_all;
+    const int units_all = sm ? ksteps_all >> 1 : (X2 ? ksteps_all + (a.C2 >> 5) : ksteps_all);
     const int per_split = (units_all + a.splits - 1) / a.splits;
     const int s_begin = split * per_split;
     const int s_end = min(units_all, s_begin + per_split);
@@ -79,6 +80,18 @@
     }
     int st_s[2], st_ty[2], st_tx[2], st_cb[2];
     bool st_live[2];
+    unsigned voffA2[X2 ? 2 : 1], voffB2[X2 ? 2 : 1];
+    int a_cpt = cpt;
+    bool a_x2 = false;
+    if constexpr (X2) {
+#pragma unroll
+        for (int h = 0; h < 2; ++h) {
+            const long m = m0 + h * HM + lrow;
+            voffA2[h] = a_ok[h] ? (unsigned)((m * a.ldx2 + kc * 8) * 2) : OOB8;
+            const int n = n0 + h * HN + brow;
+            voffB2[h] = n < a.N ? (unsigned)(((long)n * a.C2 + kc * 8) * 2) : OOB8;
+        }
+    }
     int a_t = s_begin, a_slice = 0;
     unsigned voffT[2][2];
     auto set_tap = [&](int kh) {
@@ -132,6 +145,19 @@
         if constexpr (ONE) {
             st_s[0] += 2; st_cb[0] += 8;
             st_live[0] = st_s[0] < s_end;
+            if constexpr (X2) {
+                if (st_cb[0] >= a_cpt && !a_x2) {
+                    st_cb[0] = 0;
+                    if (st_ty[0] == a.KH - 1 && st_tx[0] == a.KW - 1) {
+                        a_x2 = true; a_cpt = a.C2 >> 3;
+                        voffT[0][0] = voffA2[0]; voffT[0][1] = voffA2[1];
+                    } else {
+                        if (++st_tx[0] == a.KW) { st_tx[0] = 0; ++st_ty[0]; }
+                        set_tap(0);
+                    }
+                }
+                return;
+            }
             if (st_cb[0] >= cpt) {
                 st_cb[0] = 0;
                 if (++st_tx[0] == a.KW) { st_tx[0] = 0; ++st_ty[0]; }
@@ -162,12 +188,17 @@
     typedef __attribute__((address_space(3))) void* lptr_t;
     const auto rsA = __builtin_amdgcn_make_buffer_rsrc((void*)xp, 0, (int)(((a.M - 1) * a.ldx + a.Cin_p) * 2), 0x00020000);
     const auto rsB = __builtin_amdgcn_make_buffer_rsrc((void*)wp, 0, (int)((long)a.N * Kp * 2), 0x00020000);
+    const auto rsA2 = __builtin_amdgcn_make_buffer_rsrc((void*)a.x2, 0, X2 ? (int)(((a.M - 1) * a.ldx2 + a.C2) * 2) : 0, 0x00020000);
+    const auto rsB2 = __builtin_amdgcn_make_buffer_rsrc((void*)a.w2, 0, X2 ? (int)((long)a.N * a.C2 * 2) : 0, 0x00020000);
 #endif
     auto stageA = [&](int h, int buf) {
 #if defined(__HIP_DEVICE_COMPILE__)
 #pragma unroll
         for (int kh = 0; kh < 2; ++kh) {
-            if constexpr (ONE) {
+            if constexpr (X2) {
+                const unsigned vo = st_live[0] ? voffT[0][h] : OOB8;
+                __builtin_amdgcn_raw_ptr_buffer_load_lds(a_x2 ? rsA2 : rsA, (lptr_t)(smem + buf * BUF + (h * 2 + kh) * (HM * 64) + wv * 1024), 16, vo, (st_cb[0] + 4 * kh) * 16, 0, 0);
+            } else if constexpr (ONE) {
                 const unsigned vo = st_live[0] ? voffT[0][h] : OOB8;
                 __builtin_amdgcn_raw_ptr_buffer_load_lds(rsA, (lptr_t)(smem + buf * BUF + (h * 2 + kh) * (HM * 64) + wv * 1024), 16, vo, (st_cb[0] + 4 * kh) * 16, 0, 0);
             } else {
@@ -179,6 +210,20 @@
     };
     auto stageB = [&](int h, int buf) {
 #if defined(__HIP_DEVICE_COMPILE__)
+        if constexpr (X2) {
+            const bool b2 = b_sp0 >= ksteps_all;
+            const unsigned vo = b_t < s_end ? (b2 ? voffB2[h] : voffB[h]) : OOB8;
+            const int sp = b2 ? b_sp0 - ksteps_all : b_sp0;
+            if constexpr (BN == 256) {
+#pragma unroll
+                for (int kh = 0; kh < 2; ++kh)
+                    __builtin_amdgcn_raw_ptr_buffer_load_lds(b2 ? rsB2 : rsB, (lptr_t)(smem + buf * BUF + A_BYTES + (h * 2 + kh) * (HN * 64) + wv * 1024), 16, vo, (sp + kh) * 64, 0, 0);
+            } else {
+                const int kh = wv >> 2;
+                __builtin_amdgcn_raw_ptr_buffer_load_lds(b2 ? rsB2 : rsB, (lptr_t)(smem + buf * BUF + A_BYTES + (h * 2 + kh) * (HN * 64) + (wv & 3) * 1024), 16, vo, (sp + kh) * 64, 0, 0);
+            }
+            return;
+        }
         if constexpr (BN == 256) {
 #pragma unroll
             for (int kh = 0; kh < 2; ++kh) {
@@ -378,6 +423,11 @@
     }
 }
 
+template <int BN, bool SM = false, bool ONE = false>
+__global__ __launch_bounds__(512, 2) void conv_igemm8_kernel(ConvArgs a) { conv_igemm8_tile<BN, SM, ONE, false>(a); }
+template <int BN>
+__global__ __launch_bounds__(512, 2) void conv_igemm8_x2_kernel(ConvArgs a) { conv_igemm8_tile<BN, false, true, true>(a); }
+
 
 template <auto Kernel> int launch8(const IgemmPlan& p, const ConvArgs& a, hipStream_t st) {
     if (mte_allow_lds<Kernel>(p.lds_bytes) != MTE_OK) return MTE_ERR_LAUNCH;
@@ -396,6 +446,10 @@
         return MTE_ERR_UNSUPPORTED;
 #endif
     }
+    if (a.C2) {
+        if (!p.one || p.splits != 1) return MTE_ERR_UNSUPPORTED;
+        return wide ? launch8<conv_igemm8_x2_kernel<256>>(p, a, st) : launch8<conv_igemm8_x2_kernel<128>>(p, a, st);
+    }
     if (p.one) return wide ? launch8<conv_igemm8_kernel<256, false, true>>(p, a, st) : launch8<conv_igemm8_kernel<128, false, true>>(p, a, st);
     return wide ? launch8<conv_igemm8_kernel<256, false>>(p, a, st) : launch8<conv_igemm8_kernel<128, false>>(p, a, st);
 }
diff --git a/mindtheedge_amd/csrc/conv_patch.hip b/mindtheedge_amd/csrc/conv_patch.hip
--- a/mindtheedge_amd/csrc/conv_patch.hip
+++ b/mindtheedge_amd/csrc/conv_patch.hip
@@ -1,5 +1,6 @@
 #include "common.hpp"
 #include "patch_plan.hpp"
+#include "conv_args.hpp"
 #include <type_traits>
 
 #ifdef MTE_STAMPS
@@ -1089,12 +1090,23 @@
     return launch_patch_plan(plan_patch(fwd_problem(PatchOp::FwdRank1, bias, ldx, B, H, W, Cin_p, N, 3, 3), g_patch_knobs), a, stream);
 }
 
+int mte_conv2d_plus1x1_supported(int B, int H, int W, int Cin_p, int N, int C2) {
+    if (B <= 0 || H <= 0 || W <= 0 || Cin_p <= 0 || N <= 0 || C2 <= 0) return 0;
+    if (plan_patch(fwd_problem(PatchOp::FwdPlus1x1, nullptr, Cin_p, B, H, W, Cin_p, N, 3, 3, 0, C2), g_patch_knobs).rc == MTE_OK) return 1;
+    if (Cin_p % 8 != 0) return 0;
+    return igemm_plus1x1_plan((long)B * H * W, N, Cin_p, 3, 3, Cin_p, C2).rc == MTE_OK ? 2 : 0;
+}
 int mte_conv2d_patch_fwd_plus1x1(const void* x, long ldx, const void* wpatch, const float* bias, void* y, long ldy, int B, int H, int W, int Cin_p, int N,
                                  const void* x2, long ldx2, const void* wpatch2, int C2, hipStream_t stream) {
     (void)hipGetLastError();
     if (!x || !wpatch || !y || !x2 || !wpatch2) return MTE_ERR_ARG;
+    const PatchPlan pl = plan_patch(fwd_problem(PatchOp::FwdPlus1x1, bias, ldx, B, H, W, Cin_p, N, 3, 3, 0, C2), g_patch_knobs);
+    if (pl.rc != MTE_OK && B > 0 && H > 0 && W > 0 && N > 0 && C2 > 0 && Cin_p > 0 && Cin_p % 8 == 0 && ldx % 8 == 0 && ldx2 % 8 == 0) {
+        ConvArgs g{x, ldx, wpatch, bias, y, ldy, 0, B, H, W, Cin_p, N, 3, 3, (long)B * H * W, 1, nullptr, 0, 0, nullptr, nullptr, 0, 0, x2, ldx2, wpatch2, C2};
+        if (igemm_plus1x1_plan(g.M, N, Cin_p, 3, 3, ldx, C2).rc == MTE_OK) return igemm_plus1x1_launch(g, stream);
+    }
     PatchArgs a{(const bf16_t*)x, ldx, (const bf16_t*)wpatch, bias, (bf16_t*)y, ldy, B, H, W, Cin_p, N, 0, nullptr, nullptr, 0, (const bf16_t*)x2, ldx2, (const bf16_t*)wpatch2, C2};
-    return launch_patch_plan(plan_patch(fwd_problem(PatchOp::FwdPlus1x1, bias, ldx, B, H, W, Cin_p, N, 3, 3, 0, C2), g_patch_knobs), a, stream);
+    return launch_patch_plan(pl, a, stream);
 }
 int mte_conv2d_patch_wgrad(const void* x, long ldx, const void* dy, long lddy, float* dw_stage, int stage_parts, int* parts_out,
                            int B, int H, int W, int Cin_p, int N, int KH, int KW, hipStream_t stream) {
diff --git a/mindtheedge_amd/csrc/conv_plan.hpp b/mindtheedge_amd/csrc/conv_plan.hpp
--- a/mindtheedge_amd/csrc/conv_plan.hpp
+++ b/mindtheedge_amd/csrc/conv_plan.hpp
@@ -59,6 +59,7 @@
     int unshuffle_c;
     int solo;
     bool has_ws; long ws_elems;
+    int extra_c = 0;
 };
 
 enum class IgemmForm {
@@ -96,6 +97,7 @@
     int ablate = 0;
     int one = 0, kslice = 0;
     int splits = 1;
+    int ksteps = 0;
     unsigned grid = 0; int threads = 0, lds_bytes = 0;
     bool lds_optin = false;
     bool finish = false;
@@ -132,9 +134,9 @@
     const int BM = t.WM * t.TM * 32, BN = t.WN * t.TN * 32, NTHR = t.WM * t.WN * 64;
     const bool bf16 = p.elem_size == 2;
     const long tiles = ((p.M + BM - 1) / BM) * ((p.N + BN - 1) / BN);
-    const int ksteps = (p.KH * p.KW * (p.Cin_p / (16 / p.elem_size)) + 3) / 4;
+    const int ksteps = (p.KH * p.KW * (p.Cin_p / (16 / p.elem_size)) + 3) / 4 + p.extra_c / 32;
     pl.splits = (p.has_ws && !p.out_f32 && !p.sparse) ? choose_splits(tiles, ksteps, p.M, p.N, ws_elems, NTHR) : 1;
-    pl.threads = NTHR;
+    pl.threads = NTHR; pl.ksteps = ksteps;
     pl.grid = (unsigned)(tiles * pl.splits);
     finish_after(pl, p);
     const bool dma_stage = (BN * 4) % NTHR == 0;
@@ -163,7 +165,7 @@
 
 }
 
-inline IgemmPlan plan_igemm(const IgemmProblem& p, const IgemmKnobs& k, bool dev_build) {
+inline IgemmPlan plan_igemm_form(const IgemmProblem& p, const IgemmKnobs& k, bool dev_build) {
     using namespace igemm_plan_detail;
     using F = IgemmForm;
     if (p.elem_size != 2 && p.elem_size != 4) { IgemmPlan pl; pl.rc = MTE_ERR_UNSUPPORTED; return pl; }
@@ -174,7 +176,7 @@
         const long n256 = (p.N + 255) / 256;
         const long t256 = ((p.M + 255) / 256) * n256;
         const bool wide = p.N > 128 && (p.N % 256 == 0 || p.N % 256 > 128);
-        const int ksteps = p.KH * p.KW * (p.Cin_p / 32);
+        const int ksteps = p.KH * p.KW * (p.Cin_p / 32) + p.extra_c / 32;
         const bool can_split = p.has_ws && p.ws_elems >= 2 * p.M * p.N && p.N % 4 == 0;
         long smax = can_split ? p.ws_elems / (p.M * p.N) : 1;
         if (smax > 8) smax = 8;
@@ -204,7 +206,7 @@
                 pl.elem_size = 2; pl.form = bn == 256 ? F::P8_256x256 : F::P8_256x128;
                 pl.loader = 2; pl.kslice = kslice; pl.splits = splits;
                 pl.one = !kslice && k.igemm8_one && p.Cin_p % 64 == 0 && (splits == 1 || ((ksteps + splits - 1) / splits) % 2 == 0);
-                pl.threads = 512;
+                pl.threads = 512; pl.ksteps = ksteps;
                 pl.lds_bytes = 2 * (4 * 128 * 64 + 4 * (bn / 2) * 64); pl.lds_optin = true;
                 pl.grid = (unsigned)(((p.M + 255) / 256) * ((p.N + bn - 1) / bn) * splits);
                 finish_after(pl, p);
@@ -224,3 +226,29 @@
     }
     return plan_tile(p.N <= 32 ? F::T128x32 : p.N <= 64 ? F::T128x64 : F::T128x128, p.ws_elems, p, k, dev_build);
 }
+
+inline bool igemm_extra_fits(const IgemmPlan& pl, const IgemmProblem& p) {
+    if (pl.rc != MTE_OK || pl.elem_size != 2 || pl.splits != 1 || pl.ablate) return false;
+    if (pl.form == IgemmForm::P8_256x256 || pl.form == IgemmForm::P8_256x128) return pl.one && !pl.kslice && p.extra_c % 64 == 0;
+    if (pl.form == IgemmForm::T256x128) return pl.loader == 2 && pl.ring == 3 && p.extra_c % 32 == 0;
+    return false;
+}
+
+inline IgemmPlan plan_igemm(const IgemmProblem& p, const IgemmKnobs& k, bool dev_build) {
+    if (p.extra_c == 0) return plan_igemm_form(p, k, dev_build);
+    IgemmPlan pl;
+    pl.rc = MTE_ERR_UNSUPPORTED;
+    if (p.extra_c < 0 || p.extra_c % 32 != 0 || p.elem_size != 2 || p.sparse || p.unshuffle_c || p.out_f32) return pl;
+    const IgemmPlan form = plan_igemm_form(p, k, dev_build);
+    return igemm_extra_fits(form, p) ? form : pl;
+}
+
+inline IgemmPlan plan_igemm_plus1x1(long M, int N, int Cin_p, int KH, int KW, long ldx, int C2, const IgemmKnobs& k, bool dev_build) {
+    const IgemmProblem fused{2, M, N, Cin_p, KH, KW, ldx, 0, false, 0, 0, false, 0, C2};
+    IgemmPlan pl = plan_igemm(fused, k, dev_build);
+    if (pl.rc != MTE_OK) return pl;
+    const bool offered = ((M + 127) / 128) * ((N + 127) / 128) < 384;
+    const IgemmProblem alone{2, M, N, Cin_p, KH, KW, ldx, 0, false, 0, 0, offered, offered ? 8 * M * N : 0};
+    if (plan_igemm(alone, k, dev_build).splits > 1) pl.rc = MTE_ERR_UNSUPPORTED;
+    return pl;
+}
diff --git a/mindtheedge_amd/kernels.py b/mindtheedge_amd/kernels.py
--- a/mindtheedge_amd/kernels.py
+++ b/mindtheedge_amd/kernels.py
@@ -514,6 +514,18 @@
     return _cfg["patch_kernels"] and dtype == torch.bfloat16 and lib.mte_conv2d_patch_supported(W, cin_p, n, kh, kw, DT_BF16) == 1
 
 
+def _plus1x1_route(B, H, W, cin_p, n, c2, dtype):
+    if dtype != torch.bfloat16:
+        return 0
+    route = int(lib.mte_conv2d_plus1x1_supported(B, H, W, cin_p, n, c2))
+    if route == 1 and not _cfg["patch_kernels"]:
+        return 0
+    return route
+
+
+_dgrad_counts = {"folded": 0, "standalone_1x1": 0}
+
+
 class SiteList:
 
     def __init__(self, mask):
@@ -696,7 +708,7 @@
     st = _stream()
     target = _fork_target(fork_slot, (B, Cp, H, W), x.dtype, keep_pending=True)
     if (target is None and fork_slot is not None and (kh, kw) == (1, 1) and sites is None and _cfg["fold_shortcut_dgrad"]
-            and not _cfg.get("no_fork_accumulate") and _patch_ok(W, cout, Cp, 1, 1, x.dtype) and _patch_ok(W, 32, Cp, 3, 3, x.dtype)):
+            and not _cfg.get("no_fork_accumulate") and _plus1x1_route(B, H, W, cout, Cp, cout, x.dtype)):
         dx = new_act(B, Cp, H, W, x.dtype, x.device)
         fork_slot["buf"] = dx
         fork_slot["pending"] = (dy, w, pack)
@@ -704,16 +716,25 @@
     pend = _pending_slot(fork_slot) if target is not None else None
     if pend is not None:
         dy3, w3, pack3 = pend["pending"]
-        if ((kh, kw) == (3, 3) and sites is None and target is pend["buf"] and _patch_ok(W, cout, Cp, 3, 3, x.dtype)
-                and tuple(dy3.shape[2:]) == (H, W) and dy3.dtype == x.dtype):
+        route = 0
+        if ((kh, kw) == (3, 3) and sites is None and target is pend["buf"] and tuple(dy3.shape[2:]) == (H, W) and dy3.dtype == x.dtype
+                and tuple(w3.shape[2:]) == (1, 1)):
+            route = _plus1x1_route(B, H, W, cout, Cp, dy3.shape[1], x.dtype)
+        if route:
             del pend["pending"]
             d3p, ldd3 = _pl(dy3)
             dxp, lddx = _pl(target)
-            lib.mte_conv2d_patch_fwd_plus1x1(dyp, lddy, pack.get_patch(w, 'b').data_ptr(), 0, dxp, lddx, B, H, W, cout, Cp,
-                                             d3p, ldd3, pack3.get_patch(w3, 'b').data_ptr(), dy3.shape[1], st)
+            if route == 1:
+                wp, wp3 = pack.get_patch(w, 'b'), pack3.get_patch(w3, 'b')
+            else:
+                wp, wp3 = pack.get(w, x.dtype, True)[1], pack3.get(w3, x.dtype, True)[1]
+            lib.mte_conv2d_patch_fwd_plus1x1(dyp, lddy, wp.data_ptr(), 0, dxp, lddx, B, H, W, cout, Cp, d3p, ldd3, wp3.data_ptr(), dy3.shape[1], st)
+            _dgrad_counts["folded"] += 1
             fork_slot["buf"] = target
             return target
         _flush_pending(pend)
+    if (kh, kw) == (1, 1) and fork_slot is not None:
+        _dgrad_counts["standalone_1x1"] += 1
     dx = target if target is not None else new_act(B, Cp, H, W, x.dtype, x.device)
     if target is None and sites is not None:
         dx.zero_()
@@ -1487,7 +1508,13 @@
     cout = w3.shape[0]
     d3p, ldd3 = _pl(dy3)
     dxp, lddx = _pl(dx)
-    lib.mte_conv2d_patch_fwd(d3p, ldd3, pack3.get_patch(w3, 'b').data_ptr(), 0, dxp, lddx, B, H, W, cout, Cp, 1, 1, 0, _stream())
+    _dgrad_counts["standalone_1x1"] += 1
+    if _patch_ok(W, cout, Cp, 1, 1, dx.dtype):
+        lib.mte_conv2d_patch_fwd(d3p, ldd3, pack3.get_patch(w3, 'b').data_ptr(), 0, dxp, lddx, B, H, W, cout, Cp, 1, 1, 0, _stream())
+    else:
+        _, wb = pack3.get(w3, dx.dtype, True)
+        ws, ws_n = _splitk_workspace(B * H * W, Cp, dx.device)
+        lib.mte_conv2d_igemm(d3p, ldd3, wb.data_ptr(), 0, dxp, lddx, 0, B, H, W, cout, Cp, 1, 1, _dt(dx), _ptr(ws), ws_n, 0, _stream())
 
 
 def _fork_target(slot, shape, dtype, keep_pending=False):
```

Result: no change. 385.2 images/sec (median of 2 runs) (+0.4%).
